# TheoCoombes/ClipCap

Measured on AMD Instinct MI355X. Metric: train samples/sec (512-d prefix, 40-tok caption), higher is better.
Workload: dtype bf16; 1 GPU; BASELINE configs[1]: TransformerMapper(8L,P=L=10,H=8)+frozen GPT-2-small; per_gpu_batch=256, global_batch=256, encoder_dim=512, train_language_model=False, parallelism=dp1

## Files before the change

clipcap_amd/_lib.py:

```python
from __future__ import annotations

import ctypes as C
import os
import threading

HERE = os.path.dirname(os.path.abspath(__file__))
_SEL = os.environ.get("CLIPCAP_HIP_LIB", "")
LIB_PATH = os.path.join(HERE, "libclipcap_hip.so") if not _SEL else os.path.join(HERE, "libclipcap_hip_lab.so") if _SEL == "lab" else _SEL
IS_LAB = _SEL == "lab"

ERR = {0: "ok", -1: "invalid argument", -2: "unsupported shape / alignment", -3: "kernel launch failed", -4: "invalid state"}


class HipExtensionMissing(RuntimeError):
    pass


class CCError(RuntimeError):
    pass


OP_BF16, OP_FP16, OP_X3 = 0, 1, 2


def op_dtype_of(precision) -> int:
    if precision in ("bf16", None) or (precision == OP_BF16 and not isinstance(precision, bool)):
        return OP_BF16
    if precision in (16, "fp16", "16", OP_FP16):
        return OP_FP16
    if precision in (32, 64, "32", "64", "bf16x3", "fp32", OP_X3):
        return OP_X3
    raise ValueError(f"unsupported precision {precision!r}: use 32 / 64 (split-bf16 operands, the reference default), 16 (fp16 operands) "
                     "or 'bf16' (bf16 operands)")


class MapperCfg(C.Structure):
    _fields_ = [(n, C.c_int32) for n in ("E", "D", "P", "L", "H", "N", "Hm", "W", "use_pos", "op_dtype")]


class Gpt2Cfg(C.Structure):
    _fields_ = [(n, C.c_int32) for n in ("D", "H", "NL", "V", "Vp", "NPOS", "op_dtype")]


class Gpt2Shape(C.Structure):
    _fields_ = [(n, C.c_int32) for n in ("B", "L", "T", "cap", "mode")] + [(n, C.c_float) for n in ("p_embd", "p_attn", "p_resid")] + \
               [("drop_seed", C.c_uint64)]


_P, _I, _L, _F = C.c_void_p, C.c_int32, C.c_int64, C.c_float
_MC, _GC, _GS = C.POINTER(MapperCfg), C.POINTER(Gpt2Cfg), C.POINTER(Gpt2Shape)

SIGNATURES = {
    "cc_abi_version": (_I, []),
    "cc_mapper_param_count": (_L, [_MC]),
    "cc_mapper_param_offsets": (_I, [_MC, C.POINTER(_L)]),
    "cc_mapper_ws_bytes": (_L, [_MC, _I, _I]),
    "cc_mapper_sync_weights": (_I, [_MC, _P, _P, _P]),
    "cc_mapper_transpose_weights": (_I, [_MC, _P, _P]),
    "cc_gpt2_sync_weights": (_I, [_GC, _P, _P, _P]),
    "cc_gpt2_transpose_weights": (_I, [_GC, _P, _P]),
    "cc_mapper_fwd": (_I, [_MC, _I, _P, _P, _P, _P, _P, _I, _P]),
    "cc_mapper_attention_probs": (_I, [_MC, _I, _P, _I, _P, _P]),
    "cc_mapper_bwd": (_I, [_MC, _I, _P, _P, _P, _P, _P, _P]),
    "cc_mapper_bwd_range": (_I, [_MC, _I, _P, _P, _P, _P, _P, _I, _I, _P]),
    "cc_gpt2_bwd_range": (_I, [_GC, _GS, _P, _P, _P, _P, _P, _P, _I, _I, _P]),
    "cc_gpt2_param_count": (_L, [_GC]),
    "cc_gpt2_param_offsets": (_I, [_GC, C.POINTER(_L)]),
    "cc_gpt2_ws_bytes": (_L, [_GC, _GS]),
    "cc_gpt2_embed": (_I, [_GC, _GS, _P, _P, _P, _P, _P]),
    "cc_gpt2_embed_from": (_I, [_GC, _GS, _P, _P, _P, _P]),
    "cc_gpt2_fwd": (_I, [_GC, _GS, _P, _P, _P, _P]),
    "cc_gpt2_logits": (_I, [_GC, _GS, _P, _P, _P, _P, _L, _P]),
    "cc_gpt2_logits_bwd": (_I, [_GC, _GS, _P, _P, _P, _P, _L, _P, _P, _P]),
    "cc_lmhead_ce_fwd": (_I, [_GC, _GS, _P, _P, _P, _P, _P, _P]),
    "cc_lmhead_score": (_I, [_GC, _GS, _P, _P, _P, _P, _I, _P, _P, _P]),
    "cc_lmhead_ce_bwd": (_I, [_GC, _GS, _P, _P, _P, _P, _P, _P, _P]),
    "cc_gpt2_bwd": (_I, [_GC, _GS, _P, _P, _P, _P, _P, _P, _P]),
    "cc_decode_ws_bytes": (_L, [_GC, _I, _I]),
    "cc_decode_fwd": (_I, [_GC, _I, _I, _I, _I, _P, _P, _P, _P, _P, _P, _P, _L, _P]),
    "cc_decode_part_floats": (_L, [_GC, _I]),
    "cc_decode_fwd_p": (_I, [_GC, _I, _I, _I, _I, _P, _P, _P, _P, _P, _P, _P, _L, _P, _P]),
    "cc_decode_fwd_g": (_I, [_GC, _I, _I, _I, _I, _P, _P, _P, _P, _P, _I, _P, _P, _L, _P, _P]),
    "cc_beam_step_p": (_I, [_I, _I, _I, _P, _L, _P, _I, _F, _I, _I, _P, _P, _P, _P, _P, _P, _P]),
    "cc_decode_reorder": (_I, [_GC, _I, _I, _I, _I, _P, _P, _P, _P]),
    "cc_beam_step": (_I, [_I, _I, _I, _P, _L, _F, _I, _I, _P, _P, _P, _P, _P, _P, _P]),
    "cc_beam_ws_bytes": (_L, [_I, _I, _I]),
    "cc_embed_tokens": (_I, [_GC, _I, _P, _P, _P, _P]),
    "cc_embed_tokens_bwd": (_I, [_GC, _I, _P, _P, _P, _P]),
    "cc_embed_tokens_bwd_ws": (_I, [_GC, _I, _P, _P, _P, _P, _P]),
    "cc_embed_tokens_bwd_ws_bytes": (_L, [_GC, _I]),
    "cc_beam_advance": (_I, [_GC, _I, _I, _P, _P, _P, _I, _I, _P, _P, _I, _I, _P, _P, _P, _P]),
    "cc_adamw_step": (_I, [_P, _P, _P, _P, _L, _F, _F, _F, _F, _F, _I, _F, _P, _P, _P]),
    "cc_adamw_step_cast": (_I, [_I, _P, _P, _P, _P, _L, _F, _F, _F, _F, _F, _I, _F, _P, _P, _P, _P]),
    "cc_cast_op16": (_I, [_I, _P, _P, _L, _P]),
    "cc_grad_wire_pack": (_I, [_P, _P, _L, _P]),
    "cc_grad_wire_unpack": (_I, [_P, _P, _L, _P]),
    "cc_grad_nonfinite": (_I, [_P, _L, _P, _P]),
    "cc_loss_scale_update": (_I, [_P, _P, _F, _F, _I, _P]),
    "cc_dropout_mask": (_I, [C.c_uint64, _I, _I, _F, _L, _P, _P]),
    "cc_sample_step": (_I, [_P, _I, _I, _I, _F, _I, _F, _I, _P, _I, _I, _F, _P, _P, _P, _P]),
    "cc_sample_step_lp": (_I, [_P, _I, _I, _I, _F, _I, _F, _I, _P, _I, _I, _F, _I, _F, _P, _P, _P, _P]),
    "cc_wgrad_scratch_bytes": (_L, []),
    "cc_gemm_wgrad": (_I, [_I, _P, _I, _P, _I, _I, _I, _I, _P, _I, _P, _P]),
    "cc_x3_image_bytes": (_L, [_L, _L]),
    "cc_x3_split_rows": (_I, [_I, _P, _L, _I, _I, _I, _P, _P]),
    "cc_gemm_act": (_I, [_I, _I, _I, _P, _I, _I, _P, _I, _I, _I, _I, _P, _I, _I, _P, _I, _P, _P, _L, _P]),
    "cc_gemm_resid": (_I, [_I, _I, _I, _P, _I, _I, _P, _I, _I, _I, _I, _P, _P, _I, _P, _F, C.c_uint64, _I, _I, _P, _L, _P]),
    "cc_gemm_dact": (_I, [_I, _I, _I, _P, _I, _I, _P, _I, _I, _I, _I, _P, _I, _I, _P, _I, _P, _L, _P]),
    "cc_gemm_f32": (_I, [_I, _I, _I, _P, _I, _I, _P, _I, _I, _I, _I, _P, _I, _P, _I, _F, _I, _P, _L, _P]),
    "cc_gemm_wgrad_split": (_I, [_I, _P, _I, _I, _P, _I, _I, _I, _I, _P, _I, _P, _P, _L, _P]),
    "cc_gemm_tile_mode": (_I, [_I]),
    "cc_gemm_skinny_mode": (_I, [_I]),
    "cc_decode_mode": (_I, [_I]),
    "cc_gemm_op16_f32": (_I, [_I, _I, _I, _P, _I, _P, _I, _I, _I, _I, _P, _I, _P, _I, _P]),
    "cc_layernorm_fwd": (_I, [_I, _P, _P, _P, _P, _P, _P, _I, _I, _P]),
    "cc_attention_fwd": (_I, [_I, _P, _I, _I, _I, _I, _I, _P, _P, _P]),
    "cc_attention_bwd": (_I, [_I, _P, _P, _P, _P, _P, _I, _I, _I, _I, _I, _P, _P]),
    "cc_red_scratch_floats": (_L, []),
    "cc_layernorm_bwd": (_I, [_I, _P, _P, _I, _P, _P, _P, _P, _P, _P, _P, _P, _P, _P, _I, _I, _P, _P]),
    "cc_colsum_bf16": (_I, [_I, _P, _I, _I, _I, _P, _P, _P]),
    "cc_colsum_multi": (_I, [_I, _P, _P, _I, _I, _I, _I, _P, _P]),
    "cc_batch_sum": (_I, [_P, _L, _P, _I, _I, _P, _P]),
    "cc_comm_unique_id": (_I, [_P]),
    "cc_comm_create": (_I, [C.POINTER(_P), _I, _I, _P]),
    "cc_allreduce_bucket": (_I, [_P, _P, _L, _I, _P]),
    "cc_broadcast_bucket": (_I, [_P, _P, _L, _I, _I, _P]),
    "cc_reduce_bucket": (_I, [_P, _P, _L, _I, _I, _P]),
    "cc_comm_destroy": (_I, [_P]),
    "cc_comm_count": (_I, [_P, C.POINTER(_I)]),
    "cc_prof_start": (_I, [_I, _I]),
    "cc_prof_stop": (_I, [C.POINTER(C.c_float), C.POINTER(C.c_double), C.POINTER(_I)]),
}

LAB_SIGNATURES = {
    "cc_decode_ws_check": (_I, [_GC, _I, _I, _P, _P]),
    "cc_decode_image_bytes": (_L, [_GC]),
    "cc_decode_image": (_I, [_GC, _P, _P, _P]),
    "cc_decode_xt_image_bytes": (_L, [_GC]),
    "cc_decode_xt_image": (_I, [_GC, _P, _P, _P]),
    "cc_decode_fwd_x": (_I, [_GC, _I, _I, _I, _I, _P, _P, _P, _P, _P, _P, _P, _I, _P, _P, _L, _P, _P]),
    "cc_decode_last_path": (_I, []),
}

ABI_VERSION = 3

SITES = {"lmhead_fwd": 1, "lmhead_dgrad": 2, "gpt2_fc_fwd": 3, "gpt2_proj2_fwd": 4, "gpt2_fc_dgrad": 5, "mapper_fc1_fwd": 6,
         "mapper_qkv_fwd": 7, "mapper_wgrad_fc2": 8, "all_gemms": 100}

_lib = None
_lock = threading.Lock()


def lib() -> C.CDLL:
    global _lib
    if _lib is not None:
        return _lib
    with _lock:
        if _lib is None:
            if not os.path.exists(LIB_PATH):
                raise HipExtensionMissing(
                    f"{LIB_PATH} not found: build it with `make -C clipcap_amd/csrc` (hipcc, gfx950). "
                    "clipcap_amd has no CPU fallback.")
            try:
                l = C.CDLL(LIB_PATH)
            except OSError as e:
                raise HipExtensionMissing(f"cannot load {LIB_PATH}: {e}") from e
            sigs = dict(SIGNATURES, **LAB_SIGNATURES) if IS_LAB else SIGNATURES
            for name, (res, args) in sigs.items():
                fn = getattr(l, name)
                fn.restype = res
                fn.argtypes = args
            if l.cc_abi_version() != ABI_VERSION:
                raise HipExtensionMissing(f"libclipcap_hip.so ABI version {l.cc_abi_version()} != {ABI_VERSION} (include/clipcap_hip.h); rebuild")
            _lib = l
    return _lib


def check(rc: int, what: str = "") -> int:
    if rc < 0:
        raise CCError(f"{what or 'clipcap_hip call'} failed: {ERR.get(rc, rc)} ({rc})")
    return rc
```

clipcap_amd/csrc/api.hip:

```cpp
#include "../../include/clipcap_hip.h"
#include "gemm_api.h"
#include "kernels.h"
#include "shared.h"

using namespace CC_NS;

#define CC_TRY(expr)                 \
    do {                             \
        int _e = (expr);             \
        if (_e != CC_OK) return _e;  \
    } while (0)

#include <vector>

namespace {

constexpr int MAX_LAYERS = 96;

#define CC_TIMED(site, st, expr)                 \
    do {                                         \
        cc_shared::ProfScope _ps(site, st);      \
        int _e = (expr);                         \
        if (_e != CC_OK) return _e;              \
    } while (0)

struct TileScope {
    int old;
    bool on;
    explicit TileScope(int mode) : old(cc_shared::g_gemm_tile_mode), on(mode != -2) { if (on) cc_shared::g_gemm_tile_mode = mode; }
    ~TileScope() { if (on) cc_shared::g_gemm_tile_mode = old; }
};
inline int env_tile(const char* name) {
    const char* e = cc_lab_env(name);
    return e ? atoi(e) : -2;
}

struct Carver {
    char* base;
    size_t off = 0;
    explicit Carver(void* p) : base(static_cast<char*>(p)) {}
    template <class T>
    T* take(size_t n) {
        off = (off + 255) & ~size_t(255);
        T* r = base ? reinterpret_cast<T*>(base + off) : nullptr;
        off += n * sizeof(T);
        return r;
    }
};

inline hipStream_t S_(void* s) { return static_cast<hipStream_t>(s); }
inline int rup(int x, int m) { return (x + m - 1) / m * m; }

constexpr int PL = kX3 ? 3 : 1;
inline const uint16_t* W16(const uint16_t* w16, int64_t off) { return w16 + (size_t)PL * off; }
inline uint16_t* W16(uint16_t* w16, int64_t off) { return w16 + (size_t)PL * off; }
inline size_t x3_img(size_t rows, size_t depth) { return ((rows * 3 * depth * sizeof(op16_t)) + 255) & ~size_t(255); }
template <class WS>
inline Call call_of(hipStream_t st, const WS& w) { return Call{st, w.red, w.x3, w.x3_bytes}; }

struct MapperOff {
    int64_t lin_w, lin_b, prefix, pos;
    struct Layer {
        int64_t n1w, n1b, wq, wkv, wp, bp, n2w, n2b, w1, b1, w2, b2;
    } layer[MAX_LAYERS];
    int64_t total;
};

bool mapper_cfg_ok(const cc_mapper_cfg* c) {
    return c && (c->op_dtype == CC_OP) && c->E > 0 && c->D > 0 && c->P > 0 && c->L > 0 && c->H > 0 && c->N >= 0 && c->N <= MAX_LAYERS && c->Hm > 0 && c->W >= 1 &&
           (c->E % 8) == 0 && (c->D % 8) == 0 && (c->Hm % 8) == 0 && (c->D % c->H) == 0 && ((c->D / c->H) % 8) == 0;
}

void mapper_offsets(const cc_mapper_cfg* c, MapperOff& o) {
    int64_t p = 0;
    const int64_t D = c->D, E = c->E, PD = (int64_t)c->P * D, Hm = c->Hm;
    o.lin_w = p; p += PD * E;
    o.lin_b = p; p += PD;
    o.prefix = p; p += (int64_t)c->L * D;
    if (c->W > 1 && c->use_pos) { o.pos = p; p += (int64_t)c->W * PD; } else o.pos = -1;
    for (int l = 0; l < c->N; l++) {
        auto& y = o.layer[l];
        y.n1w = p; p += D;
        y.n1b = p; p += D;
        y.wq = p; p += D * D;
        y.wkv = p; p += 2 * D * D;
        y.wp = p; p += D * D;
        y.bp = p; p += D;
        y.n2w = p; p += D;
        y.n2b = p; p += D;
        y.w1 = p; p += Hm * D;
        y.b1 = p; p += Hm;
        y.w2 = p; p += D * Hm;
        y.b2 = p; p += D;
    }
    o.total = p;
}

constexpr int kDeferRows = 40960;
struct MapperWS {
    act_t* emb16;
    float* lin_tmp;
    float* x[MAX_LAYERS + 1];
    float* x1[MAX_LAYERS];
    act_t *xn1[MAX_LAYERS], *xn2[MAX_LAYERS], *qkv[MAX_LAYERS], *att[MAX_LAYERS], *h[MAX_LAYERS];
    float *lse[MAX_LAYERS], *mean1[MAX_LAYERS], *rstd1[MAX_LAYERS], *mean2[MAX_LAYERS], *rstd2[MAX_LAYERS];
    float* dx32;
    act_t *dx16, *dx16b, *dh16, *dxn16, *datt16, *dqkv16, *dlin16;
    act_t *gdx[MAX_LAYERS], *gdxb[MAX_LAYERS], *gdh[MAX_LAYERS], *gdqkv[MAX_LAYERS];
    bool own_grads;
    float* wg_scratch;
    float* red;
    float* adelta;
    uint16_t* gimg;
    char* x3;
    size_t x3_bytes;
    size_t bytes;
};

void mapper_carve(const cc_mapper_cfg* c, int B, int save, void* ws, MapperWS& w) {
    Carver cv(ws);
    const int S = c->W * c->P + c->L;
    const size_t M = (size_t)B * S, D = c->D;
    w.emb16 = cv.take<act_t>((size_t)B * c->W * c->E);
    w.lin_tmp = c->W > 1 ? cv.take<float>((size_t)B * c->W * c->P * D) : nullptr;
    const int nx = save ? c->N + 1 : 2;
    float* xb[MAX_LAYERS + 1];
    for (int i = 0; i < nx; i++) xb[i] = cv.take<float>(M * D);
    for (int l = 0; l <= c->N; l++) w.x[l] = save ? xb[l] : xb[l & 1];
    const int nl = save ? c->N : 1;
    for (int l = 0; l < c->N; l++) {
        const bool fresh = l < nl;
        const int s = fresh ? l : 0;
        if (fresh) {
            w.x1[l] = cv.take<float>(M * D);
            w.xn1[l] = cv.take<act_t>(M * D);
            w.xn2[l] = cv.take<act_t>(M * D);
            w.qkv[l] = cv.take<act_t>(M * 3 * D);
            w.att[l] = cv.take<act_t>(M * D);
            w.h[l] = cv.take<act_t>(M * c->Hm);
            w.lse[l] = cv.take<float>((size_t)B * c->H * S);
            w.mean1[l] = cv.take<float>(M);
            w.rstd1[l] = cv.take<float>(M);
            w.mean2[l] = cv.take<float>(M);
            w.rstd2[l] = cv.take<float>(M);
        } else {
            w.x1[l] = w.x1[s]; w.xn1[l] = w.xn1[s]; w.xn2[l] = w.xn2[s]; w.qkv[l] = w.qkv[s]; w.att[l] = w.att[s]; w.h[l] = w.h[s];
            w.lse[l] = w.lse[s]; w.mean1[l] = w.mean1[s]; w.rstd1[l] = w.rstd1[s]; w.mean2[l] = w.mean2[s]; w.rstd2[l] = w.rstd2[s];
        }
    }
    if (save) {
        w.dx32 = cv.take<float>(M * D);
        w.dx16 = cv.take<act_t>(M * D);
        w.dx16b = cv.take<act_t>(M * D);
        w.dh16 = cv.take<act_t>(M * c->Hm);
        w.dxn16 = cv.take<act_t>(M * D);
        w.datt16 = cv.take<act_t>(M * D);
        w.dqkv16 = cv.take<act_t>(M * 3 * D);
        w.dlin16 = cv.take<act_t>((size_t)B * c->W * c->P * D);
        w.own_grads = !kX3 && M <= (size_t)kDeferRows && c->N <= 8;
        for (int l = 0; l < c->N; l++) {
            const bool own = w.own_grads;
            w.gdx[l] = own ? cv.take<act_t>(M * D) : w.dx16;
            w.gdxb[l] = own ? cv.take<act_t>(M * D) : w.dx16b;
            w.gdh[l] = own ? cv.take<act_t>(M * c->Hm) : w.dh16;
            w.gdqkv[l] = own ? cv.take<act_t>(M * 3 * D) : w.dqkv16;
        }
        w.wg_scratch = cv.take<float>(WGRAD_SCRATCH_BYTES / sizeof(float));
        w.red = cv.take<float>(RED_SCRATCH_FLOATS);
        w.adelta = cv.take<float>((size_t)B * c->H * S);
        w.gimg = kX3 ? reinterpret_cast<uint16_t*>(cv.take<char>(x3_img(M, std::max<size_t>(3 * (size_t)D, c->Hm)))) : nullptr;
    } else {
        w.dx32 = nullptr; w.dx16 = w.dx16b = w.dh16 = w.dxn16 = w.datt16 = w.dqkv16 = w.dlin16 = nullptr; w.wg_scratch = nullptr; w.adelta = nullptr;
        w.red = nullptr;
        w.gimg = nullptr;
        for (int l = 0; l < c->N; l++) w.gdx[l] = w.gdxb[l] = w.gdh[l] = w.gdqkv[l] = nullptr;
        w.own_grads = false;
    }
    w.x3 = nullptr; w.x3_bytes = 0;
    if (kX3) {
        const size_t Hm = c->Hm, Mb = (size_t)B * c->W, PD = (size_t)c->P * D;
        size_t need = std::max(x3_img(Mb, c->E), x3_img(M, std::max(D, Hm)));
        if (save) {
            need = std::max(need, x3_img(M, 3 * D));
            need = std::max(need, std::max(x3_img(M, D) + x3_img(M, Hm), x3_img(M, 3 * D) + x3_img(M, D)));
            need = std::max(need, x3_img(Mb, PD) + x3_img(Mb, c->E));
        }
        w.x3_bytes = need;
        w.x3 = cv.take<char>(need);
    }
    w.bytes = (cv.off + 255) & ~size_t(255);
}

struct Gpt2Off {
    int64_t wte, wpe, lnf_w, lnf_b;
    struct Layer {
        int64_t l1w, l1b, aw, ab, pw, pb, l2w, l2b, fw, fb, p2w, p2b;
    } layer[MAX_LAYERS];
    int64_t total;
};

bool gpt2_cfg_ok(const cc_gpt2_cfg* c) {
    return c && (c->op_dtype == CC_OP) && c->D > 0 && c->H > 0 && c->NL > 0 && c->NL <= MAX_LAYERS && c->V > 0 && c->Vp >= c->V && (c->Vp % 128) == 0 &&
           c->NPOS > 0 && (c->D % 8) == 0 && (c->D % c->H) == 0 && ((c->D / c->H) % 8) == 0;
}

void gpt2_offsets(const cc_gpt2_cfg* c, Gpt2Off& o) {
    int64_t p = 0;
    const int64_t D = c->D;
    o.wte = p; p += (int64_t)c->Vp * D;
    o.wpe = p; p += (int64_t)c->NPOS * D;
    for (int l = 0; l < c->NL; l++) {
        auto& y = o.layer[l];
        y.l1w = p; p += D;
        y.l1b = p; p += D;
        y.aw = p; p += D * 3 * D;
        y.ab = p; p += 3 * D;
        y.pw = p; p += D * D;
        y.pb = p; p += D;
        y.l2w = p; p += D;
        y.l2b = p; p += D;
        y.fw = p; p += D * 4 * D;
        y.fb = p; p += 4 * D;
        y.p2w = p; p += 4 * D * D;
        y.p2b = p; p += D;
    }
    o.lnf_w = p; p += D;
    o.lnf_b = p; p += D;
    o.total = p;
}

static bool x3_img_on() {
    static const bool on = []() { const char* e = cc_lab_env("CC_X3_IMG"); return !e || atoi(e) != 0; }();
    return on;
}
static bool lm_exp_form(const cc_gpt2_shape* s) {
    static const bool env = []() { const char* e = cc_lab_env("CC_LM_EXPFORM"); return !e || atoi(e) != 0; }();
    if (CC_OP == 0) return env;
    if (CC_OP == 2) return env && x3_img_on() && s->mode == 1;
    return false;
}
static Act lm_logits(const cc_gpt2_cfg* c, const cc_gpt2_shape* s, act_t* logits16) { return Act(logits16, (kX3 && lm_exp_form(s)) ? c->Vp : 0); }

struct Gpt2WS {
    float* x[MAX_LAYERS + 1];
    float* x1[MAX_LAYERS];
    act_t *qkv[MAX_LAYERS], *u[MAX_LAYERS];
    Act xn1[MAX_LAYERS], xn2[MAX_LAYERS], att[MAX_LAYERS], hact[MAX_LAYERS];
    float *lse[MAX_LAYERS], *mean1[MAX_LAYERS], *rstd1[MAX_LAYERS], *mean2[MAX_LAYERS], *rstd2[MAX_LAYERS];
    act_t* hf16;
    float *meanf, *rstdf;
    int *target, *row_map;
    int* keep;
    act_t* logits16;
    float *pmax, *psum, *tgt_logit, *lse_row, *row_loss;
    float *cref, *lmfac;
    act_t* hfs16;
    float* dx32;
    Act dx16, dx16b, du16, dqkv16;
    act_t *dhf16, *dxn16, *datt16;
    float* wg_scratch;
    float* red;
    void* scat;
    float* adelta;
    char* x3;
    size_t x3_bytes;
    size_t bytes;
};

void gpt2_carve(const cc_gpt2_cfg* c, const cc_gpt2_shape* s, int cap, void* ws, Gpt2WS& w) {
    Carver cv(ws);
    const int B = s->B, T = s->T, hd = c->D / c->H;
    const size_t M = (size_t)B * T, D = c->D, Mc = (size_t)B * cap;
    const bool keep = s->mode >= 1, full = s->mode >= 2;
    const bool img = kX3 && !full && x3_img_on();
    const bool bimg = img && keep && s->p_resid == 0.f && s->p_attn == 0.f && s->p_embd == 0.f;
    const int xw = img ? (int)D : 0, attw = (img && attn_fwd_can_image(T, hd)) ? (int)D : 0, hw = img ? 4 * (int)D : 0;
    const int dxw = bimg ? (int)D : 0, dqw = (bimg && attn_bwd_can_image(T, hd)) ? 3 * (int)D : 0;
    const int nx = keep ? c->NL + 1 : 2;
    float* xb[MAX_LAYERS + 1];
    for (int i = 0; i < nx; i++) xb[i] = cv.take<float>(M * D);
    for (int l = 0; l <= c->NL; l++) w.x[l] = keep ? xb[l] : xb[l & 1];
    for (int l = 0; l < c->NL; l++) {
        const bool k0 = keep || l == 0, f0 = full || l == 0;
        w.x1[l] = k0 ? cv.take<float>(M * D) : w.x1[0];
        w.qkv[l] = k0 ? cv.take<act_t>(M * 3 * D) : w.qkv[0];
        w.u[l] = k0 ? cv.take<act_t>(M * 4 * D) : w.u[0];
        w.lse[l] = k0 ? cv.take<float>((size_t)B * c->H * T) : w.lse[0];
        w.mean1[l] = k0 ? cv.take<float>(M) : w.mean1[0];
        w.rstd1[l] = k0 ? cv.take<float>(M) : w.rstd1[0];
        w.mean2[l] = k0 ? cv.take<float>(M) : w.mean2[0];
        w.rstd2[l] = k0 ? cv.take<float>(M) : w.rstd2[0];
        w.xn1[l] = f0 ? Act(cv.take<act_t>(M * D * ((kX3 && !full) ? 3 : 2) / 2), xw) : w.xn1[0];
        w.xn2[l] = f0 ? Act(cv.take<act_t>(M * D * ((kX3 && !full) ? 3 : 2) / 2), xw) : w.xn2[0];
        w.att[l] = k0 ? Act(cv.take<act_t>(M * D * ((kX3 && !full) ? 3 : 2) / 2), attw) : w.att[0];
        w.hact[l] = f0 ? Act(cv.take<act_t>(M * 4 * D * ((kX3 && !full) ? 3 : 2) / 2), hw) : w.hact[0];
    }
    const size_t Mh = std::max(M, Mc);
    w.hf16 = cv.take<act_t>(Mh * D);
    w.meanf = cv.take<float>(Mh);
    w.rstdf = cv.take<float>(Mh);
    w.target = cv.take<int>(Mh);
    w.row_map = cv.take<int>(Mh);
    w.keep = nullptr;
    if (keep) {
        const int npart = c->Vp / 64;
        w.logits16 = cv.take<act_t>(Mc * c->Vp * ((kX3 && !full) ? 3 : 2) / 2);
        w.pmax = cv.take<float>(Mc * npart);
        w.psum = cv.take<float>(Mc * npart);
        w.tgt_logit = cv.take<float>(Mc);
        w.lse_row = cv.take<float>(Mc);
        w.row_loss = cv.take<float>(Mc);
        w.cref = cv.take<float>(Mc);
        w.lmfac = cv.take<float>(2 * Mc);
        w.hfs16 = full ? cv.take<act_t>(Mc * D) : nullptr;
        w.dx32 = cv.take<float>(M * D);
        w.dx16 = Act(cv.take<act_t>(M * D * ((kX3 && !full) ? 3 : 2) / 2), dxw);
        w.dx16b = full ? Act(cv.take<act_t>(M * D)) : w.dx16;
        w.dhf16 = cv.take<act_t>(Mc * D);
        w.du16 = Act(cv.take<act_t>(M * 4 * D * ((kX3 && !full) ? 3 : 2) / 2), hw);
        w.dxn16 = cv.take<act_t>(M * D);
        w.datt16 = cv.take<act_t>(M * D);
        w.dqkv16 = Act(cv.take<act_t>(M * 3 * D * ((kX3 && !full) ? 3 : 2) / 2), dqw);
        w.wg_scratch = full ? cv.take<float>(WGRAD_SCRATCH_BYTES / sizeof(float)) : nullptr;
        w.red = full ? cv.take<float>(RED_SCRATCH_FLOATS) : nullptr;
        w.scat = full ? cv.take<char>(scatter_ws_bytes((int)Mc, (int)D)) : nullptr;
        w.adelta = cv.take<float>((size_t)B * c->H * T);
    } else {
        w.wg_scratch = nullptr; w.adelta = nullptr; w.red = nullptr; w.scat = nullptr;
        w.logits16 = nullptr; w.pmax = w.psum = w.tgt_logit = w.lse_row = w.row_loss = nullptr;
        w.cref = w.lmfac = nullptr; w.hfs16 = nullptr;
        w.dx32 = nullptr; w.dx16 = w.dx16b = w.du16 = w.dqkv16 = Act(); w.dhf16 = w.dxn16 = w.datt16 = nullptr;
        if (Mc > 0) {
            const int npart = c->Vp / 64;
            w.pmax = cv.take<float>(Mc * npart);
            w.psum = cv.take<float>(Mc * npart);
            w.tgt_logit = cv.take<float>(Mc);
            w.lse_row = cv.take<float>(Mc);
            w.keep = cv.take<int>(Mc);
        }
    }
    w.x3 = nullptr; w.x3_bytes = 0;
    if (kX3) {
        size_t need = x3_img(Mh, 4 * D);
        if (keep) need = std::max(need, x3_img(Mc, c->Vp));
        if (full) need = std::max(need, std::max(x3_img(M, D) + x3_img(M, 4 * D), x3_img(Mc, c->Vp) + x3_img(Mc, D)));
        w.x3_bytes = need;
        w.x3 = cv.take<char>(need);
    }
    w.bytes = (cv.off + 255) & ~size_t(255);
}

}

extern "C" {

int CC_API(cc_mapper_bwd_range)(const cc_mapper_cfg* c, int32_t B, const float* w32, const uint16_t* w16, void* ws, const float* dout, float* g32,
                        int32_t l_hi, int32_t l_lo, void* stream);
int CC_API(cc_gpt2_bwd_range)(const cc_gpt2_cfg* c, const cc_gpt2_shape* s, const float* w32, const uint16_t* w16, void* ws, const int64_t* tokens,
                      float* dprefix, float* g32, int32_t l_hi, int32_t l_lo, void* stream);

int64_t CC_API(cc_mapper_param_count)(const cc_mapper_cfg* cfg) {
    if (!mapper_cfg_ok(cfg)) return CC_ERR_SHAPE;
    MapperOff o;
    mapper_offsets(cfg, o);
    return o.total;
}

int CC_API(cc_mapper_param_offsets)(const cc_mapper_cfg* cfg, int64_t* offs) {
    if (!mapper_cfg_ok(cfg) || !offs) return CC_ERR_SHAPE;
    MapperOff o;
    mapper_offsets(cfg, o);
    int k = 0;
    offs[k++] = o.lin_w; offs[k++] = o.lin_b; offs[k++] = o.prefix; offs[k++] = o.pos;
    for (int l = 0; l < cfg->N; l++) {
        const auto& y = o.layer[l];
        const int64_t v[12] = {y.n1w, y.n1b, y.wq, y.wkv, y.wp, y.bp, y.n2w, y.n2b, y.w1, y.b1, y.w2, y.b2};
        for (int i = 0; i < 12; i++) offs[k++] = v[i];
    }
    return CC_OK;
}

int64_t CC_API(cc_mapper_ws_bytes)(const cc_mapper_cfg* cfg, int32_t B, int32_t save) {
    if (!mapper_cfg_ok(cfg) || B <= 0) return CC_ERR_SHAPE;
    MapperWS w;
    mapper_carve(cfg, B, save, nullptr, w);
    return (int64_t)w.bytes;
}

#if CC_OP == 2
static int mapper_sync_x3(const cc_mapper_cfg* c, const float* w32, uint16_t* w16, hipStream_t st) {
    MapperOff o;
    mapper_offsets(c, o);
    const int D = c->D, Hm = c->Hm;
    X3SplitBatch sb;
    sb.add(w32 + o.lin_w, W16(w16, o.lin_w), c->P * D, c->E, 0, 1);
    for (int l = 0; l < c->N; l++) {
        const auto& y = o.layer[l];
        const int64_t off[4] = {y.wq, y.wp, y.w1, y.w2};
        const int R[4] = {3 * D, D, Hm, D}, C[4] = {D, D, D, Hm};
        for (int i = 0; i < 4; i++) {
            if (sb.n + 2 > 32) { CC_TRY(x3_split_multi(sb, st)); sb.n = 0; }
            sb.add(w32 + off[i], W16(w16, off[i]), R[i], C[i], 0, 1);
            sb.add(w32 + off[i], W16(w16, o.total + off[i]), R[i], C[i], 1, 1);
        }
    }
    return x3_split_multi(sb, st);
}
#endif

static int mapper_transposes(const cc_mapper_cfg* c, uint16_t* w16, hipStream_t st) {
    if (kX3) return CC_ERR_ARG;
    MapperOff o;
    mapper_offsets(c, o);
    op16_t* t = w16 + o.total;
    const int D = c->D, Hm = c->Hm;
    TransposeBatch tb;
    for (int l = 0; l < c->N; l++) {
        const auto& y = o.layer[l];
        tb.add(w16 + y.wq, t + y.wq, 3 * D, D);
        tb.add(w16 + y.wp, t + y.wp, D, D);
        tb.add(w16 + y.w1, t + y.w1, Hm, D);
        tb.add(w16 + y.w2, t + y.w2, D, Hm);
        if (tb.n == 32) { CC_TRY(transpose_bf16_multi(tb, st)); tb.n = 0; }
    }
    CC_TRY(transpose_bf16_multi(tb, st));
    return CC_OK;
}

int CC_API(cc_mapper_sync_weights)(const cc_mapper_cfg* c, const float* w32, uint16_t* w16, void* stream) {
    if (!mapper_cfg_ok(c) || !w32 || !w16) return CC_ERR_ARG;
    hipStream_t st = S_(stream);
#if CC_OP == 2
    return mapper_sync_x3(c, w32, w16, st);
#else
    MapperOff o;
    mapper_offsets(c, o);
    CC_TRY(f32_to_bf16(w32, w16, (size_t)o.total, st));
    return mapper_transposes(c, w16, st);
#endif
}

int CC_API(cc_mapper_transpose_weights)(const cc_mapper_cfg* c, uint16_t* w16, void* stream) {
    if (!mapper_cfg_ok(c) || !w16) return CC_ERR_ARG;
    return mapper_transposes(c, w16, S_(stream));
}

int CC_API(cc_mapper_fwd)(const cc_mapper_cfg* c, int32_t B, const float* w32, const uint16_t* w16, const float* emb, void* ws, float* out,
                  int32_t save, void* stream) {
    if (!mapper_cfg_ok(c) || B <= 0 || !w32 || !w16 || !emb || !ws || !out) return CC_ERR_ARG;
    hipStream_t st = S_(stream);
    MapperOff o;
    mapper_offsets(c, o);
    MapperWS w;
    mapper_carve(c, B, save, ws, w);
    Call cx = call_of(st, w);
    const int D = c->D, PP = c->W * c->P, S = PP + c->L, M = B * S, H = c->H, hd = D / H, Hm = c->Hm;
    const int PD = c->P * D;
    CC_TRY(f32_to_act(emb, w.emb16, (size_t)B * c->W * c->E, st));
    if (c->W == 1) {
        CC_TRY(gemm_f32out(0, 0, w.emb16, c->E, W16(w16, o.lin_w), c->E, B, PD, c->E, w.x[0], S * D, w32 + o.lin_b, 0, 1.0f, 1, cx));
    } else {
        CC_TRY(gemm_f32out(0, 0, w.emb16, c->E, W16(w16, o.lin_w), c->E, B * c->W, PD, c->E, w.lin_tmp, PD, w32 + o.lin_b, 0, 1.0f, 1, cx));
        CC_TRY(copy_rows(w.lin_tmp, (size_t)PP * D, w.x[0], (size_t)S * D, PP * D, B, st));
        if (o.pos >= 0) CC_TRY(add_rows(w.x[0], (size_t)S * D, w32 + o.pos, PP * D, B, st));
    }
    CC_TRY(broadcast_rows(w.x[0] + (size_t)PP * D, (size_t)S * D, w32 + o.prefix, c->L * D, B, st));
    for (int l = 0; l < c->N; l++) {
        const auto& y = o.layer[l];
        CC_TRY(ln_fwd(w.x[l], D, nullptr, w32 + y.n1w, w32 + y.n1b, w.xn1[l], nullptr, w.mean1[l], w.rstd1[l], M, D, st));
        CC_TIMED(CC_SITE_MAPPER_QKV_FWD, st, gemm_bf16out(0, 0, w.xn1[l], D, W16(w16, y.wq), D, M, 3 * D, D, w.qkv[l], 3 * D, nullptr, 0, nullptr, cx));
        CC_TRY(attn_fwd(w.qkv[l], B, S, H, hd, false, w.att[l], w.lse[l], st));
        CC_TRY(gemm_resid(0, 0, w.att[l], D, W16(w16, y.wp), D, M, D, D, w.x1[l], w.x[l], D, w32 + y.bp, cx));
        CC_TRY(ln_fwd(w.x1[l], D, nullptr, w32 + y.n2w, w32 + y.n2b, w.xn2[l], nullptr, w.mean2[l], w.rstd2[l], M, D, st));
        CC_TIMED(CC_SITE_MAPPER_FC1_FWD, st, gemm_bf16out(0, 0, w.xn2[l], D, W16(w16, y.w1), D, M, Hm, D, w.h[l], Hm, w32 + y.b1, 1, nullptr, cx));
        CC_TRY(gemm_resid(0, 0, w.h[l], Hm, W16(w16, y.w2), Hm, M, D, Hm, w.x[l + 1], w.x1[l], D, w32 + y.b2, cx));
    }
    CC_TRY(copy_rows(w.x[c->N] + (size_t)PP * D, (size_t)S * D, out, (size_t)c->L * D, c->L * D, B, st));
    return CC_OK;
}

int CC_API(cc_mapper_attention_probs)(const cc_mapper_cfg* c, int32_t B, void* ws, int32_t layer, float* out, void* stream) {
    if (!mapper_cfg_ok(c) || B <= 0 || !ws || !out || layer < 0 || layer >= c->N) return CC_ERR_ARG;
    MapperWS w;
    mapper_carve(c, B, 1, ws, w);
    const int S = c->W * c->P + c->L;
    return attn_probs(w.qkv[layer], B, S, c->H, c->D / c->H, out, S_(stream));
}

int CC_API(cc_mapper_bwd)(const cc_mapper_cfg* c, int32_t B, const float* w32, const uint16_t* w16, void* ws, const float* dout, float* g32,
                  void* stream) {
    if (!mapper_cfg_ok(c)) return CC_ERR_ARG;
    return CC_API(cc_mapper_bwd_range)(c, B, w32, w16, ws, dout, g32, c->N, 0, stream);
}

int CC_API(cc_mapper_bwd_range)(const cc_mapper_cfg* c, int32_t B, const float* w32, const uint16_t* w16, void* ws, const float* dout, float* g32,
                        int32_t l_hi, int32_t l_lo, void* stream) {
    if (!mapper_cfg_ok(c) || B <= 0 || !w32 || !w16 || !ws || !dout || !g32 || l_lo < 0 || l_hi > c->N || l_lo > l_hi) return CC_ERR_ARG;
    hipStream_t st = S_(stream);
    MapperOff o;
    mapper_offsets(c, o);
    MapperWS w;
    mapper_carve(c, B, 1, ws, w);
    Call cx = call_of(st, w);
    const int D = c->D, PP = c->W * c->P, S = PP + c->L, M = B * S, H = c->H, hd = D / H, Hm = c->Hm;
    const int PD = c->P * D;
    const uint16_t* w16t = W16(w16, o.total);
    if (l_hi == c->N) {
        if (hipMemsetAsync(w.dx32, 0, (size_t)M * D * sizeof(float), st) != hipSuccess) return CC_ERR_LAUNCH;
        CC_TRY(copy_rows(dout, (size_t)c->L * D, w.dx32 + (size_t)PP * D, (size_t)S * D, c->L * D, B, st));
        if (c->N > 0) CC_TRY(f32_to_act(w.dx32, w.gdx[c->N - 1], (size_t)M * D, st));
    }
    WgradBatch wb;
    wb.defer = true;
    constexpr bool kDeferAll = !kX3;
    static const bool defer_all_on = []() { const char* e = cc_lab_env("CC_MAPPER_WGRAD_DEFER"); return !e || atoi(e) != 0; }();
    static const int defer_rows = []() { const char* e = cc_lab_env("CC_MAPPER_DEFER_ROWS"); return e ? std::min(atoi(e), kDeferRows) : kDeferRows; }();
    const bool defer_all = kDeferAll && defer_all_on && w.own_grads && 4 * (l_hi - l_lo) <= 32 && M <= defer_rows;
    if (defer_all) { wb.direct = true; wb.cap = 4 * (l_hi - l_lo); }
    ColsumBatch cs;
#if CC_OP == 2
    static const bool share = []() { const char* e = cc_lab_env("CC_X3_SHARE"); return !e || atoi(e) != 0; }();
    int g2rc = CC_OK;
    auto G2 = [&](const act_t* t, int width) -> ActIn {
        if (!share) return t;
        g2rc = x3_split_rows(t, (size_t)width, w.gimg, M, width, 0, st);
        return ActIn(reinterpret_cast<const act_t*>(w.gimg), width);
    };
#else
    auto G2 = [&](const act_t* t, int) -> ActIn { return t; };
    const int g2rc = CC_OK;
#endif
    for (int l = l_hi - 1; l >= l_lo; l--) {
        const auto& y = o.layer[l];
        act_t* dx16 = w.gdx[l];
        act_t* dx16b = w.gdxb[l];
        act_t* dh16 = w.gdh[l];
        act_t* dqkv16 = w.gdqkv[l];
        act_t* dx16_below = l > 0 ? w.gdx[l - 1] : w.datt16;
        const ActIn gx = G2(dx16, D);
        CC_TRY(g2rc);
        CC_TIMED(CC_SITE_MAPPER_WGRAD_FC2, st, gemm_wgrad(gx, D, w.h[l], Hm, D, Hm, M, g32 + y.w2, Hm, w.wg_scratch, cx, &wb));
        if (l == c->N - 1) CC_TRY(colsum_bf16(dx16, D, M, D, g32 + y.b2, cx));
        CC_TRY(gemm_dact(0, 0, gx, D, W16(w16t, y.w2), D, M, Hm, D, dh16, Hm, w.h[l], 1, cx));
        const ActIn gh = G2(dh16, Hm);
        CC_TRY(g2rc);
        CC_TRY(gemm_wgrad(gh, Hm, w.xn2[l], D, Hm, D, M, g32 + y.w1, D, w.wg_scratch, cx, &wb));
        if (defer_all) cs.add(dh16, g32 + y.b1);
        else CC_TRY(colsum_bf16(dh16, Hm, M, Hm, g32 + y.b1, cx));
        CC_TRY(gemm_bf16out(0, 0, gh, Hm, W16(w16t, y.w1), Hm, M, D, Hm, w.dxn16, D, nullptr, 0, nullptr, cx));
        CC_TRY(ln_bwd(w.dxn16, w.x1[l], D, nullptr, w.mean2[l], w.rstd2[l], w32 + y.n2w, w.dx32, w.dx32, dx16b, g32 + y.n2w,
                      g32 + y.n2b, M, D, cx, g32 + y.bp));
        const ActIn gb = G2(dx16b, D);
        CC_TRY(g2rc);
        CC_TRY(gemm_wgrad(gb, D, w.att[l], D, D, D, M, g32 + y.wp, D, w.wg_scratch, cx, &wb));
        CC_TRY(gemm_bf16out(0, 0, gb, D, W16(w16t, y.wp), D, M, D, D, w.datt16, D, nullptr, 0, nullptr, cx));
        CC_TRY(attn_bwd(w.qkv[l], w.datt16, w.att[l], w.lse[l], w.adelta, B, S, H, hd, false, dqkv16, st));
        const ActIn gq = G2(dqkv16, 3 * D);
        CC_TRY(g2rc);
        CC_TRY(gemm_wgrad(gq, 3 * D, w.xn1[l], D, 3 * D, D, M, g32 + y.wq, D, w.wg_scratch, cx, &wb));
        CC_TRY(gemm_bf16out(0, 0, gq, 3 * D, W16(w16t, y.wq), 3 * D, M, D, 3 * D, w.dxn16, D, nullptr, 0, nullptr, cx));
        if (!defer_all) CC_TRY(wgrad_flush(wb, st));
        CC_TRY(ln_bwd(w.dxn16, w.x[l], D, nullptr, w.mean1[l], w.rstd1[l], w32 + y.n1w, w.dx32, w.dx32, dx16_below, g32 + y.n1w,
                      g32 + y.n1b, M, D, cx, l > 0 ? g32 + o.layer[l - 1].b2 : nullptr));
    }
    CC_TRY(wgrad_flush(wb, st));
    CC_TRY(colsum_bf16_multi(cs, Hm, M, Hm, cx));
    if (l_lo > 0) return CC_OK;
    CC_TRY(batch_sum(w.dx32 + (size_t)PP * D, (size_t)S * D, g32 + o.prefix, c->L * D, B, cx));
    if (o.pos >= 0) CC_TRY(batch_sum(w.dx32, (size_t)S * D, g32 + o.pos, PP * D, B, cx));
    CC_TRY(slice_f32_to_bf16(w.dx32, (size_t)S * D, w.dlin16, (size_t)PP * D, PP * D, B, st));
    CC_TRY(gemm_wgrad(w.dlin16, PD, w.emb16, c->E, PD, c->E, B * c->W, g32 + o.lin_w, c->E, w.wg_scratch, cx));
    CC_TRY(colsum_bf16(w.dlin16, PD, B * c->W, PD, g32 + o.lin_b, cx));
    return CC_OK;
}

namespace {
static bool gelu_grad_fwd() {
    static const bool on = []() { const char* e = cc_lab_env("CC_GELU_GRAD_FWD"); return !e || atoi(e) != 0; }();
    return on;
}
static bool shape_ok(const cc_gpt2_cfg* c, const cc_gpt2_shape* s) {
    return s && s->B > 0 && s->T > 0 && s->L >= 0 && s->L <= s->T && s->cap >= s->T - s->L && s->mode >= 0 && s->mode <= 2 && s->T <= c->NPOS &&
           s->p_embd >= 0.f && s->p_embd < 1.f && s->p_attn >= 0.f && s->p_attn < 1.f && s->p_resid >= 0.f && s->p_resid < 1.f;
}
}

int64_t CC_API(cc_gpt2_param_count)(const cc_gpt2_cfg* cfg) {
    if (!gpt2_cfg_ok(cfg)) return CC_ERR_SHAPE;
    Gpt2Off o;
    gpt2_offsets(cfg, o);
    return o.total;
}

int CC_API(cc_gpt2_param_offsets)(const cc_gpt2_cfg* cfg, int64_t* offs) {
    if (!gpt2_cfg_ok(cfg) || !offs) return CC_ERR_SHAPE;
    Gpt2Off o;
    gpt2_offsets(cfg, o);
    int k = 0;
    offs[k++] = o.wte; offs[k++] = o.wpe;
    for (int l = 0; l < cfg->NL; l++) {
        const auto& y = o.layer[l];
        const int64_t v[12] = {y.l1w, y.l1b, y.aw, y.ab, y.pw, y.pb, y.l2w, y.l2b, y.fw, y.fb, y.p2w, y.p2b};
        for (int i = 0; i < 12; i++) offs[k++] = v[i];
    }
    offs[k++] = o.lnf_w; offs[k++] = o.lnf_b;
    return CC_OK;
}

int64_t CC_API(cc_gpt2_ws_bytes)(const cc_gpt2_cfg* cfg, const cc_gpt2_shape* s) {
    if (!gpt2_cfg_ok(cfg) || !shape_ok(cfg, s)) return CC_ERR_SHAPE;
    Gpt2WS w;
    gpt2_carve(cfg, s, s->T - s->L, nullptr, w);
    return (int64_t)w.bytes;
}

#if CC_OP == 2
static int gpt2_sync_x3(const cc_gpt2_cfg* c, const float* w32, uint16_t* w16, hipStream_t st) {
    Gpt2Off o;
    gpt2_offsets(c, o);
    const int D = c->D;
    X3SplitBatch sb;
    sb.add(w32 + o.wte, W16(w16, o.wte), c->Vp, D, 0, 1);
    sb.add(w32 + o.wte, W16(w16, o.total + o.wte), c->Vp, D, 1, 1);
    CC_TRY(x3_split_multi(sb, st));
    sb.n = 0;
    for (int l = 0; l < c->NL; l++) {
        const auto& y = o.layer[l];
        const int64_t off[4] = {y.aw, y.pw, y.fw, y.p2w};
        const int R[4] = {D, D, D, 4 * D}, C[4] = {3 * D, D, 4 * D, D};
        for (int i = 0; i < 4; i++) {
            if (sb.n + 2 > 32) { CC_TRY(x3_split_multi(sb, st)); sb.n = 0; }
            sb.add(w32 + off[i], W16(w16, off[i]), R[i], C[i], 0, 1);
            sb.add(w32 + off[i], W16(w16, o.total + off[i]), R[i], C[i], 1, 1);
        }
    }
    return x3_split_multi(sb, st);
}
#endif

static int gpt2_transposes(const cc_gpt2_cfg* c, uint16_t* w16, hipStream_t st) {
    if (kX3) return CC_ERR_ARG;
    Gpt2Off o;
    gpt2_offsets(c, o);
    op16_t* t = w16 + o.total;
    const int D = c->D;
    CC_TRY(transpose_bf16(w16 + o.wte, t + o.wte, c->Vp, D, st));
    TransposeBatch tb;
    for (int l = 0; l < c->NL; l++) {
        const auto& y = o.layer[l];
        tb.add(w16 + y.aw, t + y.aw, D, 3 * D);
        tb.add(w16 + y.pw, t + y.pw, D, D);
        tb.add(w16 + y.fw, t + y.fw, D, 4 * D);
        tb.add(w16 + y.p2w, t + y.p2w, 4 * D, D);
        if (tb.n == 32) { CC_TRY(transpose_bf16_multi(tb, st)); tb.n = 0; }
    }
    CC_TRY(transpose_bf16_multi(tb, st));
    return CC_OK;
}

int CC_API(cc_gpt2_sync_weights)(const cc_gpt2_cfg* c, const float* w32, uint16_t* w16, void* stream) {
    if (!gpt2_cfg_ok(c) || !w32 || !w16) return CC_ERR_ARG;
    hipStream_t st = S_(stream);
#if CC_OP == 2
    return gpt2_sync_x3(c, w32, w16, st);
#else
    Gpt2Off o;
    gpt2_offsets(c, o);
    CC_TRY(f32_to_bf16(w32, w16, (size_t)o.total, st));
    return gpt2_transposes(c, w16, st);
#endif
}

int CC_API(cc_gpt2_transpose_weights)(const cc_gpt2_cfg* c, uint16_t* w16, void* stream) {
    if (!gpt2_cfg_ok(c) || !w16) return CC_ERR_ARG;
    return gpt2_transposes(c, w16, S_(stream));
}

int CC_API(cc_dropout_mask)(uint64_t seed, int32_t site, int32_t layer, float p, int64_t n, uint8_t* out, void* stream) {
    if (!out || n < 0 || site < 0 || site > 3 || layer < 0 || layer > 255 || p < 0.f || p >= 1.f) return CC_ERR_ARG;
    return dropout_mask_u8(out, (size_t)n, make_drop(p, seed, (unsigned)site, (unsigned)layer), S_(stream));
}

int CC_API(cc_gpt2_embed)(const cc_gpt2_cfg* c, const cc_gpt2_shape* s, const float* w32, const float* prefix, const int64_t* tokens, void* ws,
                  void* stream) {
    if (!gpt2_cfg_ok(c) || !shape_ok(c, s) || !w32 || !ws || (s->L > 0 && !prefix) || (s->T > s->L && !tokens)) return CC_ERR_ARG;
    Gpt2Off o;
    gpt2_offsets(c, o);
    Gpt2WS w;
    gpt2_carve(c, s, s->T - s->L, ws, w);
    CC_TRY(embed_concat(prefix, reinterpret_cast<const long long*>(tokens), s->cap, w32 + o.wte, w32 + o.wpe, w.x[0], s->B, s->L, s->T,
                        c->D, 0, S_(stream)));
    return dropout_f32(w.x[0], (size_t)s->B * s->T * c->D, make_drop(s->p_embd, s->drop_seed, DROP_EMBD, 0), S_(stream));
}

int CC_API(cc_gpt2_embed_from)(const cc_gpt2_cfg* c, const cc_gpt2_shape* s, const float* w32, const float* inputs_embeds, void* ws,
                       void* stream) {
    if (!gpt2_cfg_ok(c) || !shape_ok(c, s) || !w32 || !ws || !inputs_embeds) return CC_ERR_ARG;
    Gpt2Off o;
    gpt2_offsets(c, o);
    Gpt2WS w;
    gpt2_carve(c, s, s->T - s->L, ws, w);
    return embed_concat(inputs_embeds, nullptr, 0, w32 + o.wte, w32 + o.wpe, w.x[0], s->B, s->T, s->T, c->D, 0, S_(stream));
}

int CC_API(cc_gpt2_fwd)(const cc_gpt2_cfg* c, const cc_gpt2_shape* s, const float* w32, const uint16_t* w16, void* ws, void* stream) {
    if (!gpt2_cfg_ok(c) || !shape_ok(c, s) || !w32 || !w16 || !ws) return CC_ERR_ARG;
    hipStream_t st = S_(stream);
    Gpt2Off o;
    gpt2_offsets(c, o);
    Gpt2WS w;
    gpt2_carve(c, s, s->T - s->L, ws, w);
    Call cx = call_of(st, w);
    const int D = c->D, M = s->B * s->T, H = c->H, hd = D / H;
    const uint16_t* w16t = W16(w16, o.total);
    for (int l = 0; l < c->NL; l++) {
        const auto& y = o.layer[l];
        CC_TRY(ln_fwd(w.x[l], D, nullptr, w32 + y.l1w, w32 + y.l1b, w.xn1[l], nullptr, w.mean1[l], w.rstd1[l], M, D, st));
        CC_TRY(gemm_bf16out(0, 0, w.xn1[l], D, W16(w16t, y.aw), D, M, 3 * D, D, w.qkv[l], 3 * D, w32 + y.ab, 0, nullptr, cx));
        CC_TRY(attn_fwd(w.qkv[l], s->B, s->T, H, hd, true, w.att[l], w.lse[l], st, make_drop(s->p_attn, s->drop_seed, DROP_ATTN, l)));
        {
            static const int tile_proj = env_tile("CC_TILE_PROJ");
            TileScope ts(tile_proj);
            CC_TRY(gemm_resid(0, 0, w.att[l], D, W16(w16t, y.pw), D, M, D, D, w.x1[l], w.x[l], D, w32 + y.pb, cx,
                              make_drop(s->p_resid, s->drop_seed, DROP_RESID_ATTN, l)));
        }
        CC_TRY(ln_fwd(w.x1[l], D, nullptr, w32 + y.l2w, w32 + y.l2b, w.xn2[l], nullptr, w.mean2[l], w.rstd2[l], M, D, st));
        {
            static const int tile_fc = env_tile("CC_TILE_FC");
            TileScope ts(tile_fc);
            CC_TIMED(CC_SITE_GPT2_FC_FWD, st, gemm_bf16out(0, 0, w.xn2[l], D, W16(w16t, y.fw), D, M, 4 * D, D, w.hact[l], 4 * D, w32 + y.fb, (s->mode >= 1 && gelu_grad_fwd()) ? 3 : 2,
                                                            s->mode >= 1 ? w.u[l] : nullptr, cx));
        }
        {
            static const int tile_proj2 = env_tile("CC_TILE_PROJ2");
            TileScope ts(tile_proj2);
            CC_TIMED(CC_SITE_GPT2_PROJ2_FWD, st, gemm_resid(0, 0, w.hact[l], 4 * D, W16(w16t, y.p2w), 4 * D, M, D, 4 * D, w.x[l + 1], w.x1[l], D, w32 + y.p2b, cx,
                                                           make_drop(s->p_resid, s->drop_seed, DROP_RESID_MLP, l)));
        }
    }
    return CC_OK;
}

int CC_API(cc_gpt2_logits)(const cc_gpt2_cfg* c, const cc_gpt2_shape* s, const float* w32, const uint16_t* w16, void* ws, float* logits,
                   int64_t ldl, void* stream) {
    if (!gpt2_cfg_ok(c) || !shape_ok(c, s) || !w32 || !w16 || !ws || !logits) return CC_ERR_ARG;
    const int Ns = std::min(c->Vp, rup(c->V, 8));
    if (ldl < Ns || (ldl & 3) || ldl > 0x7fffffff) return CC_ERR_SHAPE;
    hipStream_t st = S_(stream);
    Gpt2Off o;
    gpt2_offsets(c, o);
    Gpt2WS w;
    gpt2_carve(c, s, s->T - s->L, ws, w);
    Call cx = call_of(st, w);
    const int D = c->D, M = s->B * s->T;
    CC_TRY(ln_fwd(w.x[c->NL], D, nullptr, w32 + o.lnf_w, w32 + o.lnf_b, w.hf16, nullptr, w.meanf, w.rstdf, M, D, st));
    return gemm_f32out(0, 0, w.hf16, D, W16(w16, o.wte), D, M, Ns, D, logits, (int)ldl, nullptr, 0, 1.0f, 1, cx);
}

int CC_API(cc_lmhead_ce_fwd)(const cc_gpt2_cfg* c, const cc_gpt2_shape* s, const float* w32, const uint16_t* w16, void* ws, const int64_t* tokens,
                     float* stats, void* stream) {
    if (!gpt2_cfg_ok(c) || !shape_ok(c, s) || s->mode < 1 || s->L < 1 || !w32 || !w16 || !ws || !tokens || !stats) return CC_ERR_ARG;
    hipStream_t st = S_(stream);
    Gpt2Off o;
    gpt2_offsets(c, o);
    Gpt2WS w;
    const int cap = s->T - s->L;
    gpt2_carve(c, s, cap, ws, w);
    Call cx = call_of(st, w);
    const int D = c->D, Mc = s->B * cap, npart = c->Vp / 64;
    if (cap != s->cap) return CC_ERR_SHAPE;
    if (hipMemsetAsync(stats, 0, 2 * sizeof(float), st) != hipSuccess) return CC_ERR_LAUNCH;
    CC_TRY(ce_targets(reinterpret_cast<const long long*>(tokens), w.target, w.row_map, s->B, cap, s->L, s->T, st));
    CC_TRY(ln_fwd(w.x[c->NL], D, w.row_map, w32 + o.lnf_w, w32 + o.lnf_b, w.hf16, nullptr, w.meanf, w.rstdf, Mc, D, st));
    const bool ef = lm_exp_form(s);
    const op16_t* wte_rows = kX3 ? reinterpret_cast<const op16_t*>(w32 + o.wte) : W16(w16, o.wte);
    if (ef) CC_TRY(lm_tgt_ref(w.hf16, wte_rows, D, w.target, w.cref, Mc, st));
    CC_TIMED(CC_SITE_LMHEAD_FWD, st, gemm_lmhead(w.hf16, D, W16(w16, o.wte), D, Mc, c->Vp, c->V, D, lm_logits(c, s, w.logits16), c->Vp, w.pmax, w.psum, npart, w.target, w.tgt_logit, cx,
                                                 ef ? w.cref : nullptr));
    CC_TRY(ce_rows(w.pmax, w.psum, npart, w.target, ef ? w.cref : w.tgt_logit, w.lse_row, w.row_loss, stats, Mc, st));
    return CC_OK;
}

int CC_API(cc_lmhead_score)(const cc_gpt2_cfg* c, const cc_gpt2_shape* s, const float* w32, const uint16_t* w16, void* ws, const int64_t* tokens,
                    int32_t ignore_zero, float* token_logprob, float* sample_stats, void* stream) {
    if (!gpt2_cfg_ok(c) || !shape_ok(c, s) || s->mode != 0 || s->L < 1 || !w32 || !w16 || !ws || !tokens || !token_logprob || !sample_stats)
        return CC_ERR_ARG;
    const int cap = s->T - s->L;
    if (cap < 1 || cap != s->cap) return CC_ERR_SHAPE;
    hipStream_t st = S_(stream);
    Gpt2Off o;
    gpt2_offsets(c, o);
    Gpt2WS w;
    gpt2_carve(c, s, cap, ws, w);
    Call cx = call_of(st, w);
    const int D = c->D, Mc = s->B * cap, npart = c->Vp / 64;
    CC_TRY(ce_targets(reinterpret_cast<const long long*>(tokens), w.target, w.row_map, s->B, cap, s->L, s->T, st));
    CC_TRY(score_keep(reinterpret_cast<const long long*>(tokens), w.keep, Mc, ignore_zero, st));
    CC_TRY(ln_fwd(w.x[c->NL], D, w.row_map, w32 + o.lnf_w, w32 + o.lnf_b, w.hf16, nullptr, w.meanf, w.rstdf, Mc, D, st));
    CC_TIMED(CC_SITE_LMHEAD_FWD, st, gemm_lmhead_score(w.hf16, D, W16(w16, o.wte), D, Mc, c->Vp, c->V, D, w.pmax, w.psum, npart, w.target, w.tgt_logit, cx));
    return score_rows(w.pmax, w.psum, npart, w.keep, w.tgt_logit, w.lse_row, token_logprob, sample_stats, s->B, cap, st);
}

int CC_API(cc_lmhead_ce_bwd)(const cc_gpt2_cfg* c, const cc_gpt2_shape* s, const float* w32, const uint16_t* w16, void* ws, const float* denom,
                     const float* loss_scale, float* g32, void* stream) {
    if (!gpt2_cfg_ok(c) || !shape_ok(c, s) || s->mode < 1 || !w32 || !w16 || !ws || !denom || (s->mode == 2 && !g32)) return CC_ERR_ARG;
    hipStream_t st = S_(stream);
    Gpt2Off o;
    gpt2_offsets(c, o);
    Gpt2WS w;
    const int cap = s->T - s->L;
    gpt2_carve(c, s, cap, ws, w);
    Call cx = call_of(st, w);
    const int D = c->D, Mc = s->B * cap, M = s->B * s->T;
    const bool full = s->mode == 2;
    const bool ef = lm_exp_form(s);
    const LmFix fix{w.lmfac, w.target, kX3 ? reinterpret_cast<const op16_t*>(w32 + o.wte) : W16(w16, o.wte)};
    if (ef) CC_TRY(lm_rowfac(w.cref, w.lse_row, w.target, denom, loss_scale, w.lmfac, Mc, st));
    const Act lg = lm_logits(c, s, w.logits16);
    ActIn dlog = lg;
    op16_t* dimg = (kX3 && !ef && !full && x3_img_on()) ? x3_scratch_block(cx, x3_img(Mc, c->Vp)) : nullptr;
    if (dimg) dlog = ActIn(reinterpret_cast<const act_t*>(dimg), c->Vp);
    if (!ef) CC_TRY(ce_dlogits(w.logits16, c->Vp, c->V, w.target, w.lse_row, denom, loss_scale, Mc, st, dimg));
    const auto lm_dgrad = [&]() {
        const int rc = gemm_nt_deepk(dlog, c->Vp, W16(w16, o.total + o.wte), c->Vp, Mc, D, c->Vp, w.dhf16, D, reinterpret_cast<float*>(w.du16.p),
                                     (size_t)M * 4 * D * sizeof(act_t), cx, ef ? &fix : nullptr);
        if (rc != CC_ERR_SHAPE) return rc;
        const int rc2 = gemm_bf16out(0, 0, dlog, c->Vp, W16(w16, o.total + o.wte), c->Vp, Mc, D, c->Vp, w.dhf16, D, nullptr, 0, nullptr, cx);
        return (rc2 != CC_OK || !ef) ? rc2 : lm_dgrad_fix(w.dhf16, w.lmfac, w.target, fix.wte, D, Mc, st);
    };
    CC_TIMED(CC_SITE_LMHEAD_DGRAD, st, lm_dgrad());
    if (full) {
        if (ef) {
            CC_TRY(lm_scale_rows(w.hf16, w.lmfac, w.hfs16, D, Mc, st));
            CC_TRY(gemm_wgrad(lg, c->Vp, w.hfs16, D, c->Vp, D, Mc, g32 + o.wte, D, w.wg_scratch, cx));
            ScatterSrc oh;
            oh.ids32 = w.target; oh.act = w.hf16; oh.fac = w.lmfac;
            CC_TRY(scatter_rows(oh, Mc, D, c->Vp, g32 + o.wte, w.scat, st));
        } else {
            CC_TRY(gemm_wgrad(lg, c->Vp, w.hf16, D, c->Vp, D, Mc, g32 + o.wte, D, w.wg_scratch, cx));
        }
    }
    if (hipMemsetAsync(w.dx32, 0, (size_t)M * D * sizeof(float), st) != hipSuccess) return CC_ERR_LAUNCH;
    const size_t dx16_bytes = (size_t)M * D * (w.dx16.img ? 3 * sizeof(op16_t) : sizeof(act_t));
    if (hipMemsetAsync(w.dx16.p, 0, dx16_bytes, st) != hipSuccess) return CC_ERR_LAUNCH;
    CC_TRY(ln_bwd(w.dhf16, w.x[c->NL], D, w.row_map, w.meanf, w.rstdf, w32 + o.lnf_w, nullptr, w.dx32, w.dx16, full ? g32 + o.lnf_w : nullptr,
                  full ? g32 + o.lnf_b : nullptr, Mc, D, cx));
    return CC_OK;
}

int CC_API(cc_gpt2_logits_bwd)(const cc_gpt2_cfg* c, const cc_gpt2_shape* s, const float* w32, const uint16_t* w16, void* ws, const float* dlogits,
                       int64_t ldl, float* dx0, float* g32, void* stream) {
    if (!gpt2_cfg_ok(c) || !shape_ok(c, s) || s->mode < 1 || s->L != 0 || !w32 || !w16 || !ws || !dlogits || ldl < c->V || (s->mode == 2 && !g32))
        return CC_ERR_ARG;
    hipStream_t st = S_(stream);
    Gpt2Off o;
    gpt2_offsets(c, o);
    Gpt2WS w;
    gpt2_carve(c, s, s->T, ws, w);
    Call cx = call_of(st, w);
    const int D = c->D, M = s->B * s->T;
    const bool full = s->mode == 2;
    CC_TRY(f32_to_op16_pad(dlogits, ldl, c->V, w.logits16, c->Vp, M, st));
    CC_TRY(gemm_bf16out(0, 0, w.logits16, c->Vp, W16(w16, o.total + o.wte), c->Vp, M, D, c->Vp, w.dhf16, D, nullptr, 0, nullptr, cx));
    if (full) CC_TRY(gemm_wgrad(w.logits16, c->Vp, w.hf16, D, c->Vp, D, M, g32 + o.wte, D, w.wg_scratch, cx));
    if (hipMemsetAsync(w.dx32, 0, (size_t)M * D * sizeof(float), st) != hipSuccess) return CC_ERR_LAUNCH;
    CC_TRY(ln_bwd(w.dhf16, w.x[c->NL], D, nullptr, w.meanf, w.rstdf, w32 + o.lnf_w, nullptr, w.dx32, w.dx16, full ? g32 + o.lnf_w : nullptr,
                  full ? g32 + o.lnf_b : nullptr, M, D, cx));
    CC_TRY(CC_API(cc_gpt2_bwd_range)(c, s, w32, w16, ws, nullptr, nullptr, g32, c->NL, 0, stream));
    if (dx0 && hipMemcpyAsync(dx0, w.dx32, (size_t)M * D * sizeof(float), hipMemcpyDeviceToDevice, st) != hipSuccess) return CC_ERR_LAUNCH;
    return CC_OK;
}

int CC_API(cc_gpt2_bwd)(const cc_gpt2_cfg* c, const cc_gpt2_shape* s, const float* w32, const uint16_t* w16, void* ws, const int64_t* tokens,
                float* dprefix, float* g32, void* stream) {
    if (!gpt2_cfg_ok(c)) return CC_ERR_ARG;
    return CC_API(cc_gpt2_bwd_range)(c, s, w32, w16, ws, tokens, dprefix, g32, c->NL, 0, stream);
}

int CC_API(cc_gpt2_bwd_range)(const cc_gpt2_cfg* c, const cc_gpt2_shape* s, const float* w32, const uint16_t* w16, void* ws, const int64_t* tokens,
                      float* dprefix, float* g32, int32_t l_hi, int32_t l_lo, void* stream) {
    if (!gpt2_cfg_ok(c) || !shape_ok(c, s) || s->mode < 1 || !w32 || !w16 || !ws || (s->L > 0 && !dprefix) || (s->mode == 2 && !g32) ||
        l_lo < 0 || l_hi > c->NL || l_lo > l_hi)
        return CC_ERR_ARG;
    hipStream_t st = S_(stream);
    Gpt2Off o;
    gpt2_offsets(c, o);
    Gpt2WS w;
    gpt2_carve(c, s, s->T - s->L, ws, w);
    Call cx = call_of(st, w);
    const int D = c->D, M = s->B * s->T, H = c->H, hd = D / H, D3 = 3 * D, D4 = 4 * D;
    const bool full = s->mode == 2;
    WgradBatch wb;
    wb.defer = full;
    WgradBatch* wbp = full ? &wb : nullptr;
    if (full && (w.dx16.img || w.dx16b.img || w.du16.img || w.dqkv16.img)) return CC_ERR_STATE;
    for (int l = l_hi - 1; l >= l_lo; l--) {
        const auto& y = o.layer[l];
        const bool top = l == c->NL - 1;
        if (top) CC_TRY(dropout_bf16(w.dx16.p, (size_t)M * D, make_drop(s->p_resid, s->drop_seed, DROP_RESID_MLP, l), st));
        if (full) {
            CC_TRY(gemm_wgrad(w.hact[l], D4, w.dx16.p, D, D4, D, M, g32 + y.p2w, D, w.wg_scratch, cx, wbp));
            if (top) CC_TRY(colsum_bf16(w.dx16.p, D, M, D, g32 + y.p2b, cx));
        }
        {
            static const int tile_dact = env_tile("CC_TILE_DACT");
            TileScope ts(tile_dact);
            CC_TRY(gemm_dact(0, 0, w.dx16, D, W16(w16, y.p2w), D, M, D4, D, w.du16, D4, w.u[l], gelu_grad_fwd() ? 3 : 2, cx));
        }
        if (full) {
            CC_TRY(gemm_wgrad(w.xn2[l], D, w.du16.p, D4, D, D4, M, g32 + y.fw, D4, w.wg_scratch, cx, wbp));
            CC_TRY(colsum_bf16(w.du16.p, D4, M, D4, g32 + y.fb, cx));
        }
        CC_TIMED(CC_SITE_GPT2_FC_DGRAD, st, gemm_bf16out(0, 0, w.du16, D4, W16(w16, y.fw), D4, M, D, D4, w.dxn16, D, nullptr, 0, nullptr, cx));
        CC_TRY(ln_bwd(w.dxn16, w.x1[l], D, nullptr, w.mean2[l], w.rstd2[l], w32 + y.l2w, w.dx32, w.dx32, w.dx16b, full ? g32 + y.l2w : nullptr,
                      full ? g32 + y.l2b : nullptr, M, D, cx, full ? g32 + y.pb : nullptr,
                      make_drop(s->p_resid, s->drop_seed, DROP_RESID_ATTN, l)));
        if (full) CC_TRY(gemm_wgrad(w.att[l], D, w.dx16b.p, D, D, D, M, g32 + y.pw, D, w.wg_scratch, cx, wbp));
        CC_TRY(gemm_bf16out(0, 0, w.dx16b, D, W16(w16, y.pw), D, M, D, D, w.datt16, D, nullptr, 0, nullptr, cx));
        CC_TRY(attn_bwd(w.qkv[l], w.datt16, w.att[l].p, w.lse[l], w.adelta, s->B, s->T, H, hd, true, w.dqkv16, st,
                        make_drop(s->p_attn, s->drop_seed, DROP_ATTN, l)));
        if (full) {
            CC_TRY(gemm_wgrad(w.xn1[l], D, w.dqkv16.p, D3, D, D3, M, g32 + y.aw, D3, w.wg_scratch, cx, wbp));
            CC_TRY(colsum_bf16(w.dqkv16.p, D3, M, D3, g32 + y.ab, cx));
        }
        CC_TRY(gemm_bf16out(0, 0, w.dqkv16, D3, W16(w16, y.aw), D3, M, D, D3, w.dxn16, D, nullptr, 0, nullptr, cx));
        if (full) CC_TRY(wgrad_flush(wb, st));
        CC_TRY(ln_bwd(w.dxn16, w.x[l], D, nullptr, w.mean1[l], w.rstd1[l], w32 + y.l1w, w.dx32, w.dx32, w.dx16, full ? g32 + y.l1w : nullptr,
                      full ? g32 + y.l1b : nullptr, M, D, cx, (full && l > 0) ? g32 + o.layer[l - 1].p2b : nullptr,
                      l > 0 ? make_drop(s->p_resid, s->drop_seed, DROP_RESID_MLP, l - 1) : Drop()));
    }
    if (l_lo > 0) return CC_OK;
    CC_TRY(dropout_f32(w.dx32, (size_t)M * D, make_drop(s->p_embd, s->drop_seed, DROP_EMBD, 0), st));
    if (s->L > 0) CC_TRY(copy_rows(w.dx32, (size_t)s->T * D, dprefix, (size_t)s->L * D, s->L * D, s->B, st));
    if (full) {
        if (tokens) {
            ScatterSrc e;
            e.ids64 = reinterpret_cast<const long long*>(tokens);
            e.ids_ld = s->cap;
            e.f32 = w.dx32 + (size_t)s->L * D; e.rpb = s->T - s->L; e.bstride = (size_t)s->T * D;
            CC_TRY(scatter_rows(e, s->B * (s->T - s->L), D, c->Vp, g32 + o.wte, w.scat, st));
        }
        CC_TRY(batch_sum(w.dx32, (size_t)s->T * D, g32 + o.wpe, s->T * D, s->B, cx));
    }
    return CC_OK;
}

int CC_API(cc_adamw_step)(float* p32, const float* g32, float* m, float* v, int64_t n, float lr, float beta1, float beta2, float eps,
                  float weight_decay, int32_t step, float grad_scale, const float* loss_scale, const float* found_inf, void* stream) {
    if (!p32 || !g32 || !m || !v || n < 0 || step < 0 || (step == 0 && !loss_scale)) return CC_ERR_ARG;
    return adamw(p32, g32, m, v, (size_t)n, lr, beta1, beta2, eps, weight_decay, step, grad_scale, loss_scale, found_inf, S_(stream));
}

int CC_API(cc_adamw_step_cast)(float* p32, const float* g32, float* m, float* v, int64_t n, float lr, float beta1, float beta2, float eps,
                       float weight_decay, int32_t step, float grad_scale, const float* loss_scale, const float* found_inf, uint16_t* w16, void* stream) {
    if (!p32 || !g32 || !m || !v || !w16 || n < 0 || step < 0 || (step == 0 && !loss_scale)) return CC_ERR_ARG;
    if (kX3) return CC_ERR_ARG;
    return adamw(p32, g32, m, v, (size_t)n, lr, beta1, beta2, eps, weight_decay, step, grad_scale, loss_scale, found_inf, S_(stream), w16);
}

int CC_API(cc_cast_op16)(const float* src, uint16_t* dst, int64_t n, void* stream) {
    if (!src || !dst || n < 0 || kX3) return CC_ERR_ARG;
    return f32_to_bf16(src, dst, (size_t)n, S_(stream));
}

int CC_API(cc_grad_wire_pack)(const float* g32, uint16_t* wire, int64_t n, void* stream) {
    if (!g32 || !wire || n < 0) return CC_ERR_ARG;
    return wire_pack(g32, wire, (size_t)n, S_(stream));
}

int CC_API(cc_grad_wire_unpack)(const uint16_t* wire, float* g32, int64_t n, void* stream) {
    if (!g32 || !wire || n < 0) return CC_ERR_ARG;
    return wire_unpack(wire, g32, (size_t)n, S_(stream));
}

int CC_API(cc_grad_nonfinite)(const float* g32, int64_t n, float* found_inf, void* stream) {
    if (!g32 || !found_inf || n < 0) return CC_ERR_ARG;
    return grad_nonfinite(g32, (size_t)n, found_inf, S_(stream));
}

int CC_API(cc_loss_scale_update)(float* state, float* found_inf, float growth, float backoff, int32_t interval, void* stream) {
    if (!state || !found_inf || growth < 1.f || backoff <= 0.f || backoff > 1.f || interval < 1) return CC_ERR_ARG;
    return loss_scale_update(state, found_inf, growth, backoff, interval, S_(stream));
}

int CC_API(cc_gemm_op16_f32)(int32_t al, int32_t bl, const uint16_t* A, int32_t lda, const uint16_t* B, int32_t ldb, int32_t M, int32_t N, int32_t K,
                     float* C, int32_t ldc, const float* bias, int32_t ksplit, void* stream) {
    if (!A || !B || !C || kX3) return CC_ERR_ARG;
    Call cx{S_(stream)};
    return gemm_f32out(al, bl, reinterpret_cast<const act_t*>(A), lda, B, ldb, M, N, K, C, ldc, ksplit > 1 ? nullptr : bias, ksplit > 1 ? 2 : 0, 1.0f, ksplit, cx);
}

int CC_API(cc_sample_step)(const float* logits, int32_t R, int32_t V, int32_t ld, float temperature, int32_t top_k, float top_p, int32_t mode,
                   const int64_t* history, int32_t hist_len, int32_t hist_ld, float repetition_penalty, const float* u, int32_t* next_token,
                   float* probs_out, void* stream) {
    if (!logits || !u || !next_token || R < 0) return CC_ERR_ARG;
    return sample_rows(logits, R, V, ld, temperature, top_k, top_p, mode, reinterpret_cast<const long long*>(history), hist_len, hist_ld,
                       repetition_penalty, u, next_token, probs_out, S_(stream));
}

int CC_API(cc_sample_step_lp)(const float* logits, int32_t R, int32_t V, int32_t ld, float temperature, int32_t top_k, float top_p, int32_t mode,
                      const int64_t* history, int32_t hist_len, int32_t hist_ld, float repetition_penalty, int32_t stop_token,
                      float length_penalty, const float* u, int32_t* next_token, float* probs_out, void* stream) {
    if (!logits || !u || !next_token || R < 0) return CC_ERR_ARG;
    return sample_rows(logits, R, V, ld, temperature, top_k, top_p, mode, reinterpret_cast<const long long*>(history), hist_len, hist_ld,
                       repetition_penalty, u, next_token, probs_out, S_(stream), stop_token, length_penalty);
}

int64_t CC_API(cc_wgrad_scratch_bytes)(void) { return (int64_t)WGRAD_SCRATCH_BYTES; }

int CC_API(cc_gemm_wgrad)(const uint16_t* X, int32_t ldx, const uint16_t* Y, int32_t ldy, int32_t Mw, int32_t Nw, int32_t K, float* dW, int32_t ldw,
                  float* scratch, void* stream) {
    if (!X || !Y || !dW || kX3) return CC_ERR_ARG;
    Call cx{S_(stream)};
    return gemm_wgrad(reinterpret_cast<const act_t*>(X), ldx, reinterpret_cast<const act_t*>(Y), ldy, Mw, Nw, K, dW, ldw, scratch, cx);
}

int CC_API(cc_layernorm_fwd)(const float* x, const float* gamma, const float* beta, uint16_t* y, float* mean, float* rstd, int32_t rows, int32_t D,
                     void* stream) {
    if (!x || !gamma || !beta || !y) return CC_ERR_ARG;
    return ln_fwd(x, D, nullptr, gamma, beta, reinterpret_cast<act_t*>(y), nullptr, mean, rstd, rows, D, S_(stream));
}

int64_t CC_API(cc_red_scratch_floats)(void) { return (int64_t)RED_SCRATCH_FLOATS; }

int CC_API(cc_layernorm_bwd)(const uint16_t* dy, const float* x, int32_t ldx, const int32_t* row_map, const float* mean, const float* rstd,
                     const float* gamma, const float* dres, float* dx32, uint16_t* dx16, float* dgamma, float* dbeta, float* dcol, int32_t rows,
                     int32_t D, float* red_ws, void* stream) {
    if (!dy || !x || !mean || !rstd || !gamma || !dx32 || !dgamma != !dbeta || kX3) return CC_ERR_ARG;
    Call cx{S_(stream), red_ws};
    return ln_bwd(reinterpret_cast<const act_t*>(dy), x, ldx, row_map, mean, rstd, gamma, dres, dx32, reinterpret_cast<act_t*>(dx16), dgamma,
                  dbeta, rows, D, cx, dcol);
}

int CC_API(cc_colsum_bf16)(const uint16_t* X, int32_t ld, int32_t M, int32_t N, float* out, float* red_ws, void* stream) {
    if (!X || !out || kX3) return CC_ERR_ARG;
    Call cx{S_(stream), red_ws};
    return colsum_bf16(reinterpret_cast<const act_t*>(X), ld, M, N, out, cx);
}

int CC_API(cc_colsum_multi)(const uint16_t* const* X_host, float* const* out_host, int32_t n, int32_t ld, int32_t M, int32_t N, float* red_ws,
                    void* stream) {
    if (!X_host || !out_host || n < 0 || n > 32 || kX3) return CC_ERR_ARG;
    ColsumBatch b;
    for (int i = 0; i < n; i++) {
        if (!X_host[i] || !out_host[i]) return CC_ERR_ARG;
        b.add(reinterpret_cast<const act_t*>(X_host[i]), out_host[i]);
    }
    Call cx{S_(stream), red_ws};
    return colsum_bf16_multi(b, ld, M, N, cx);
}

int CC_API(cc_batch_sum)(const float* src, int64_t src_stride, float* dst, int32_t len, int32_t B, float* red_ws, void* stream) {
    if (!src || !dst || len < 0 || src_stride < len) return CC_ERR_ARG;
    Call cx{S_(stream), red_ws};
    return batch_sum(src, (size_t)src_stride, dst, len, B, cx);
}

int CC_API(cc_attention_fwd)(const uint16_t* qkv, int32_t B, int32_t S, int32_t H, int32_t hd, int32_t causal, uint16_t* out, float* lse, void* stream) {
    if (!qkv || !out) return CC_ERR_ARG;
    return attn_fwd(reinterpret_cast<const act_t*>(qkv), B, S, H, hd, causal != 0, reinterpret_cast<act_t*>(out), lse, S_(stream));
}

int CC_API(cc_attention_bwd)(const uint16_t* qkv, const uint16_t* dout, const uint16_t* o, const float* lse, float* delta_ws, int32_t B, int32_t S,
                     int32_t H, int32_t hd, int32_t causal, uint16_t* dqkv, void* stream) {
    if (!qkv || !dout || !lse || !dqkv) return CC_ERR_ARG;
    return attn_bwd(reinterpret_cast<const act_t*>(qkv), reinterpret_cast<const act_t*>(dout), reinterpret_cast<const act_t*>(o), lse, delta_ws, B, S, H, hd,
                    causal != 0, reinterpret_cast<act_t*>(dqkv), S_(stream));
}

namespace {
inline bool al16(const void* p) { return ((uintptr_t)p & 15) == 0; }
inline bool hook_operands_ok(int al, int bl, const void* A, int a_img, int lda, const void* B, int ldb, int M, int N, int K) {
    if (!A || !B || !al16(A) || !al16(B) || M <= 0 || N <= 0 || K <= 0 || a_img < 0) return false;
    if (!kX3 && a_img) return false;
    return lda >= (a_img ? 0 : (al ? M : K)) && ldb >= (bl ? N : K);
}
inline void hook_scratch(Call& cx, void* x3, int64_t x3_bytes) {
    if (kX3 && x3 && x3_bytes > 0 && al16(x3)) { cx.x3 = static_cast<char*>(x3); cx.x3_bytes = (size_t)x3_bytes; }
}
inline bool hook_c_img_ok(int c_img, int N) { return c_img == 0 || (kX3 && c_img == N); }
}

int64_t CC_API(cc_x3_image_bytes)(int64_t rows, int64_t depth) {
    if (rows < 0 || depth < 0) return CC_ERR_ARG;
    return (int64_t)x3_img((size_t)rows, (size_t)depth);
}

int CC_API(cc_x3_split_rows)(const float* src, int64_t ld, int32_t rows, int32_t width, int32_t form, uint16_t* dst, void* stream) {
#if CC_OP == 2
    if (!src || !dst || rows < 0 || width < 0 || ld < width || (form != 0 && form != 1)) return CC_ERR_ARG;
    return x3_split_rows(src, (size_t)ld, dst, rows, width, form, S_(stream));
#else
    (void)src; (void)ld; (void)rows; (void)width; (void)form; (void)dst; (void)stream;
    return CC_ERR_ARG;
#endif
}

int CC_API(cc_gemm_act)(int32_t al, int32_t bl, const void* A, int32_t a_img, int32_t lda, const uint16_t* B, int32_t ldb, int32_t M, int32_t N, int32_t K,
                void* C, int32_t c_img, int32_t ldc, const float* bias, int32_t act, void* pre, void* x3, int64_t x3_bytes, void* stream) {
    if (!hook_operands_ok(al, bl, A, a_img, lda, B, ldb, M, N, K) || !C || !al16(C) || !al16(pre) || !al16(bias) || ldc < N || act < 0 || act > 3 ||
        !hook_c_img_ok(c_img, N))
        return CC_ERR_ARG;
    Call cx{S_(stream)};
    hook_scratch(cx, x3, x3_bytes);
    return gemm_bf16out(al, bl, ActIn(static_cast<const act_t*>(A), a_img), lda, B, ldb, M, N, K, Act(static_cast<act_t*>(C), c_img), ldc, bias, act,
                        static_cast<act_t*>(pre), cx);
}

int CC_API(cc_gemm_resid)(int32_t al, int32_t bl, const void* A, int32_t a_img, int32_t lda, const uint16_t* B, int32_t ldb, int32_t M, int32_t N, int32_t K,
                  float* out, const float* res, int32_t ld, const float* bias, float p, uint64_t seed, int32_t site, int32_t layer, void* x3,
                  int64_t x3_bytes, void* stream) {
    if (!hook_operands_ok(al, bl, A, a_img, lda, B, ldb, M, N, K) || !out || !res || !al16(out) || !al16(res) || !al16(bias) || ld < N || site < 0 ||
        site > 3 || layer < 0 || layer > 255 || p < 0.f || p >= 1.f)
        return CC_ERR_ARG;
    Call cx{S_(stream)};
    hook_scratch(cx, x3, x3_bytes);
    return gemm_resid(al, bl, ActIn(static_cast<const act_t*>(A), a_img), lda, B, ldb, M, N, K, out, res, ld, bias, cx,
                      make_drop(p, seed, (unsigned)site, (unsigned)layer));
}

int CC_API(cc_gemm_dact)(int32_t al, int32_t bl, const void* A, int32_t a_img, int32_t lda, const uint16_t* B, int32_t ldb, int32_t M, int32_t N, int32_t K,
                 void* C, int32_t c_img, int32_t ldc, const void* aux, int32_t act, void* x3, int64_t x3_bytes, void* stream) {
    if (!hook_operands_ok(al, bl, A, a_img, lda, B, ldb, M, N, K) || !C || !aux || !al16(C) || !al16(aux) || ldc < N || act < 1 || act > 3 ||
        !hook_c_img_ok(c_img, N))
        return CC_ERR_ARG;
    Call cx{S_(stream)};
    hook_scratch(cx, x3, x3_bytes);
    return gemm_dact(al, bl, ActIn(static_cast<const act_t*>(A), a_img), lda, B, ldb, M, N, K, Act(static_cast<act_t*>(C), c_img), ldc,
                     static_cast<const act_t*>(aux), act, cx);
}

int CC_API(cc_gemm_f32)(int32_t al, int32_t bl, const void* A, int32_t a_img, int32_t lda, const uint16_t* B, int32_t ldb, int32_t M, int32_t N, int32_t K,
                float* C, int32_t ldc, const float* bias, int32_t mode, float alpha, int32_t ksplit, void* x3, int64_t x3_bytes, void* stream) {
    if (!hook_operands_ok(al, bl, A, a_img, lda, B, ldb, M, N, K) || !C || !al16(C) || !al16(bias) || ldc < N || mode < 0 || mode > 2 || ksplit < 1 ||
        (bias && mode != 0))
        return CC_ERR_ARG;
    Call cx{S_(stream)};
    hook_scratch(cx, x3, x3_bytes);
    return gemm_f32out(al, bl, ActIn(static_cast<const act_t*>(A), a_img), lda, B, ldb, M, N, K, C, ldc, bias, mode, alpha, ksplit, cx);
}

int CC_API(cc_gemm_wgrad_split)(const void* X, int32_t x_img, int32_t ldx, const float* Y, int32_t ldy, int32_t Mw, int32_t Nw, int32_t K, float* dW,
                     int32_t ldw, float* scratch, void* x3, int64_t x3_bytes, void* stream) {
#if CC_OP == 2
    if (!X || !Y || !dW || !al16(X) || !al16(Y) || !al16(dW) || Mw <= 0 || Nw <= 0 || K <= 0 || x_img < 0 || (!x_img && ldx < Mw) || ldy < Nw || ldw < Nw)
        return CC_ERR_ARG;
    Call cx{S_(stream)};
    hook_scratch(cx, x3, x3_bytes);
    return gemm_wgrad(ActIn(static_cast<const act_t*>(X), x_img), ldx, Y, ldy, Mw, Nw, K, dW, ldw, scratch, cx);
#else
    (void)X; (void)x_img; (void)ldx; (void)Y; (void)ldy; (void)Mw; (void)Nw; (void)K; (void)dW; (void)ldw; (void)scratch; (void)x3; (void)x3_bytes; (void)stream;
    return CC_ERR_ARG;
#endif
}

}
```

clipcap_amd/csrc/gemm_api.h:

```cpp
#pragma once
#include "common.hip.h"
#include "shared.h"

namespace CC_NS {
int gemm_bf16out(int al, int bl, ActIn A, int lda, const op16_t* B, int ldb, int M, int N, int K, Act C, int ldc,
                 const float* bias, int act, act_t* pre, Call& cx);
int gemm_resid(int al, int bl, ActIn A, int lda, const op16_t* B, int ldb, int M, int N, int K, float* out, const float* res,
               int ld, const float* bias, Call& cx, Drop drop = Drop());
int gemm_f32out(int al, int bl, ActIn A, int lda, const op16_t* B, int ldb, int M, int N, int K, float* C, int ldc,
                const float* bias, int mode, float alpha, int ksplit, Call& cx);
int gemm_dact(int al, int bl, ActIn A, int lda, const op16_t* B, int ldb, int M, int N, int K, Act C, int ldc,
              const act_t* aux, int act, Call& cx);
int gemm_lmhead(ActIn A, int lda, const op16_t* B, int ldb, int M, int Vp, int V, int K, Act C, int ldc, float* pmax,
                float* psum, int npart, const int* target, float* tgt_logit, Call& cx, const float* cref = nullptr);
int gemm_lmhead_score(ActIn A, int lda, const op16_t* B, int ldb, int M, int Vp, int V, int K, float* pmax, float* psum, int npart,
                      const int* target, float* tgt_logit, Call& cx);

int gemm_logits_part(ActIn A, int lda, const op16_t* B, int ldb, int M, int Ns, int V, int K, float* C, int ldc, float* pmax, float* psum,
                     int npart, Call& cx);

#if CC_OP == 2
const op16_t* x3_operand(Call& cx, const float* src, size_t ld, int rows, int width, int form, bool first, int* rc);
#endif
inline op16_t* x3_scratch_block(const Call& cx, size_t bytes) { return (cx.x3 && bytes <= cx.x3_bytes) ? reinterpret_cast<op16_t*>(cx.x3) : nullptr; }
inline int nt_operand(Call& cx, ActIn A, int al, int bl, int M, int& lda, int& ldb, int& K, const op16_t*& A16) {
#if CC_OP == 2
    if (al || bl || (A.img && A.img != K)) return CC_ERR_ARG;
    if (A.img) {
        A16 = reinterpret_cast<const op16_t*>(A.p);
    } else {
        int rc = CC_OK;
        A16 = x3_operand(cx, A.p, (size_t)lda, M, K, 0, true, &rc);
        if (!A16) return rc;
    }
    lda = 3 * K; ldb = 3 * ldb; K = 3 * K;
#else
    if (A.img) return CC_ERR_ARG;
    A16 = A.p;
#endif
    return CC_OK;
}
constexpr size_t WGRAD_SCRATCH_BYTES = size_t(96) << 20;
struct WgradBatch {
    struct Item { const float* slabs; size_t slab; int ks, Nw; float* dW; int ldw; size_t n4; };
    Item it[8];
    int n = 0;
    size_t used = 0;
    bool defer = false;
    struct Deferred { const op16_t* X; const op16_t* Y; int ldx, ldy, Mw, Nw, K; float* dW; int ldw; };
    Deferred d[32];
    int nd = 0;
    int cap = 4;
    bool direct = false;
    float* scratch = nullptr;
};
int wgrad_flush(WgradBatch& b, hipStream_t st);
int gemm_wgrad(ActIn X, int ldx, const act_t* Y, int ldy, int Mw, int Nw, int K, float* dW, int ldw, float* scratch,
               Call& cx, WgradBatch* batch = nullptr);
struct SkinnyFuse {
    const float* ln_gamma = nullptr;
    const float* ln_beta = nullptr;
    act_t* ln_out16 = nullptr;
    act_t* kcache = nullptr;
    act_t* vcache = nullptr;
    int Tn = 1, pos0 = 0, ctx_max = 0;
    const op16_t* bimg = nullptr;
};
int skinny_image(const op16_t* W, op16_t* img, int N, int K, hipStream_t st);
int gemm_nt_skinny(ActIn A, int lda, const op16_t* B, int ldb, int M, int N, int K, const float* bias, int act, const float* res,
                   float* out32, act_t* out16, int ldo, float* scratch, size_t scratch_bytes, Call& cx,
                   const SkinnyFuse* fuse = nullptr);
struct LmFix { const float* fac; const int* target; const op16_t* wte; };
int gemm_nt_deepk(ActIn A, int lda, const op16_t* B, int ldb, int M, int N, int K, act_t* out16, int ldo, float* scratch,
                  size_t scratch_bytes, Call& cx, const LmFix* fix = nullptr);
int skinny_single_min_tiles();
bool gemm_nt_skinny_can_fuse(int M, int N, int K, size_t scratch_bytes);
}
```

clipcap_amd/csrc/gemm_inst_f32.hip:

```cpp
#include "gemm.hip.h"
#include <algorithm>
#include "gemm_api.h"
namespace CC_NS {
static int gemm_f32out_op(int al, int bl, const op16_t* A, int lda, const op16_t* B, int ldb, int M, int N, int K, float* C, int ldc,
                          const float* bias, int mode, float alpha, int ksplit, hipStream_t st) {
    if ((ldc & 3) || (N & 7)) return CC_ERR_SHAPE;
    if (ksplit > 1 && mode != 2) return CC_ERR_ARG;
    EpiF32 e{C, bias, ldc, M, N, mode, alpha};
    return launch_gemm(al, bl, A, lda, B, ldb, M, N, K, ksplit, e, st);
}
int gemm_f32out(int al, int bl, ActIn A, int lda, const op16_t* B, int ldb, int M, int N, int K, float* C, int ldc,
                const float* bias, int mode, float alpha, int ksplit, Call& cx) {
    const hipStream_t st = cx.st;
    cc_shared::ProfScope _all(cc_shared::SITE_ALL_GEMMS, st, 2.0 * M * N * (double)K);
    const op16_t* A16;
    const int rca = nt_operand(cx, A, al, bl, M, lda, ldb, K, A16);
    if (rca != CC_OK) return rca;
    return gemm_f32out_op(al, bl, A16, lda, B, ldb, M, N, K, C, ldc, bias, mode, alpha, ksplit, st);
}
__global__ __launch_bounds__(256) void k_slab_reduce(const float* __restrict__ slabs, size_t slab_elems, int ks, int Nw, float* __restrict__ dW,
                                                     int ldw, size_t n4) {
    for (size_t i = (size_t)blockIdx.x * blockDim.x + threadIdx.x; i < n4; i += (size_t)gridDim.x * blockDim.x) {
        float4 a = reinterpret_cast<const float4*>(slabs)[i];
        for (int s = 1; s < ks; s++) {
            const float4 b = reinterpret_cast<const float4*>(slabs + s * slab_elems)[i];
            a.x += b.x; a.y += b.y; a.z += b.z; a.w += b.w;
        }
        const size_t e = i * 4;
        float* d = dW + (e / Nw) * ldw + (e % Nw);
        const float4 c = *reinterpret_cast<const float4*>(d);
        *reinterpret_cast<float4*>(d) = make_float4(a.x + c.x, a.y + c.y, a.z + c.z, a.w + c.w);
    }
}

struct SlabItems { WgradBatch::Item it[8]; };
__global__ __launch_bounds__(256) void k_slab_reduce_multi(SlabItems items) {
    const WgradBatch::Item& q = items.it[blockIdx.y];
    for (size_t i = (size_t)blockIdx.x * blockDim.x + threadIdx.x; i < q.n4; i += (size_t)gridDim.x * blockDim.x) {
        float4 a = reinterpret_cast<const float4*>(q.slabs)[i];
        for (int s = 1; s < q.ks; s++) {
            const float4 b = reinterpret_cast<const float4*>(q.slabs + s * q.slab)[i];
            a.x += b.x; a.y += b.y; a.z += b.z; a.w += b.w;
        }
        const size_t e = i * 4;
        float* d = q.dW + (e / q.Nw) * q.ldw + (e % q.Nw);
        const float4 c = *reinterpret_cast<const float4*>(d);
        *reinterpret_cast<float4*>(d) = make_float4(a.x + c.x, a.y + c.y, a.z + c.z, a.w + c.w);
    }
}
static int wgrad_launch_group(WgradBatch& b, hipStream_t st) {
    if (b.nd == 0) return CC_OK;
    TTGroup grp;
    grp.n = b.nd;
    grp.mode = 0;
    const int K = b.d[0].K;
    if (b.direct) {
        double fl = 0.0;
        for (int i = 0; i < b.nd; i++) fl += 2.0 * b.d[i].Mw * b.d[i].Nw * (double)K;
        cc_shared::ProfScope _alld(cc_shared::SITE_ALL_GEMMS, st, fl);
        const bool t256 = (K % H_BK) == 0;
        const int tile = t256 ? 256 : 128;
        const int kt64 = (K + G_BK - 1) / G_BK;
        int first = 0;
        for (int i = 0; i < b.nd; i++) {
            const auto& d = b.d[i];
            grp.A[i] = d.X; grp.B[i] = d.Y;
            grp.g[i] = GemmShape{d.Mw, d.Nw, d.K, d.ldx, d.ldy, kt64 * G_BK, 8, 0};
            grp.slab[i] = d.dW; grp.zstride[i] = 0; grp.ldc[i] = d.ldw;
            grp.first[i] = first;
            first += ((d.Mw + tile - 1) / tile) * ((d.Nw + tile - 1) / tile);
        }
        for (int i = b.nd; i <= TT_GROUP_MAX; i++) grp.first[i] = first;
        grp.mode = 1;
        if (t256) {
            static const bool tail_on = []() { const char* e = cc_lab_env("CC_WGRAD_TAIL"); return !e || atoi(e) != 0; }();
            const int full = (first / 256) * 256, rem = first - full;
            int sp = rem > 0 ? 256 / rem : 1;
            sp = std::min(sp, std::min(8, std::max(1, (K / H_BK) / 16)));
            if (tail_on && full > 0 && sp >= 2 && b.scratch && b.n == 0 && (size_t)rem * sp * H_BM * H_BN * sizeof(float) <= WGRAD_SCRATCH_BYTES) {
                grp.whole = full; grp.split = sp; grp.tail = b.scratch;
            }
        }
        b.nd = 0;
        return t256 ? launch_gemm_tt256_group(grp, st) : launch_gemm_tt128_group(grp, st);
    }
    double flops = 0.0;
    for (int i = 0; i < b.nd; i++) flops += 2.0 * b.d[i].Mw * b.d[i].Nw * (double)K;
    cc_shared::ProfScope _all(cc_shared::SITE_ALL_GEMMS, st, flops);
    size_t slab_sum = 0;
    for (int i = 0; i < b.nd; i++) slab_sum += (((size_t)b.d[i].Mw * b.d[i].Nw * sizeof(float)) + 255) & ~size_t(255);
    const size_t room = WGRAD_SCRATCH_BYTES - b.used;
    static const int force_tile = []() { const char* e = cc_lab_env("CC_WGRAD_TILE"); return e ? atoi(e) : 0; }();
    static const int force_ks = []() { const char* e = cc_lab_env("CC_WGRAD_KS"); return e ? atoi(e) : 0; }();
    int best_tile = 128, best_ks = 1;
    double best_cost = 1e30;
    for (int tile : {256, 128}) {
        if (force_tile && tile != force_tile) continue;
        if (tile == 256 && (K % H_BK)) continue;
        const int bk = tile == 256 ? H_BK : G_BK, ksteps = K / bk;
        int total = 0;
        for (int i = 0; i < b.nd; i++) total += ((b.d[i].Mw + tile - 1) / tile) * ((b.d[i].Nw + tile - 1) / tile);
        const double step_cost = tile == 256 ? 1.25 : 1.0, fixed = tile == 256 ? 16.0 : 14.0;
        for (int ks = 1; ks <= 8 && (size_t)ks * slab_sum <= room && ksteps / ks >= 8; ks++) {
            if (force_ks && ks != force_ks) continue;
            const int per = (ksteps + ks - 1) / ks;
            const int rounds = (total * ks + 255) / 256;
            const double cost = rounds * (per * step_cost + fixed);
            if (cost < best_cost) { best_cost = cost; best_tile = tile; best_ks = ks; }
        }
    }
    if (best_cost >= 1e30) return CC_ERR_STATE;
    const int bk = best_tile == 256 ? H_BK : G_BK, ksteps = K / bk;
    const int kt64 = (K + G_BK - 1) / G_BK;
    const int per64 = (kt64 + best_ks - 1) / best_ks, ks = (kt64 + per64 - 1) / per64;
    (void)ksteps;
    int first = 0;
    for (int i = 0; i < b.nd; i++) {
        const auto& d = b.d[i];
        const size_t slab = (size_t)d.Mw * d.Nw;
        float* sc = b.scratch + b.used / sizeof(float);
        const int tiles = ((d.Mw + best_tile - 1) / best_tile) * ((d.Nw + best_tile - 1) / best_tile);
        grp.A[i] = d.X; grp.B[i] = d.Y;
        grp.g[i] = GemmShape{d.Mw, d.Nw, d.K, d.ldx, d.ldy, per64 * G_BK, 8, 0};
        grp.slab[i] = sc; grp.zstride[i] = slab; grp.ldc[i] = d.Nw;
        grp.first[i] = first;
        first += tiles * ks;
        b.it[b.n++] = WgradBatch::Item{sc, slab, ks, d.Nw, d.dW, d.ldw, slab / 4};
        b.used += (size_t)ks * slab * sizeof(float);
        b.used = (b.used + 255) & ~size_t(255);
    }
    for (int i = b.nd; i <= TT_GROUP_MAX; i++) grp.first[i] = first;
    b.nd = 0;
    return best_tile == 256 ? launch_gemm_tt256_group(grp, st) : launch_gemm_tt128_group(grp, st);
}

int wgrad_flush(WgradBatch& b, hipStream_t st) {
    const int rcg = wgrad_launch_group(b, st);
    if (rcg != CC_OK) return rcg;
    if (b.n == 0) return CC_OK;
    SlabItems items;
    size_t nmax = 0;
    for (int i = 0; i < b.n; i++) { items.it[i] = b.it[i]; nmax = std::max(nmax, b.it[i].n4); }
    hipLaunchKernelGGL(k_slab_reduce_multi, dim3((int)std::min<size_t>((nmax + 255) / 256, 1024), b.n), dim3(256), 0, st, items);
    b.n = 0;
    b.used = 0;
    return hipGetLastError() == hipSuccess ? CC_OK : CC_ERR_LAUNCH;
}
static int wgrad_reduce(const float* slabs, size_t slab, int ks, int Nw, float* dW, int ldw, WgradBatch* batch, hipStream_t st) {
    const size_t n4 = slab / 4;
    if (batch) {
        batch->it[batch->n++] = WgradBatch::Item{slabs, slab, ks, Nw, dW, ldw, n4};
        batch->used += (size_t)ks * slab * sizeof(float);
        batch->used = (batch->used + 255) & ~size_t(255);
        if (batch->n == 8) return wgrad_flush(*batch, st);
        return CC_OK;
    }
    hipLaunchKernelGGL(k_slab_reduce, dim3((int)std::min<size_t>((n4 + 255) / 256, 2048)), dim3(256), 0, st, slabs, slab, ks, Nw, dW, ldw, n4);
    return hipGetLastError() == hipSuccess ? CC_OK : CC_ERR_LAUNCH;
}

int gemm_wgrad(ActIn Xa, int ldx, const act_t* Ya, int ldy, int Mw, int Nw, int K, float* dW, int ldw, float* scratch,
               Call& cx, WgradBatch* batch) {
    const hipStream_t st = cx.st;
    if ((Nw & 7) || (ldw & 3)) return CC_ERR_SHAPE;
    const double flops = 2.0 * Mw * Nw * (double)K;
#if CC_OP == 2
    if (Mw & 7) return CC_ERR_SHAPE;
    if (Xa.img && Xa.img != Mw) return CC_ERR_ARG;
    int rcx = CC_OK;
    const bool ximg = Xa.img != 0;
    const op16_t* X = ximg ? reinterpret_cast<const op16_t*>(Xa.p) : x3_operand(cx, Xa.p, (size_t)ldx, K, Mw, 0, true, &rcx);
    if (!X) return rcx;
    const op16_t* Y = x3_operand(cx, Ya, (size_t)ldy, K, Nw, 1, ximg, &rcx);
    if (!Y) return rcx;
    ldx = Mw; ldy = Nw; K *= 3;
    const bool may_defer = false;
#else
    if (Xa.img) return CC_ERR_ARG;
    const op16_t* X = Xa.p;
    const op16_t* Y = Ya;
    const bool may_defer = true;
#endif
    const size_t slab = (size_t)Mw * Nw;
    const bool tt_ok = (Mw & 7) == 0 && (ldx & 7) == 0 && (ldy & 7) == 0 && ((uintptr_t)X & 15) == 0 && ((uintptr_t)Y & 15) == 0;
    if (batch && scratch && batch->n > 0 && WGRAD_SCRATCH_BYTES - batch->used < 2 * slab * sizeof(float)) {
        const int rcf = wgrad_flush(*batch, st);
        if (rcf != CC_OK) return rcf;
    }
    const size_t slab_bytes = ((slab * sizeof(float)) + 255) & ~size_t(255);
    if (may_defer && batch && batch->defer && g_gemm_tile_mode != 0 && tt_ok && scratch && (K % G_BK) == 0 && K >= 1024 && (slab & 3) == 0 &&
        slab_bytes <= WGRAD_SCRATCH_BYTES && (batch->nd == 0 || batch->d[0].K == K)) {
        size_t pending = 0;
        for (int i = 0; i < batch->nd; i++) pending += (((size_t)batch->d[i].Mw * batch->d[i].Nw * sizeof(float)) + 255) & ~size_t(255);
        const int cap = std::min(std::max(batch->cap, 1), 32);
        if (batch->nd == cap || (!batch->direct && (batch->n + batch->nd >= 8 || batch->used + pending + slab_bytes > WGRAD_SCRATCH_BYTES))) {
            const int rcf = wgrad_flush(*batch, st);
            if (rcf != CC_OK) return rcf;
        }
        batch->scratch = scratch;
        batch->d[batch->nd++] = WgradBatch::Deferred{X, Y, ldx, ldy, Mw, Nw, K, dW, ldw};
        return CC_OK;
    }
    cc_shared::ProfScope _all(cc_shared::SITE_ALL_GEMMS, st, flops);
    const size_t used = (batch && scratch) ? batch->used : 0;
    float* sc = scratch ? scratch + used / sizeof(float) : nullptr;
    const size_t fit = scratch ? (WGRAD_SCRATCH_BYTES - used) / (slab * sizeof(float)) : 1;
    if (g_gemm_tile_mode != 0 && tt_ok && (K % H_BK) == 0 && (g_gemm_tile_mode == 4 || 2.0 * Mw * Nw * (double)K >= 3e10)) {
        const int tiles = ((Mw + H_BM - 1) / H_BM) * ((Nw + H_BN - 1) / H_BN);
        int ks = std::max(1, 256 / tiles);
        ks = std::min(ks, std::max(1, K / 512));
        if ((size_t)ks > fit) ks = (int)std::max<size_t>(fit, 1);
        if (ks == 1) {
            EpiF32 e{dW, nullptr, ldw, Mw, Nw, 1, 1.0f};
            return launch_gemm_tt256(X, ldx, Y, ldy, Mw, Nw, K, 1, e, nullptr, st);
        }
        EpiF32 e{sc, nullptr, Nw, Mw, Nw, 3, 1.0f};
        e.zstride = slab;
        int ks_eff = 1;
        const int rc = launch_gemm_tt256(X, ldx, Y, ldy, Mw, Nw, K, ks, e, &ks_eff, st);
        if (rc != CC_OK) return rc;
        return wgrad_reduce(sc, slab, ks_eff, Nw, dW, ldw, batch, st);
    }
    const int tiles = ((Mw + G_BM - 1) / G_BM) * ((Nw + G_BN - 1) / G_BN);
    if (g_gemm_tile_mode != 0 && tt_ok && (K % G_BK) == 0 && K >= 1024 && tiles <= 256 && scratch && fit >= 1) {

        int ks = std::max(1, 256 / tiles);
        ks = std::min(ks, std::max(1, K / (4 * G_BK)));
        if ((size_t)ks > fit) ks = (int)fit;
        EpiF32 e{sc, nullptr, Nw, Mw, Nw, 3, 1.0f};
        e.zstride = slab;
        int ks_eff = 1;
        const int rc = launch_gemm_tt128(X, ldx, Y, ldy, Mw, Nw, K, ks, e, &ks_eff, st);
        if (rc != CC_OK) return rc;
        return wgrad_reduce(sc, slab, ks_eff, Nw, dW, ldw, batch, st);
    }
    int ks = 512 / (tiles > 0 ? tiles : 1);
    const int kmax = (K + 255) / 256;
    if (ks > kmax) ks = kmax;
    if (scratch) { if ((size_t)ks > fit) ks = (int)fit; } else ks = 1;
    if (ks <= 1) return gemm_f32out_op(1, 1, X, ldx, Y, ldy, Mw, Nw, K, dW, ldw, nullptr, 1, 1.0f, 1, st);
    EpiF32 e{sc, nullptr, Nw, Mw, Nw, 3, 1.0f};
    e.zstride = slab;
    int rc = launch_gemm(1, 1, X, ldx, Y, ldy, Mw, Nw, K, ks, e, st);
    if (rc != CC_OK) return rc;
    const int kt = (K + G_BK - 1) / G_BK, per = (kt + ks - 1) / ks;
    const int ks_eff = (kt + per - 1) / per;
    return wgrad_reduce(sc, slab, ks_eff, Nw, dW, ldw, batch, st);
}

__global__ __launch_bounds__(256) void k_splitk_finish(const float* __restrict__ slabs, size_t slab_elems, int ks, int M, int N,
                                                       const float* __restrict__ bias, int act, const float* __restrict__ res,
                                                       float* __restrict__ out32, act_t* __restrict__ out16, int ldo) {
    const size_t n8 = (size_t)M * (N >> 3);
    for (size_t i = (size_t)blockIdx.x * blockDim.x + threadIdx.x; i < n8; i += (size_t)gridDim.x * blockDim.x) {
        const int row = (int)(i / (N >> 3)), col = (int)(i % (N >> 3)) * 8;
        const size_t e = (size_t)row * N + col;
        float v[8] = {0, 0, 0, 0, 0, 0, 0, 0};
        for (int s = 0; s < ks; s++) {
            const float4 a = *reinterpret_cast<const float4*>(slabs + s * slab_elems + e);
            const float4 b = *reinterpret_cast<const float4*>(slabs + s * slab_elems + e + 4);
            v[0] += a.x; v[1] += a.y; v[2] += a.z; v[3] += a.w; v[4] += b.x; v[5] += b.y; v[6] += b.z; v[7] += b.w;
        }
        if (bias) {
#pragma unroll
            for (int k = 0; k < 8; k++) v[k] += bias[col + k];
        }
        if (act == 1) {
#pragma unroll
            for (int k = 0; k < 8; k++) v[k] = fmaxf(v[k], 0.f);
        } else if (act == 2) {
#pragma unroll
            for (int k = 0; k < 8; k++) v[k] = gelu_new_f(v[k]);
        }
        const size_t o = (size_t)row * ldo + col;
        if (res) {
#pragma unroll
            for (int k = 0; k < 8; k++) v[k] += res[o + k];
        }
        if (out32) {
            *reinterpret_cast<float4*>(out32 + o) = make_float4(v[0], v[1], v[2], v[3]);
            *reinterpret_cast<float4*>(out32 + o + 4) = make_float4(v[4], v[5], v[6], v[7]);
        }
        if (out16) act_st8(out16 + o, v);
    }
}

__device__ __forceinline__ float block_sum256(float v, float* red) {
    v = wave_sum(v);
    if ((threadIdx.x & 63) == 0) red[threadIdx.x >> 6] = v;
    __syncthreads();
    const float t = red[0] + red[1] + red[2] + red[3];
    __syncthreads();
    return t;
}

__global__ __launch_bounds__(256) void k_splitk_finish_row(const float* __restrict__ slabs, size_t slab_elems, int ks, int M, int N,
                                                           const float* __restrict__ bias, int act, const float* __restrict__ res,
                                                           float* __restrict__ out32, act_t* __restrict__ out16, int ldo, SkinnyFuse f) {
    __shared__ float red[4];
    const int row = blockIdx.x;
    constexpr int MAXV = 3;
    float4 v[MAXV];
    float s1 = 0.f;
    float4 lg_[MAXV], lb_[MAXV];
    if (f.ln_out16) {
#pragma unroll
        for (int it = 0; it < MAXV; it++) {
            const int c = threadIdx.x * 4 + it * 1024;
            if (c < N) { lg_[it] = *reinterpret_cast<const float4*>(f.ln_gamma + c); lb_[it] = *reinterpret_cast<const float4*>(f.ln_beta + c); }
        }
    }
#pragma unroll
    for (int it = 0; it < MAXV; it++) {
        const int c = threadIdx.x * 4 + it * 1024;
        if (c < N) {
            float4 a = make_float4(0, 0, 0, 0);
            const float* sp = slabs + (size_t)row * N + c;
            float4 bb = make_float4(0, 0, 0, 0), rr = make_float4(0, 0, 0, 0);
            if (bias) bb = *reinterpret_cast<const float4*>(bias + c);
            if (res) rr = *reinterpret_cast<const float4*>(res + (size_t)row * ldo + c);
            int s = 0;
            for (; s + 4 <= ks; s += 4) {
                const float4 p0 = *reinterpret_cast<const float4*>(sp + (s + 0) * slab_elems), p1 = *reinterpret_cast<const float4*>(sp + (s + 1) * slab_elems);
                const float4 p2 = *reinterpret_cast<const float4*>(sp + (s + 2) * slab_elems), p3 = *reinterpret_cast<const float4*>(sp + (s + 3) * slab_elems);
                a.x += (p0.x + p1.x) + (p2.x + p3.x); a.y += (p0.y + p1.y) + (p2.y + p3.y);
                a.z += (p0.z + p1.z) + (p2.z + p3.z); a.w += (p0.w + p1.w) + (p2.w + p3.w);
            }
            if (ks - s == 3) {
                const float4 p0 = *reinterpret_cast<const float4*>(sp + (s + 0) * slab_elems), p1 = *reinterpret_cast<const float4*>(sp + (s + 1) * slab_elems);
                const float4 p2 = *reinterpret_cast<const float4*>(sp + (s + 2) * slab_elems);
                a.x += (p0.x + p1.x) + p2.x; a.y += (p0.y + p1.y) + p2.y; a.z += (p0.z + p1.z) + p2.z; a.w += (p0.w + p1.w) + p2.w;
            } else {
                for (; s < ks; s++) {
                    const float4 p = *reinterpret_cast<const float4*>(sp + s * slab_elems);
                    a.x += p.x; a.y += p.y; a.z += p.z; a.w += p.w;
                }
            }
            a.x += bb.x; a.y += bb.y; a.z += bb.z; a.w += bb.w;
            if (act == 2) { a.x = gelu_new_f(a.x); a.y = gelu_new_f(a.y); a.z = gelu_new_f(a.z); a.w = gelu_new_f(a.w); }
            else if (act == 1) { a.x = fmaxf(a.x, 0.f); a.y = fmaxf(a.y, 0.f); a.z = fmaxf(a.z, 0.f); a.w = fmaxf(a.w, 0.f); }
            const size_t o = (size_t)row * ldo + c;
            a.x += rr.x; a.y += rr.y; a.z += rr.z; a.w += rr.w;
            if (out32) *reinterpret_cast<float4*>(out32 + o) = a;
            const act_raw4 pk = act_pack4(a.x, a.y, a.z, a.w);
            if (out16) act_straw4(out16 + o, pk);
            if (f.kcache) {
                const int D = N / 3, which = c / D, cc_ = c - which * D;
                if (which > 0) {
                    const int r = row / f.Tn, t = row - r * f.Tn;
                    act_t* dst = (which == 1 ? f.kcache : f.vcache) + ((size_t)r * f.ctx_max + f.pos0 + t) * D + cc_;
                    act_straw4(dst, pk);
                }
            }
            v[it] = a;
            s1 += a.x + a.y + a.z + a.w;
        }
    }
    if (!f.ln_out16) return;
    const float mu = block_sum256(s1, red) / N;
    float q = 0.f;
#pragma unroll
    for (int it = 0; it < MAXV; it++) {
        const int c = threadIdx.x * 4 + it * 1024;
        if (c < N) { const float a = v[it].x - mu, b = v[it].y - mu, c2 = v[it].z - mu, d = v[it].w - mu; q += a * a + b * b + c2 * c2 + d * d; }
    }
    const float rs = rsqrtf(block_sum256(q, red) / N + 1e-5f);
#pragma unroll
    for (int it = 0; it < MAXV; it++) {
        const int c = threadIdx.x * 4 + it * 1024;
        if (c < N) {
            const float4 g = lg_[it], b = lb_[it];
            act_st4(f.ln_out16 + (size_t)row * N + c, (v[it].x - mu) * rs * g.x + b.x, (v[it].y - mu) * rs * g.y + b.y,
                    (v[it].z - mu) * rs * g.z + b.z, (v[it].w - mu) * rs * g.w + b.w);
        }
    }
}

int skinny_single_min_tiles() {
    static const int v = []() { const char* e = cc_lab_env("CC_SKINNY_SINGLE"); return e ? atoi(e) : 60; }();
    return v;
}
bool gemm_nt_skinny_can_fuse(int M, int N, int K, size_t scratch_bytes) {
    return M > 0 && N > 0 && (N & 7) == 0 && N <= 3072 && (K % G_BK) == 0 && scratch_bytes >= (size_t)M * N * sizeof(float);
}

__global__ __launch_bounds__(256) void k_deepk_finish_lm(const float* __restrict__ slabs, size_t slab_elems, int ks, int M, int N, LmFix f,
                                                         act_t* __restrict__ out16, int ldo) {
    const size_t n8 = (size_t)M * (N >> 3);
    for (size_t i = (size_t)blockIdx.x * blockDim.x + threadIdx.x; i < n8; i += (size_t)gridDim.x * blockDim.x) {
        const int row = (int)(i / (N >> 3)), col = (int)(i % (N >> 3)) * 8;
        const size_t e = (size_t)row * N + col;
        float v[8] = {0, 0, 0, 0, 0, 0, 0, 0}, b[8];
        for (int s = 0; s < ks; s++) {
            const float4 a = *reinterpret_cast<const float4*>(slabs + s * slab_elems + e);
            const float4 c = *reinterpret_cast<const float4*>(slabs + s * slab_elems + e + 4);
            v[0] += a.x; v[1] += a.y; v[2] += a.z; v[3] += a.w; v[4] += c.x; v[5] += c.y; v[6] += c.z; v[7] += c.w;
        }
        const float r = f.fac[2 * row], w = f.fac[2 * row + 1];
#if CC_OP == 2
        act_ld8(reinterpret_cast<const float*>(f.wte) + (size_t)f.target[row] * N + col, b);
#else
        unpack8(*reinterpret_cast<const uint4*>(f.wte + (size_t)f.target[row] * N + col), b);
#endif
#pragma unroll
        for (int k = 0; k < 8; k++) v[k] = r * v[k] - w * b[k];
        act_st8(out16 + (size_t)row * ldo + col, v);
    }
}

int gemm_nt_deepk(ActIn Aa, int lda, const op16_t* B, int ldb, int M, int N, int K, act_t* out16, int ldo, float* scratch,
                  size_t scratch_bytes, Call& cx, const LmFix* fix) {
    const hipStream_t st = cx.st;
    static const int knob = []() { const char* e = cc_lab_env("CC_DEEPK"); return e ? atoi(e) : -1; }();
    if (knob == 0 || g_gemm_tile_mode == 0 || !scratch || (N & 7) || (ldo & 7) || (K % 64) || (lda & 7) || (ldb & 7)) return CC_ERR_SHAPE;
    const long tiles = (long)((M + H_BM - 1) / H_BM) * ((N + H_BN - 1) / H_BN);
    const size_t slab = (size_t)M * N;
    int ks = knob > 0 ? knob : (int)(256 / (tiles > 0 ? tiles : 1));
    const size_t fit = scratch_bytes / (slab * sizeof(float));
    if ((size_t)ks > fit) ks = (int)fit;
    if (ks > K / 2048) ks = K / 2048;
    if (ks < 2 || tiles > 128) return CC_ERR_SHAPE;
    cc_shared::ProfScope _all(cc_shared::SITE_ALL_GEMMS, st, 2.0 * M * N * (double)K);
    const op16_t* A;
    const int rca = nt_operand(cx, Aa, 0, 0, M, lda, ldb, K, A);
    if (rca != CC_OK) return rca;
    EpiF32 e{scratch, nullptr, N, M, N, 3, 1.0f};
    e.zstride = slab;
    int tile = 4, tiles_n = (N + H_BN - 1) / H_BN;
    long tl = tiles;
    if (kX3 && x3_fused_on() && (K % (3 * H_BK)) == 0) {
        tile = 3;
        tiles_n = (N + 191) / 192;
        tl = (long)((M + H_BM - 1) / H_BM) * tiles_n;
        const int nc = K / (3 * H_BK);
        long best = -1;
        int best_ks = ks;
// ... 102 lines not shown
```

clipcap_amd/csrc/kernels.h:

```cpp
#pragma once
#include <algorithm>
#include <cmath>
#include <cstdlib>
#include "common.hip.h"

namespace CC_NS {

int f32_to_bf16(const float* src, op16_t* dst, size_t n, hipStream_t st);
int f32_to_act(const float* src, act_t* dst, size_t n, hipStream_t st);
int wire_pack(const float* src, unsigned short* dst, size_t n, hipStream_t st);
int wire_unpack(const unsigned short* src, float* dst, size_t n, hipStream_t st);
int slice_f32_to_bf16(const float* src, size_t src_stride, act_t* dst, size_t dst_stride, int len, int B, hipStream_t st);
int broadcast_rows(float* dst, size_t dst_stride, const float* src, int len, int B, hipStream_t st);
int add_rows(float* dst, size_t dst_stride, const float* add, int len, int B, hipStream_t st);
constexpr size_t RED_SCRATCH_FLOATS = size_t(1) << 20;
int batch_sum(const float* src, size_t src_stride, float* dst, int len, int B, Call& cx);
int copy_rows(const float* src, size_t src_stride, float* dst, size_t dst_stride, int len, int B, hipStream_t st);

int transpose_bf16(const op16_t* src, op16_t* dst, int R, int C, hipStream_t st);
struct TransposeBatch {
    struct Item { const op16_t* src; op16_t* dst; int R, C; };
    Item it[32];
    int n = 0;
    void add(const op16_t* s, op16_t* d, int R, int C) { it[n++] = Item{s, d, R, C}; }
};
int transpose_bf16_multi(const TransposeBatch& b, hipStream_t st);

int ln_fwd(const float* x, int ldx, const int* row_map, const float* gamma, const float* beta, Act y, float* y32, float* mean,
           float* rstd, int rows, int D, hipStream_t st);
int ln_bwd(const act_t* dy, const float* x, int ldx, const int* row_map, const float* mean, const float* rstd, const float* gamma,
           const float* dres, float* dx32, Act dx16, float* dgamma, float* dbeta, int rows, int D, Call& cx,
           float* dcol = nullptr, Drop dmask = Drop());
int colsum_bf16(const act_t* X, int ld, int M, int N, float* out, Call& cx);
struct ColsumBatch { const act_t* X[32]; float* out[32]; int n = 0; void add(const act_t* x, float* o) { X[n] = x; out[n] = o; n++; } };
int colsum_bf16_multi(const ColsumBatch& b, int ld, int M, int N, Call& cx);

int attn_probs(const act_t* qkv, int B, int S, int H, int hd, float* out, hipStream_t st);
int attn_fwd(const act_t* qkv, int B, int S, int H, int hd, bool causal, Act out, float* lse, hipStream_t st, Drop drop = Drop());
int attn_bwd(const act_t* qkv, const act_t* dout, const act_t* o, const float* lse, float* delta, int B, int S, int H, int hd, bool causal,
             Act dqkv, hipStream_t st, Drop drop = Drop());
bool attn_fwd_can_image(int S, int hd);
bool attn_bwd_can_image(int S, int hd);
int dropout_f32(float* x, size_t n, Drop drop, hipStream_t st);
int dropout_bf16(act_t* x, size_t n, Drop drop, hipStream_t st);
int dropout_mask_u8(unsigned char* out, size_t n, Drop drop, hipStream_t st);

int embed_concat(const float* prefix, const long long* tokens, int cap, const float* wte, const float* wpe, float* x0, int B, int L,
                 int T, int D, int pos0, hipStream_t st);
int f32_to_op16_pad(const float* src, long long lds, int V, act_t* dst, int ldd, int M, hipStream_t st);
constexpr int SCATTER_CHUNK = 512;
constexpr unsigned SC_SKIP = 0xffffffffu;
struct ScatterSrc {
    const int* ids32 = nullptr;
    const long long* ids64 = nullptr;
    const float* f32 = nullptr;
    size_t bstride = 0;
    int rpb = 1;
    size_t ids_ld = 1;
    const act_t* act = nullptr;
    const float* fac = nullptr;
};
size_t scatter_ws_bytes(int R, int D);
int scatter_rows(const ScatterSrc& s, int R, int D, int Vp, float* dst, void* ws, hipStream_t st);

int ce_rows(const float* pmax, const float* psum, int npart, const int* target, const float* tgt_logit, float* lse, float* row_loss,
            float* stats, int M, hipStream_t st);
int score_rows(const float* pmax, const float* psum, int npart, const int* keep, const float* tgt_logit, float* lse, float* token_logprob,
               float* sample_stats, int B, int cap, hipStream_t st);
int ce_dlogits(act_t* logits, int ld, int V, const int* target, const float* lse, const float* denom, const float* loss_scale, int M,
               hipStream_t st, op16_t* img = nullptr);
int sample_rows(const float* logits, int R, int V, int ld, float temperature, int top_k, float top_p, int mode, const long long* hist,
                int hist_len, int hist_ld, float rep_pen, const float* u, int* next_token, float* probs_out, hipStream_t st, int stop_tok = -1,
                float len_pen = 1.0f);
int ce_targets(const long long* tokens, int* target, int* row_map, int B, int cap, int L, int T, hipStream_t st);
int score_keep(const long long* tokens, int* keep, int n, int ignore_zero, hipStream_t st);
int lm_tgt_ref(const act_t* hf, const op16_t* wte, int D, const int* target, float* cref, int M, hipStream_t st);
int lm_rowfac(const float* cref, const float* lse, const int* target, const float* denom, const float* loss_scale, float* fac, int M, hipStream_t st);
int lm_dgrad_fix(act_t* dhf, const float* fac, const int* target, const op16_t* wte, int D, int M, hipStream_t st);
int lm_scale_rows(const act_t* hf, const float* fac, act_t* out, int D, int M, hipStream_t st);

int adamw(float* p, const float* g, float* m, float* v, size_t n, float lr, float b1, float b2, float eps, float wd, int step, float gscale,
          const float* loss_scale, const float* found_inf, hipStream_t st, op16_t* w16 = nullptr);
int grad_nonfinite(const float* g, size_t n, float* found_inf, hipStream_t st);

int x3_split_rows(const float* src, size_t lds, op16_t* dst, int M, int K, int form, hipStream_t st);
struct X3SplitBatch {
    struct Item { const float* src; op16_t* dst; int R, C, tr, form; };
    Item it[32];
    int n = 0;
    void add(const float* s, op16_t* d, int R, int C, int tr, int form) { it[n++] = Item{s, d, R, C, tr, form}; }
};
int x3_split_multi(const X3SplitBatch& b, hipStream_t st);
int loss_scale_update(float* state, float* found_inf, float growth, float backoff, int interval, hipStream_t st);

}
```

clipcap_amd/csrc/kernels.hip:

```cpp
#include "kernels.h"
#include "gemm_api.h"

namespace CC_NS {

__global__ void k_f32_to_bf16(const float* __restrict__ src, op16_t* __restrict__ dst, size_t n8) {
    for (size_t i = (size_t)blockIdx.x * blockDim.x + threadIdx.x; i < n8; i += (size_t)gridDim.x * blockDim.x) {
        const float4 a = reinterpret_cast<const float4*>(src)[2 * i], b = reinterpret_cast<const float4*>(src)[2 * i + 1];
        float v[8] = {a.x, a.y, a.z, a.w, b.x, b.y, b.z, b.w};
        reinterpret_cast<uint4*>(dst)[i] = pack8(v);
    }
}
int f32_to_bf16(const float* src, op16_t* dst, size_t n, hipStream_t st) {
    if (n & 7) return CC_ERR_SHAPE;
    const size_t n8 = n >> 3;
    if (!n8) return CC_OK;
    const int grid = (int)std::min<size_t>((n8 + 255) / 256, 2048);
    hipLaunchKernelGGL(k_f32_to_bf16, dim3(grid), dim3(256), 0, st, src, dst, n8);
    return CC_OK;
}

__device__ __forceinline__ unsigned short wire_bf16(float f) {
    const unsigned u = __float_as_uint(f);
    if ((u & 0x7fffffffu) > 0x7f800000u) return (unsigned short)((u >> 16) | 0x40u);
    return (unsigned short)((u + 0x7fffu + ((u >> 16) & 1u)) >> 16);
// ... 271 lines not shown
#pragma unroll
    for (int it = 0; it < NV; it++) {
        const int c = lane * 4 + it * 256;
        g[it] = c < D ? *reinterpret_cast<const float4*>(gamma + c) : make_float4(0, 0, 0, 0);
        bt[it] = c < D ? *reinterpret_cast<const float4*>(beta + c) : make_float4(0, 0, 0, 0);
    }
    float mu[R], rs[R];
#pragma unroll
    for (int r = 0; r < R; r++) {
        float s = 0.f;
#pragma unroll
        for (int it = 0; it < NV; it++) s += v[r][it].x + v[r][it].y + v[r][it].z + v[r][it].w;
        mu[r] = wave_sum(s) / D;
        float q = 0.f;
#pragma unroll
        for (int it = 0; it < NV; it++) {
            const int c = lane * 4 + it * 256;
            if (c < D) {
                const float a = v[r][it].x - mu[r], b = v[r][it].y - mu[r], cc_ = v[r][it].z - mu[r], d = v[r][it].w - mu[r];
                q += a * a + b * b + cc_ * cc_ + d * d;
            }
        }
        rs[r] = rsqrtf(wave_sum(q) / D + eps);
    }
#pragma unroll
    for (int r = 0; r < R; r++) {
        const int row = row0 + r;
        if (row >= rows) break;
        if (lane == 0) {
            if (mean) mean[row] = mu[r];
            if (rstd) rstd[row] = rs[r];
        }
#pragma unroll
        for (int it = 0; it < NV; it++) {
            const int c = lane * 4 + it * 256;
            if (c < D) {
                const float o0 = (v[r][it].x - mu[r]) * rs[r] * g[it].x + bt[it].x, o1 = (v[r][it].y - mu[r]) * rs[r] * g[it].y + bt[it].y;
                const float o2 = (v[r][it].z - mu[r]) * rs[r] * g[it].z + bt[it].z, o3 = (v[r][it].w - mu[r]) * rs[r] * g[it].w + bt[it].w;
#if CC_OP == 2
                if (y && img) {
                    const unsigned h01 = pack2op(o0, o1), h23 = pack2op(o2, o3);
                    float a0, a1, a2, a3;
                    unpack2(h01, a0, a1);
                    unpack2(h23, a2, a3);
                    const uint2 hi = make_uint2(h01, h23), lo = make_uint2(pack2op(o0 - a0, o1 - a1), pack2op(o2 - a2, o3 - a3));
                    op16_t* r3 = reinterpret_cast<op16_t*>(y) + (size_t)row * 3 * D + c;
                    *reinterpret_cast<uint2*>(r3) = hi;
                    *reinterpret_cast<uint2*>(r3 + D) = hi;
                    *reinterpret_cast<uint2*>(r3 + 2 * D) = lo;
                } else
#endif
                if (y) act_st4(y + (size_t)row * D + c, o0, o1, o2, o3);
                if (y32) *reinterpret_cast<float4*>(y32 + (size_t)row * D + c) = make_float4(o0, o1, o2, o3);
            }
        }
    }
}
int ln_fwd(const float* x, int ldx, const int* row_map, const float* gamma, const float* beta, Act yo, float* y32,
           float* mean, float* rstd, int rows, int D, hipStream_t st) {
    if (D > LN_MAXV * 256 || (D & 3) || (ldx & 3)) return CC_ERR_SHAPE;
    if (rows <= 0) return CC_OK;
    const int rpb = D <= 1024 ? 8 : 4;
    const dim3 gr((rows + rpb - 1) / rpb);
    act_t* const y = yo.p;
    const int img = yo.img ? 1 : 0;
    if (img && (!kX3 || yo.img != D)) return CC_ERR_STATE;
#define LN_FWD(NV) hipLaunchKernelGGL(k_ln_fwd<NV>, gr, dim3(256), 0, st, x, ldx, row_map, gamma, beta, y, y32, mean, rstd, rows, D, 1e-5f, img)
    if (D <= 256) LN_FWD(1); else if (D <= 512) LN_FWD(2); else if (D <= 768) LN_FWD(3); else if (D <= 1024) LN_FWD(4); else LN_FWD(LN_MAXV);
#undef LN_FWD
    return CC_OK;
}

template <int NV, bool DG, int NW>
__global__ __launch_bounds__(NW * 64) void k_ln_bwd(const act_t* __restrict__ dy, const float* __restrict__ x, int ldx,
                                                const int* __restrict__ row_map, const float* __restrict__ mean,
                                                const float* __restrict__ rstd, const float* __restrict__ gamma,
                                                const float* __restrict__ dres, float* __restrict__ dx32,
                                                act_t* __restrict__ dx16, float* __restrict__ dgamma, float* __restrict__ dbeta,
                                                float* __restrict__ dcol, int rows, int D, Drop dmask, int img, float* __restrict__ part) {
    extern __shared__ __attribute__((aligned(16))) float ln_red[];
    const int lane = threadIdx.x & 63, wave = threadIdx.x >> 6;
    float4 pg[DG ? NV : 1], pb[DG ? NV : 1], pc[DG ? NV : 1];
#pragma unroll
    for (int it = 0; it < (DG ? NV : 1); it++) pg[it] = pb[it] = pc[it] = make_float4(0, 0, 0, 0);
    float4 gmv[NV];
#pragma unroll
    for (int it = 0; it < NV; it++) {
        const int c = lane * 4 + it * 256;
        gmv[it] = c < D ? *reinterpret_cast<const float4*>(gamma + c) : make_float4(0, 0, 0, 0);
    }
    struct RowIn { act_raw4 d[NV]; float4 xv[NV], rr[NV]; float mu, rs; size_t xr; };
    auto fetch = [&](int row, RowIn& r) {
        r.xr = (size_t)(row_map ? row_map[row] : row) * ldx;
        r.mu = mean[row]; r.rs = rstd[row];
#pragma unroll
        for (int it = 0; it < NV; it++) {
            const int c = lane * 4 + it * 256;
            if (c < D) {
                r.d[it] = act_ldraw4(dy + (size_t)row * D + c);
                r.xv[it] = *reinterpret_cast<const float4*>(x + r.xr + c);
                r.rr[it] = dres ? *reinterpret_cast<const float4*>(dres + r.xr + c) : make_float4(0, 0, 0, 0);
            }
        }
    };
    const int rstep = gridDim.x * NW;
    int row = blockIdx.x * NW + wave;
    RowIn cur;
    if (row < rows) fetch(row, cur);
    for (; row < rows; row += rstep) {
        RowIn nxt;
        const bool more = DG && row + rstep < rows;
        if constexpr (DG) { if (more) fetch(row + rstep, nxt); }
        const size_t xr = cur.xr;
        const float mu = cur.mu, rs = cur.rs;
        float4 g[NV], xh[NV], rr[NV];
        float s1 = 0.f, s2 = 0.f;
#pragma unroll
        for (int it = 0; it < NV; it++) {
            const int c = lane * 4 + it * 256;
            if (c < D) {
                float d0, d1, d2, d3;
                act_unpack4(cur.d[it], d0, d1, d2, d3);
                const float4 xv = cur.xv[it];
                const float4 gm = gmv[it];
                rr[it] = cur.rr[it];
                xh[it] = make_float4((xv.x - mu) * rs, (xv.y - mu) * rs, (xv.z - mu) * rs, (xv.w - mu) * rs);
                g[it] = make_float4(d0 * gm.x, d1 * gm.y, d2 * gm.z, d3 * gm.w);
                s1 += g[it].x + g[it].y + g[it].z + g[it].w;
                s2 += g[it].x * xh[it].x + g[it].y * xh[it].y + g[it].z * xh[it].z + g[it].w * xh[it].w;
                if constexpr (DG) {
                    pg[it].x += d0 * xh[it].x; pg[it].y += d1 * xh[it].y; pg[it].z += d2 * xh[it].z; pg[it].w += d3 * xh[it].w;
                    pb[it].x += d0; pb[it].y += d1; pb[it].z += d2; pb[it].w += d3;
                }
            }
        }
        const float m1 = wave_sum(s1) / D, m2 = wave_sum(s2) / D;
#pragma unroll
        for (int it = 0; it < NV; it++) {
            const int c = lane * 4 + it * 256;
            if (c < D) {
                float4 o = make_float4(rs * (g[it].x - m1 - xh[it].x * m2), rs * (g[it].y - m1 - xh[it].y * m2),
                                       rs * (g[it].z - m1 - xh[it].z * m2), rs * (g[it].w - m1 - xh[it].w * m2));
                o.x += rr[it].x; o.y += rr[it].y; o.z += rr[it].z; o.w += rr[it].w;
                *reinterpret_cast<float4*>(dx32 + xr + c) = o;
                if (dx16) {
                    if (dmask.thresh) {
                        const unsigned e = (unsigned)(xr + c);
                        float m0, m1, m2, m3;
                        drop_mul_pair(dmask, e, m0, m1);
                        drop_mul_pair(dmask, e + 2, m2, m3);
                        o.x *= m0; o.y *= m1; o.z *= m2; o.w *= m3;
                    }
                    const act_raw4 pk = act_pack4(o.x, o.y, o.z, o.w);
#if CC_OP == 2
                    if (img) {
                        const unsigned h01 = pack2op(o.x, o.y), h23 = pack2op(o.z, o.w);
                        float a0, a1, a2, a3;
                        unpack2(h01, a0, a1);
                        unpack2(h23, a2, a3);
                        const uint2 hi = make_uint2(h01, h23), lo = make_uint2(pack2op(o.x - a0, o.y - a1), pack2op(o.z - a2, o.w - a3));
                        op16_t* r3 = reinterpret_cast<op16_t*>(dx16) + 3 * (size_t)xr + c;
                        *reinterpret_cast<uint2*>(r3) = hi;
                        *reinterpret_cast<uint2*>(r3 + D) = hi;
                        *reinterpret_cast<uint2*>(r3 + 2 * D) = lo;
                    } else
#endif
                    act_straw4(dx16 + xr + c, pk);
                    if constexpr (DG) {
                        if (dcol) {
                            float r0, r1, r2, r3;
                            act_unpack4(pk, r0, r1, r2, r3);
                            pc[it].x += r0; pc[it].y += r1; pc[it].z += r2; pc[it].w += r3;
                        }
                    }
                }
            }
        }
        if constexpr (DG) { if (more) cur = nxt; } else { if (row + rstep < rows) fetch(row + rstep, cur); }
    }
    if constexpr (DG) {
        float* rg = ln_red;
        float* rb = ln_red + NW * D;
        float* pp = part + (size_t)blockIdx.x * (dcol ? 3 : 2) * D;
#pragma unroll
        for (int it = 0; it < NV; it++) {
            const int c = lane * 4 + it * 256;
            if (c < D) {
                *reinterpret_cast<float4*>(rg + wave * D + c) = pg[it];
                *reinterpret_cast<float4*>(rb + wave * D + c) = pb[it];
            }
        }
        __syncthreads();
        for (int c = threadIdx.x; c < D; c += NW * 64) {
            float sg = 0.f, sb = 0.f;
#pragma unroll
            for (int w = 0; w < NW; w++) { sg += rg[w * D + c]; sb += rb[w * D + c]; }
            pp[c] = sg;
            pp[D + c] = sb;
        }
        if (dcol) {
            __syncthreads();
#pragma unroll
            for (int it = 0; it < NV; it++) {
                const int c = lane * 4 + it * 256;
                if (c < D) *reinterpret_cast<float4*>(rg + wave * D + c) = pc[it];
            }
            __syncthreads();
            for (int c = threadIdx.x; c < D; c += NW * 64) {
                float sc = 0.f;
#pragma unroll
                for (int w = 0; w < NW; w++) sc += rg[w * D + c];
                pp[2 * D + c] = sc;
            }
        }
    }
}
int ln_bwd(const act_t* dy, const float* x, int ldx, const int* row_map, const float* mean, const float* rstd,
           const float* gamma, const float* dres, float* dx32, Act dxo, float* dgamma, float* dbeta, int rows, int D,
           Call& cx, float* dcol, Drop dmask) {
    const hipStream_t st = cx.st;
    act_t* const dx16 = dxo.p;
    if (D > LN_MAXV * 256 || (D & 3) || (ldx & 3) || (dcol && (!dgamma || !dx16 || row_map)) || (dmask.thresh && (row_map || ldx != D)))
        return CC_ERR_SHAPE;
    if (rows <= 0) return CC_OK;
    const int nw = (dgamma && (size_t)16 * D * sizeof(float) <= 65536) ? 8 : 4;
    static const int dg_grid = []() { const char* e = cc_lab_env("CC_LNBWD_GRID"); return e ? atoi(e) : 256; }();
    const int nvec = dcol ? 3 : 2;
    const int grid = std::min((rows + nw - 1) / nw, dgamma ? std::max(1, std::min(dg_grid, (int)(RED_SCRATCH_FLOATS / ((size_t)nvec * D)))) : 8192);
    float* part = dgamma ? red_scratch(cx, (size_t)grid * nvec * D) : nullptr;
    if (dgamma && !part) return CC_ERR_STATE;
    const size_t sh = dgamma ? (size_t)2 * nw * D * sizeof(float) : 0;
    const int img = dxo.img ? 1 : 0;
    if (img && (!kX3 || dxo.img != D || ldx != D || dcol || dmask.thresh)) return CC_ERR_STATE;
#define LN_BWD(NV, DG, NW) hipLaunchKernelGGL((k_ln_bwd<NV, DG, NW>), dim3(grid), dim3(NW * 64), sh, st, dy, x, ldx, row_map, mean, rstd, gamma, dres, dx32, dx16, dgamma, dbeta, dcol, rows, D, dmask, img, part)
#define LN_BWD_D(DG, NW) { if (D <= 256) LN_BWD(1, DG, NW); else if (D <= 512) LN_BWD(2, DG, NW); else if (D <= 768) LN_BWD(3, DG, NW); else if (D <= 1024) LN_BWD(4, DG, NW); else LN_BWD(LN_MAXV, DG, NW); }
    if (dgamma && nw == 8) LN_BWD_D(true, 8) else if (dgamma) LN_BWD_D(true, 4) else LN_BWD_D(false, 4)
#undef LN_BWD_D
#undef LN_BWD
    if (!dgamma) return CC_OK;
    FoldOut o{};
    o.p[0] = dgamma; o.p[1] = dbeta; o.p[2] = dcol; o.m = D; o.k = nvec;
    return fold_partials(part, grid, nvec * D, 1, o, st);
}

__global__ __launch_bounds__(256) void k_colsum_bf16(const act_t* __restrict__ X, int ld, int M, int N, float* __restrict__ out,
                                                     int rows_per_slice, float* __restrict__ part) {
    __shared__ float red[32][65];
    const int cg = threadIdx.x & 7, rl = threadIdx.x >> 3;
    const int col = blockIdx.x * 64 + cg * 8;
    const int r0 = blockIdx.y * rows_per_slice, r1 = min(M, r0 + rows_per_slice);
    float acc[8] = {0, 0, 0, 0, 0, 0, 0, 0};
    if (col < N) {
        for (int r = r0 + rl; r < r1; r += 32) {
            float f[8];
            act_ld8(X + (size_t)r * ld + col, f);
#pragma unroll
            for (int e = 0; e < 8; e++) acc[e] += f[e];
        }
    }
#pragma unroll
    for (int e = 0; e < 8; e++) red[rl][cg * 8 + e] = acc[e];
    __syncthreads();
    if (threadIdx.x < 64) {
        float s = 0.f;
#pragma unroll
        for (int r = 0; r < 32; r++) s += red[r][threadIdx.x];
        const int c = blockIdx.x * 64 + threadIdx.x;
        if (c < N) {
            if (gridDim.y == 1) out[c] += s;
            else part[(size_t)blockIdx.y * N + c] = s;
        }
    }
}
__global__ __launch_bounds__(256) void k_colsum_bf16_multi(ColsumBatch b, int ld, int M, int N, int rows_per_slice, float* __restrict__ part) {
    __shared__ float red[32][65];
    const act_t* __restrict__ X = b.X[blockIdx.z];
    float* __restrict__ out = b.out[blockIdx.z];
    const int cg = threadIdx.x & 7, rl = threadIdx.x >> 3;
    const int col = blockIdx.x * 64 + cg * 8;
    const int r0 = blockIdx.y * rows_per_slice, r1 = min(M, r0 + rows_per_slice);
    float acc[8] = {0, 0, 0, 0, 0, 0, 0, 0};
    if (col < N) {
        for (int r = r0 + rl; r < r1; r += 32) {
            float f[8];
            act_ld8(X + (size_t)r * ld + col, f);
#pragma unroll
            for (int e = 0; e < 8; e++) acc[e] += f[e];
        }
    }
#pragma unroll
    for (int e = 0; e < 8; e++) red[rl][cg * 8 + e] = acc[e];
    __syncthreads();
    if (threadIdx.x < 64) {
        float s = 0.f;
#pragma unroll
        for (int r = 0; r < 32; r++) s += red[r][threadIdx.x];
        const int c = blockIdx.x * 64 + threadIdx.x;
        if (c < N) {
            if (gridDim.y == 1) out[c] += s;
            else part[((size_t)blockIdx.z * gridDim.y + blockIdx.y) * N + c] = s;
        }
    }
}
int colsum_bf16_multi(const ColsumBatch& b, int ld, int M, int N, Call& cx) {
    const hipStream_t st = cx.st;
    if ((N & 7) || (ld & 7) || b.n < 0 || b.n > 32) return CC_ERR_SHAPE;
    if (M <= 0 || N <= 0 || b.n == 0) return CC_OK;
    const int cb = (N + 63) / 64;
    int slices = std::max(1, std::min((M + 255) / 256, std::max(1, 1024 / (cb * b.n))));
    const int rps = ((M + slices - 1) / slices + 31) / 32 * 32;
    slices = (M + rps - 1) / rps;
    float* part = slices > 1 ? red_scratch(cx, (size_t)b.n * slices * N) : nullptr;
    if (slices > 1 && !part) return CC_ERR_STATE;
    hipLaunchKernelGGL(k_colsum_bf16_multi, dim3(cb, slices, b.n), dim3(256), 0, st, b, ld, M, N, rps, part);
    if (hipGetLastError() != hipSuccess) return CC_ERR_LAUNCH;
    if (slices == 1) return CC_OK;
    FoldOut o{};
    for (int i = 0; i < b.n; i++) o.p[i] = b.out[i];
    o.m = N; o.k = 1;
    return fold_partials(part, slices, N, b.n, o, st);
}
int colsum_bf16(const act_t* X, int ld, int M, int N, float* out, Call& cx) {
    const hipStream_t st = cx.st;
    if ((N & 7) || (ld & 7)) return CC_ERR_SHAPE;
    if (M <= 0 || N <= 0) return CC_OK;
    const int cb = (N + 63) / 64;
    int slices = std::max(1, std::min((M + 255) / 256, 1024 / cb));
    const int rps = ((M + slices - 1) / slices + 31) / 32 * 32;
    slices = (M + rps - 1) / rps;
    float* part = slices > 1 ? red_scratch(cx, (size_t)slices * N) : nullptr;
    if (slices > 1 && !part) return CC_ERR_STATE;
    hipLaunchKernelGGL(k_colsum_bf16, dim3(cb, slices), dim3(256), 0, st, X, ld, M, N, out, rps, part);
    if (slices == 1) return CC_OK;
    FoldOut o{};
    o.p[0] = out; o.m = N; o.k = 1;
    return fold_partials(part, slices, N, 1, o, st);
}

__device__ __forceinline__ void load_head_rows(float* dst, int hdp, const act_t* src, size_t ld, int S, int hd) {
    const int c8n = hd >> 3;
    for (int idx = threadIdx.x; idx < S * c8n; idx += blockDim.x) {
        const int r = idx / c8n, c = idx % c8n;
        float f[8];
        act_ld8(src + (size_t)r * ld + c * 8, f);
        float* d = dst + r * hdp + c * 8;
        *reinterpret_cast<float4*>(d) = make_float4(f[0], f[1], f[2], f[3]);
        *reinterpret_cast<float4*>(d + 4) = make_float4(f[4], f[5], f[6], f[7]);
    }
}

template <bool CAUSAL, bool DROP = false>
__global__ __launch_bounds__(256) void k_attn_fwd(const act_t* __restrict__ qkv, int S, int H, int hd, float scale,
                                                  act_t* __restrict__ out, float* __restrict__ lse, Drop drop = Drop(), int img = 0) {
    extern __shared__ __attribute__((aligned(16))) float sm[];
    const int D = H * hd, hdp = hd + 4, Sp = S + 1;
    float* Qs = sm;
    float* Ks = Qs + S * hdp;
    float* Vs = Ks + S * hdp;
    float* Ps = Vs + S * hdp;
    const int b = blockIdx.x / H, h = blockIdx.x % H;
    const act_t* base = qkv + (size_t)b * S * 3 * D + h * hd;
    load_head_rows(Qs, hdp, base, 3 * D, S, hd);
    load_head_rows(Ks, hdp, base + D, 3 * D, S, hd);
    load_head_rows(Vs, hdp, base + 2 * D, 3 * D, S, hd);
    __syncthreads();
    const int nib = (S + 3) >> 2;
    for (int idx = threadIdx.x; idx < nib * S; idx += 256) {
        const int ib = idx / S, j = idx % S, i0 = ib * 4;
        if (CAUSAL && j > i0 + 3) {
#pragma unroll
            for (int ii = 0; ii < 4; ii++)
                if (i0 + ii < S) Ps[(i0 + ii) * Sp + j] = -INFINITY;
            continue;
        }
        float a0 = 0, a1 = 0, a2 = 0, a3 = 0;
        const float* kr = Ks + j * hdp;
        const float* q0 = Qs + min(i0, S - 1) * hdp;
        const float* q1 = Qs + min(i0 + 1, S - 1) * hdp;
        const float* q2 = Qs + min(i0 + 2, S - 1) * hdp;
        const float* q3 = Qs + min(i0 + 3, S - 1) * hdp;
        for (int d = 0; d < hd; d += 4) {
            const float4 k = *reinterpret_cast<const float4*>(kr + d);
            const float4 x0 = *reinterpret_cast<const float4*>(q0 + d), x1 = *reinterpret_cast<const float4*>(q1 + d);
            const float4 x2 = *reinterpret_cast<const float4*>(q2 + d), x3 = *reinterpret_cast<const float4*>(q3 + d);
            a0 += x0.x * k.x + x0.y * k.y + x0.z * k.z + x0.w * k.w;
            a1 += x1.x * k.x + x1.y * k.y + x1.z * k.z + x1.w * k.w;
            a2 += x2.x * k.x + x2.y * k.y + x2.z * k.z + x2.w * k.w;
            a3 += x3.x * k.x + x3.y * k.y + x3.z * k.z + x3.w * k.w;
        }
        const float a[4] = {a0, a1, a2, a3};
#pragma unroll
        for (int ii = 0; ii < 4; ii++)
            if (i0 + ii < S) Ps[(i0 + ii) * Sp + j] = (CAUSAL && j > i0 + ii) ? -INFINITY : a[ii] * scale;
    }
    __syncthreads();
    const int lane = threadIdx.x & 63, wave = threadIdx.x >> 6;
    for (int i = wave; i < S; i += 4) {
        float m = -INFINITY;
        for (int j = lane; j < S; j += 64) m = fmaxf(m, Ps[i * Sp + j]);
        m = wave_max(m);
        float s = 0.f;
        for (int j = lane; j < S; j += 64) {
            const float e = __expf(Ps[i * Sp + j] - m);
            Ps[i * Sp + j] = e;
            s += e;
        }
        s = wave_sum(s);
        const float inv = 1.f / s;
        for (int j = lane; j < S; j += 64) Ps[i * Sp + j] = act_round(Ps[i * Sp + j] * inv);
        if (lane == 0 && lse) lse[((size_t)b * H + h) * S + i] = m + __logf(s);
    }
    __syncthreads();
    const int d4n = hd >> 2;
    for (int idx = threadIdx.x; idx < S * d4n; idx += 256) {
        const int i = idx / d4n, d0 = (idx % d4n) * 4;
        float4 o = make_float4(0, 0, 0, 0);
        const int jmax = CAUSAL ? i + 1 : S;
        for (int j = 0; j < jmax; j++) {
            float p = Ps[i * Sp + j];
            if (DROP) p *= drop_mul(drop, ((unsigned)(b * H + h) * S + i) * S + j);
            const float4 v = *reinterpret_cast<const float4*>(Vs + j * hdp + d0);
            o.x += p * v.x; o.y += p * v.y; o.z += p * v.z; o.w += p * v.w;
        }
#if CC_OP == 2
        if (img) {
            const unsigned h01 = pack2op(o.x, o.y), h23 = pack2op(o.z, o.w);
            float a0, a1, a2, a3;
            unpack2(h01, a0, a1);
            unpack2(h23, a2, a3);
            const uint2 hi = make_uint2(h01, h23), lo = make_uint2(pack2op(o.x - a0, o.y - a1), pack2op(o.z - a2, o.w - a3));
            op16_t* r3 = reinterpret_cast<op16_t*>(out) + ((size_t)b * S + i) * 3 * D + h * hd + d0;
            *reinterpret_cast<uint2*>(r3) = hi;
            *reinterpret_cast<uint2*>(r3 + D) = hi;
            *reinterpret_cast<uint2*>(r3 + 2 * D) = lo;
            continue;
        }
#endif
        act_st4(out + ((size_t)b * S + i) * D + h * hd + d0, o.x, o.y, o.z, o.w);
    }
}

typedef __attribute__((ext_vector_type(16))) float f32x16;

template <int HD> struct AttLd { static constexpr int v = HD == 128 ? 160 : 96; };
template <int HD>
__device__ __forceinline__ op16x8 frag_tr(const op16_t* blk, int nb, int t, int lane) {
    typedef __attribute__((ext_vector_type(4))) short s16x4_t;
    typedef __attribute__((address_space(3))) s16x4_t* lp_t;
    constexpr int LD = AttLd<HD>::v;
    const int half = lane >> 5, j = lane & 15, dsub = (lane >> 4) & 1;
    const op16_t* p = blk + (16 * t + 4 * half + (j >> 2)) * LD + nb * 32 + 16 * dsub + 4 * (j & 3);
    const s16x4_t lo = __builtin_amdgcn_ds_read_tr16_b64_v4i16((lp_t)p);
    const s16x4_t hi = __builtin_amdgcn_ds_read_tr16_b64_v4i16((lp_t)(p + 8 * LD));
    typedef __attribute__((ext_vector_type(8))) short s16x8_t;
    const s16x8_t v = {lo[0], lo[1], lo[2], lo[3], hi[0], hi[1], hi[2], hi[3]};
    return __builtin_bit_cast(op16x8, v);
}

#if CC_OP == 2
__device__ __forceinline__ void x3_split8(const float (&f)[8], op16x8& hi, op16x8& lo) {
    const uint4 h = pack8(f);
    float hf[8], d[8];
    unpack8(h, hf);
#pragma unroll
    for (int e = 0; e < 8; e++) d[e] = f[e] - hf[e];
    hi = __builtin_bit_cast(op16x8, h);
    lo = __builtin_bit_cast(op16x8, pack8(d));
}
template <int HD, bool CAUSAL, bool DROP = false>
__global__ __launch_bounds__(256, 2) void k_attn_fwd_mfma3(const float* __restrict__ qkv, int B, int S, int H, float scale, float* __restrict__ out,
                                                           float* __restrict__ lse_out, Drop drop, int img) {
    constexpr int KK = HD / 16, NB = HD / 32, C8 = HD / 8, LD = AttLd<HD>::v;
    __shared__ __attribute__((aligned(16))) op16_t vsm[4][2][32 * LD];
    const int lane = threadIdx.x & 63, wave = threadIdx.x >> 6;
    const int nqb = (S + 31) >> 5;
    const int item = blockIdx.x * 4 + wave;
    if (item >= B * H * nqb) return;
    const int qb = item % nqb, h = (item / nqb) % H, b = item / (nqb * H);
    const int D = H * HD;
    const size_t rs = (size_t)3 * D;
    const float* base = qkv + (size_t)b * S * rs + h * HD;
    const int half = lane >> 5, q = qb * 32 + (lane & 31);
    op16_t* vh = vsm[wave][0];
    op16_t* vl = vsm[wave][1];
    auto ld8 = [](const float* p, bool ok, float (&f)[8]) {
        const float4 a = *reinterpret_cast<const float4*>(p), c = *reinterpret_cast<const float4*>(p + 4);
        f[0] = ok ? a.x : 0.f; f[1] = ok ? a.y : 0.f; f[2] = ok ? a.z : 0.f; f[3] = ok ? a.w : 0.f;
        f[4] = ok ? c.x : 0.f; f[5] = ok ? c.y : 0.f; f[6] = ok ? c.z : 0.f; f[7] = ok ? c.w : 0.f;
    };
    op16x8 qh[KK], ql[KK];
#pragma unroll
    for (int kk = 0; kk < KK; kk++) {
        float f[8];
        ld8(base + (size_t)min(q, S - 1) * rs + kk * 16 + half * 8, q < S, f);
        x3_split8(f, qh[kk], ql[kk]);
    }
    f32x16 o[NB];
#pragma unroll
    for (int nb = 0; nb < NB; nb++)
#pragma unroll
        for (int r = 0; r < 16; r++) o[nb][r] = 0.f;
    float m = -INFINITY, l = 0.f;
    const int nkb = CAUSAL ? qb + 1 : nqb;
    const int key_l = lane & 31;
    for (int kb = 0; kb < nkb; kb++) {
#pragma unroll
        for (int c = 0; c < HD / 16; c++) {
            const int idx = lane + 64 * c;
            const int vk = idx / C8, vc = idx % C8;
            float f[8];
            ld8(base + 2 * D + (size_t)min(kb * 32 + vk, S - 1) * rs + vc * 8, kb * 32 + vk < S, f);
            op16x8 a, c2;
            x3_split8(f, a, c2);
            *reinterpret_cast<op16x8*>(vh + vk * LD + vc * 8) = a;
            *reinterpret_cast<op16x8*>(vl + vk * LD + vc * 8) = c2;
        }
        f32x16 s;
#pragma unroll
        for (int r = 0; r < 16; r++) s[r] = 0.f;
#pragma unroll
        for (int kk = 0; kk < KK; kk++) {
            float f[8];
            const int key = kb * 32 + key_l;
            ld8(base + D + (size_t)min(key, S - 1) * rs + kk * 16 + half * 8, key < S, f);
            op16x8 kh, kl;
            x3_split8(f, kh, kl);
            s = CC_MFMA_32x32x16(kl, qh[kk], s);
            s = CC_MFMA_32x32x16(kh, ql[kk], s);
            s = CC_MFMA_32x32x16(kh, qh[kk], s);
        }
        float mx = -INFINITY;
#pragma unroll
        for (int r = 0; r < 16; r++) {
            const int kr = kb * 32 + (r & 3) + 8 * (r >> 2) + 4 * half;
            const bool ok = kr < S && (!CAUSAL || kr <= q);
            s[r] = ok ? s[r] * scale : -INFINITY;
            mx = fmaxf(mx, s[r]);
        }
        mx = fmaxf(mx, __shfl_xor(mx, 32, 64));
        const float m_new = fmaxf(m, mx);
        const float alpha = (m == -INFINITY) ? 0.f : __expf(m - m_new);
        float p[16], ps = 0.f;
#pragma unroll
        for (int r = 0; r < 16; r++) {
            p[r] = (m_new == -INFINITY) ? 0.f : __expf(s[r] - m_new);
            ps += p[r];
        }
        ps += __shfl_xor(ps, 32, 64);
        l = l * alpha + ps;
        m = m_new;
#pragma unroll
        for (int nb = 0; nb < NB; nb++)
#pragma unroll
            for (int r = 0; r < 16; r++) o[nb][r] *= alpha;
        if (DROP) {
            const unsigned rowbase = ((unsigned)(b * H + h) * S + min(q, S - 1)) * S;
#pragma unroll
            for (int r = 0; r < 16; r++) p[r] *= drop_mul(drop, rowbase + min(kb * 32 + (r & 3) + 8 * (r >> 2) + 4 * half, S - 1));
        }
        op16x8 ph[2], pl[2];
#pragma unroll
        for (int t = 0; t < 2; t++) {
            const float f[8] = {p[t * 8 + 0], p[t * 8 + 1], p[t * 8 + 2], p[t * 8 + 3], p[t * 8 + 4], p[t * 8 + 5], p[t * 8 + 6], p[t * 8 + 7]};
            x3_split8(f, ph[t], pl[t]);
        }
#pragma unroll
        for (int t = 0; t < 2; t++)
#pragma unroll
            for (int nb = 0; nb < NB; nb++) {
                const op16x8 fh = frag_tr<HD>(vh, nb, t, lane), fl = frag_tr<HD>(vl, nb, t, lane);
                o[nb] = CC_MFMA_32x32x16(fl, ph[t], o[nb]);
                o[nb] = CC_MFMA_32x32x16(fh, pl[t], o[nb]);
                o[nb] = CC_MFMA_32x32x16(fh, ph[t], o[nb]);
            }
    }
    if (q < S) {
        const float inv = l > 0.f ? 1.f / l : 0.f;
#pragma unroll
        for (int nb = 0; nb < NB; nb++)
#pragma unroll
            for (int g = 0; g < 4; g++) {
                const int d0 = nb * 32 + 8 * g + 4 * half;
                const float o0 = o[nb][g * 4 + 0] * inv, o1 = o[nb][g * 4 + 1] * inv, o2 = o[nb][g * 4 + 2] * inv, o3 = o[nb][g * 4 + 3] * inv;
                if (img) {
                    const unsigned h01 = pack2op(o0, o1), h23 = pack2op(o2, o3);
                    float a0, a1, a2, a3;
                    unpack2(h01, a0, a1);
                    unpack2(h23, a2, a3);
                    const uint2 hi = make_uint2(h01, h23), lo = make_uint2(pack2op(o0 - a0, o1 - a1), pack2op(o2 - a2, o3 - a3));
                    op16_t* r3 = reinterpret_cast<op16_t*>(out) + ((size_t)b * S + q) * 3 * D + h * HD + d0;
                    *reinterpret_cast<uint2*>(r3) = hi;
                    *reinterpret_cast<uint2*>(r3 + D) = hi;
                    *reinterpret_cast<uint2*>(r3 + 2 * D) = lo;
                } else {
                    *reinterpret_cast<float4*>(out + ((size_t)b * S + q) * D + h * HD + d0) = make_float4(o0, o1, o2, o3);
                }
            }
        if (half == 0 && lse_out) lse_out[((size_t)b * H + h) * S + q] = m + __logf(l);
    }
}
template <int HD>
static int attn_fwd_mfma3_launch(const float* qkv, int B, int S, int H, bool causal, float* out, float* lse, hipStream_t st, Drop drop, int img) {
    const int items = B * H * ((S + 31) / 32);
    const float scale = 1.0f / sqrtf((float)HD);
    if (drop.thresh) {
        if (!causal) return CC_ERR_SHAPE;
        hipLaunchKernelGGL((k_attn_fwd_mfma3<HD, true, true>), dim3((items + 3) / 4), dim3(256), 0, st, qkv, B, S, H, scale, out, lse, drop, img);
    } else if (causal)
        hipLaunchKernelGGL((k_attn_fwd_mfma3<HD, true>), dim3((items + 3) / 4), dim3(256), 0, st, qkv, B, S, H, scale, out, lse, drop, img);
    else
        hipLaunchKernelGGL((k_attn_fwd_mfma3<HD, false>), dim3((items + 3) / 4), dim3(256), 0, st, qkv, B, S, H, scale, out, lse, drop, img);
    return hipGetLastError() == hipSuccess ? CC_OK : CC_ERR_LAUNCH;
// ... 2406 lines not shown
```

clipcap_amd/csrc/shared.cpp:

```cpp
#include "../../include/clipcap_hip.h"
#ifdef CC_EXPERIMENTS
#include "../../include/clipcap_hip_lab.h"
#endif
#include "shared.h"
#include <dlfcn.h>
#include <rccl/rccl.h>
#include <algorithm>
#include <cstdlib>
#include <cstring>

namespace cc_shared {
int g_gemm_tile_mode = []() { const char* e = cc_lab_env("CC_GEMM_S256"); return e ? atoi(e) : -1; }();
int g_gemm_s64 = []() { const char* e = cc_lab_env("CC_GEMM_S64"); return e ? atoi(e) : -1; }();
int g_gemm_small_x2 = []() { const char* e = cc_lab_env("CC_GEMM_X2"); return e ? atoi(e) : 1; }();
int g_decode_mode = []() {
    const char* g = cc_lab_env("CC_DEC_GROUP");
    const char* p = cc_lab_env("CC_DEC_PK");
    const char* x = cc_lab_env("CC_DEC_XT");
    return ((g ? atoi(g) : 1) ? 1 : 0) | ((p ? atoi(p) : 0) ? 2 : 0) | ((x ? atoi(x) : 0) ? 4 : 0);
}();
Prof g_prof;
int g_decode_last_path = 0;
}

using namespace cc_shared;

extern "C" {

int cc_abi_version(void) { return CC_ABI_VERSION; }

int cc_gemm_tile_mode(int32_t mode) {
    const int old = g_gemm_tile_mode;
    g_gemm_tile_mode = mode;
    return old;
}

int cc_decode_mode(int32_t mode) {
    const int old = g_decode_mode;
    if (mode >= 0) g_decode_mode = mode & 15;
    return old;
}

#ifdef CC_EXPERIMENTS
int cc_decode_last_path(void) { return g_decode_last_path; }
#endif

int cc_gemm_skinny_mode(int32_t mode) {
    const int old = g_gemm_s64;
    g_gemm_s64 = mode;
    return old;
}

int cc_prof_start(int32_t site, int32_t max_samples) {
    if (site < 0 || max_samples < 0 || max_samples > (1 << 16)) return CC_ERR_ARG;
    for (hipEvent_t e : g_prof.ev) (void)hipEventDestroy(e);
    g_prof.ev.clear();
    g_prof.flops.assign((size_t)max_samples, 0.0);
    g_prof.n = 0;
    g_prof.cap = max_samples;
    g_prof.site = site;
    for (int i = 0; i < 2 * max_samples; i++) {
        hipEvent_t e;
        if (hipEventCreate(&e) != hipSuccess) return CC_ERR_LAUNCH;
        g_prof.ev.push_back(e);
    }
    return CC_OK;
}

int cc_prof_stop(float* ms_host, double* flops_host, int32_t* n_host) {
    if (!ms_host || !n_host) return CC_ERR_ARG;
    const int n = std::min(g_prof.n, (int)*n_host);
    for (int i = 0; i < n; i++) {
        if (hipEventSynchronize(g_prof.ev[2 * i + 1]) != hipSuccess) return CC_ERR_LAUNCH;
        if (hipEventElapsedTime(&ms_host[i], g_prof.ev[2 * i], g_prof.ev[2 * i + 1]) != hipSuccess) return CC_ERR_LAUNCH;
        if (flops_host) flops_host[i] = g_prof.flops[i];
    }
    *n_host = n;
    g_prof.site = 0;
    for (hipEvent_t e : g_prof.ev) (void)hipEventDestroy(e);
    g_prof.ev.clear();
    g_prof.flops.clear();
    g_prof.n = g_prof.cap = 0;
    return CC_OK;
}

namespace {
struct Rccl {
    void* h = nullptr;
    ncclResult_t (*get_uid)(ncclUniqueId*) = nullptr;
    ncclResult_t (*init_rank)(ncclComm_t*, int, ncclUniqueId, int) = nullptr;
    ncclResult_t (*all_reduce)(const void*, void*, size_t, ncclDataType_t, ncclRedOp_t, ncclComm_t, hipStream_t) = nullptr;
    ncclResult_t (*destroy)(ncclComm_t) = nullptr;
    ncclResult_t (*count)(const ncclComm_t, int*) = nullptr;
    ncclResult_t (*bcast)(const void*, void*, size_t, ncclDataType_t, int, ncclComm_t, hipStream_t) = nullptr;
    ncclResult_t (*reduce)(const void*, void*, size_t, ncclDataType_t, ncclRedOp_t, int, ncclComm_t, hipStream_t) = nullptr;
    bool ok = false;
    Rccl() {
        const char* names[] = {"librccl.so.1", "librccl.so", "/opt/rocm/lib/librccl.so.1"};
        for (const char* n : names)
            if ((h = dlopen(n, RTLD_NOW | RTLD_GLOBAL))) break;
        if (!h) return;
        get_uid = reinterpret_cast<decltype(get_uid)>(dlsym(h, "ncclGetUniqueId"));
        init_rank = reinterpret_cast<decltype(init_rank)>(dlsym(h, "ncclCommInitRank"));
        all_reduce = reinterpret_cast<decltype(all_reduce)>(dlsym(h, "ncclAllReduce"));
        destroy = reinterpret_cast<decltype(destroy)>(dlsym(h, "ncclCommDestroy"));
        count = reinterpret_cast<decltype(count)>(dlsym(h, "ncclCommCount"));
        bcast = reinterpret_cast<decltype(bcast)>(dlsym(h, "ncclBroadcast"));
        reduce = reinterpret_cast<decltype(reduce)>(dlsym(h, "ncclReduce"));
        ok = get_uid && init_rank && all_reduce && destroy;
    }
};
extern "C++" Rccl& rccl() {
    static Rccl r;
    return r;
}
static_assert(sizeof(ncclUniqueId) == CC_COMM_UID_BYTES, "cc_comm unique id size");
}

int cc_comm_unique_id(uint8_t* uid_host) {
    if (!uid_host) return CC_ERR_ARG;
    if (!rccl().ok) return CC_ERR_STATE;
    ncclUniqueId id;
    if (rccl().get_uid(&id) != ncclSuccess) return CC_ERR_LAUNCH;
    memcpy(uid_host, &id, sizeof(id));
    return CC_OK;
}

int cc_comm_create(void** comm, int32_t nranks, int32_t rank, const uint8_t* uid_host) {
    if (!comm || !uid_host || nranks < 1 || rank < 0 || rank >= nranks) return CC_ERR_ARG;
    if (!rccl().ok) return CC_ERR_STATE;
    ncclUniqueId id;
    memcpy(&id, uid_host, sizeof(id));
    ncclComm_t c = nullptr;
    if (rccl().init_rank(&c, nranks, id, rank) != ncclSuccess) return CC_ERR_LAUNCH;
    *comm = c;
    return CC_OK;
}

int cc_allreduce_bucket(void* comm, void* buf, int64_t count, int32_t dtype, void* stream) {
    if (!comm || !buf || count < 0 || dtype < CC_RED_F32 || dtype > CC_RED_F16) return CC_ERR_ARG;
    if (!rccl().ok) return CC_ERR_STATE;
    if (count == 0) return CC_OK;
    const ncclDataType_t t = dtype == CC_RED_F32 ? ncclFloat32 : dtype == CC_RED_BF16 ? ncclBfloat16 : ncclFloat16;
    return rccl().all_reduce(buf, buf, (size_t)count, t, ncclSum, static_cast<ncclComm_t>(comm), static_cast<hipStream_t>(stream)) == ncclSuccess
               ? CC_OK : CC_ERR_LAUNCH;
}

int cc_broadcast_bucket(void* comm, void* buf, int64_t count, int32_t dtype, int32_t root, void* stream) {
    if (!comm || !buf || count < 0 || root < 0 || dtype < CC_RED_F32 || dtype > CC_RED_F16) return CC_ERR_ARG;
    if (!rccl().ok || !rccl().bcast) return CC_ERR_STATE;
    if (count == 0) return CC_OK;
    const ncclDataType_t t = dtype == CC_RED_F32 ? ncclFloat32 : dtype == CC_RED_BF16 ? ncclBfloat16 : ncclFloat16;
    return rccl().bcast(buf, buf, (size_t)count, t, root, static_cast<ncclComm_t>(comm), static_cast<hipStream_t>(stream)) == ncclSuccess
               ? CC_OK : CC_ERR_LAUNCH;
}

int cc_reduce_bucket(void* comm, void* buf, int64_t count, int32_t dtype, int32_t root, void* stream) {
    if (!comm || !buf || count < 0 || root < 0 || dtype < CC_RED_F32 || dtype > CC_RED_F16) return CC_ERR_ARG;
    if (!rccl().ok || !rccl().reduce) return CC_ERR_STATE;
    if (count == 0) return CC_OK;
    const ncclDataType_t t = dtype == CC_RED_F32 ? ncclFloat32 : dtype == CC_RED_BF16 ? ncclBfloat16 : ncclFloat16;
    return rccl().reduce(buf, buf, (size_t)count, t, ncclSum, root, static_cast<ncclComm_t>(comm), static_cast<hipStream_t>(stream)) == ncclSuccess
               ? CC_OK : CC_ERR_LAUNCH;
}

int cc_comm_count(void* comm, int32_t* nranks) {
    if (!comm || !nranks) return CC_ERR_ARG;
    if (!rccl().ok || !rccl().count) return CC_ERR_STATE;
    int n = 0;
    if (rccl().count(static_cast<ncclComm_t>(comm), &n) != ncclSuccess) return CC_ERR_LAUNCH;
    *nranks = n;
    return CC_OK;
}

int cc_comm_destroy(void* comm) {
    if (!comm) return CC_ERR_ARG;
    if (!rccl().ok) return CC_ERR_STATE;
    return rccl().destroy(static_cast<ncclComm_t>(comm)) == ncclSuccess ? CC_OK : CC_ERR_LAUNCH;
}

}
```

clipcap_amd/csrc/shared.h:

```cpp
#pragma once
#include <hip/hip_runtime.h>
#include <vector>

#include "lab_env.h"

namespace cc_shared {

extern int g_gemm_tile_mode;
extern int g_gemm_s64;
extern int g_gemm_small_x2;
extern int g_decode_mode;
extern int g_decode_last_path;

struct Prof {
    int site = 0, cap = 0, n = 0;
    bool busy = false;
    std::vector<hipEvent_t> ev;
    std::vector<double> flops;
};
extern Prof g_prof;

struct ProfScope {
    hipStream_t st;
    bool on;
    ProfScope(int site, hipStream_t s, double flops = 0.0) : st(s), on(g_prof.site == site && g_prof.n < g_prof.cap && !g_prof.busy) {
        if (on) {
            g_prof.busy = true;
            g_prof.flops[g_prof.n] = flops;
            (void)hipEventRecord(g_prof.ev[2 * g_prof.n], st);
        }
    }
    ~ProfScope() {
        if (on) {
            (void)hipEventRecord(g_prof.ev[2 * g_prof.n + 1], st);
            g_prof.n++;
            g_prof.busy = false;
        }
    }
};

constexpr int SITE_ALL_GEMMS = 100;

}
```

include/clipcap_hip.h:

```cpp
#ifndef CLIPCAP_HIP_H
#define CLIPCAP_HIP_H

#include <stdint.h>

#ifdef __cplusplus
extern "C" {
#endif

#define CC_OK 0
#define CC_ERR_ARG (-1)
#define CC_ERR_SHAPE (-2)
#define CC_ERR_LAUNCH (-3)
#define CC_ERR_STATE (-4)

#define CC_ABI_VERSION 3
int cc_abi_version(void);

#define CC_OP_BF16 0
#define CC_OP_FP16 1
#define CC_OP_BF16X3 2

typedef struct {
    int32_t E;
    int32_t D;
    int32_t P;
    int32_t L;
    int32_t H;
    int32_t N;
    int32_t Hm;
    int32_t W;
    int32_t use_pos;
    int32_t op_dtype;
} cc_mapper_cfg;

#define CC_MAPPER_HEAD_TENSORS 4
#define CC_MAPPER_LAYER_TENSORS 12

int64_t cc_mapper_param_count(const cc_mapper_cfg* cfg);
int cc_mapper_param_offsets(const cc_mapper_cfg* cfg, int64_t* offsets);
int64_t cc_mapper_ws_bytes(const cc_mapper_cfg* cfg, int32_t B, int32_t save);

int cc_mapper_sync_weights(const cc_mapper_cfg* cfg, const float* w32, uint16_t* w16, void* stream);
int cc_mapper_transpose_weights(const cc_mapper_cfg* cfg, uint16_t* w16, void* stream);

int cc_mapper_fwd(const cc_mapper_cfg* cfg, int32_t B, const float* w32, const uint16_t* w16, const float* emb, void* ws,
                  float* out, int32_t save, void* stream);
int cc_mapper_attention_probs(const cc_mapper_cfg* cfg, int32_t B, void* ws, int32_t layer, float* out, void* stream);
int cc_mapper_bwd(const cc_mapper_cfg* cfg, int32_t B, const float* w32, const uint16_t* w16, void* ws, const float* dout,
                  float* g32, void* stream);
int cc_mapper_bwd_range(const cc_mapper_cfg* cfg, int32_t B, const float* w32, const uint16_t* w16, void* ws, const float* dout,
                        float* g32, int32_t l_hi, int32_t l_lo, void* stream);

typedef struct {
    int32_t D;
    int32_t H;
    int32_t NL;
    int32_t V;
    int32_t Vp;
    int32_t NPOS;
    int32_t op_dtype;
} cc_gpt2_cfg;

#define CC_GPT2_HEAD_TENSORS 2
#define CC_GPT2_LAYER_TENSORS 12
#define CC_GPT2_TAIL_TENSORS 2

typedef struct {
    int32_t B;
    int32_t L;
    int32_t T;
    int32_t cap;
    int32_t mode;
    float p_embd, p_attn, p_resid;
    uint64_t drop_seed;
} cc_gpt2_shape;

int64_t cc_gpt2_param_count(const cc_gpt2_cfg* cfg);
int cc_gpt2_param_offsets(const cc_gpt2_cfg* cfg, int64_t* offsets);
int64_t cc_gpt2_ws_bytes(const cc_gpt2_cfg* cfg, const cc_gpt2_shape* shp);

int cc_gpt2_sync_weights(const cc_gpt2_cfg* cfg, const float* w32, uint16_t* w16, void* stream);
int cc_gpt2_transpose_weights(const cc_gpt2_cfg* cfg, uint16_t* w16, void* stream);

int cc_gpt2_embed(const cc_gpt2_cfg* cfg, const cc_gpt2_shape* shp, const float* w32, const float* prefix, const int64_t* tokens,
                  void* ws, void* stream);
int cc_gpt2_embed_from(const cc_gpt2_cfg* cfg, const cc_gpt2_shape* shp, const float* w32, const float* inputs_embeds, void* ws,
                       void* stream);
int cc_gpt2_fwd(const cc_gpt2_cfg* cfg, const cc_gpt2_shape* shp, const float* w32, const uint16_t* w16, void* ws, void* stream);
int cc_gpt2_logits(const cc_gpt2_cfg* cfg, const cc_gpt2_shape* shp, const float* w32, const uint16_t* w16, void* ws, float* logits,
                   int64_t ldl, void* stream);

int cc_gpt2_logits_bwd(const cc_gpt2_cfg* cfg, const cc_gpt2_shape* shp, const float* w32, const uint16_t* w16, void* ws,
                       const float* dlogits, int64_t ldl, float* dx0, float* g32, void* stream);

int cc_lmhead_ce_fwd(const cc_gpt2_cfg* cfg, const cc_gpt2_shape* shp, const float* w32, const uint16_t* w16, void* ws,
                     const int64_t* tokens, float* stats, void* stream);
int cc_lmhead_score(const cc_gpt2_cfg* cfg, const cc_gpt2_shape* shp, const float* w32, const uint16_t* w16, void* ws,
                    const int64_t* tokens, int32_t ignore_zero, float* token_logprob, float* sample_stats, void* stream);
int cc_lmhead_ce_bwd(const cc_gpt2_cfg* cfg, const cc_gpt2_shape* shp, const float* w32, const uint16_t* w16, void* ws,
                     const float* denom, const float* loss_scale, float* g32, void* stream);
int cc_gpt2_bwd(const cc_gpt2_cfg* cfg, const cc_gpt2_shape* shp, const float* w32, const uint16_t* w16, void* ws,
                const int64_t* tokens, float* dprefix, float* g32, void* stream);
int cc_gpt2_bwd_range(const cc_gpt2_cfg* cfg, const cc_gpt2_shape* shp, const float* w32, const uint16_t* w16, void* ws,
                      const int64_t* tokens, float* dprefix, float* g32, int32_t l_hi, int32_t l_lo, void* stream);

int64_t cc_decode_ws_bytes(const cc_gpt2_cfg* cfg, int32_t R, int32_t Tnew);
int cc_decode_fwd(const cc_gpt2_cfg* cfg, int32_t R, int32_t Tnew, int32_t pos0, int32_t ctx_max, const float* w32,
                  const uint16_t* w16, const float* x, uint16_t* kv, const int32_t* row_map, void* ws, float* logits, int64_t ldl,
                  void* stream);
int64_t cc_decode_part_floats(const cc_gpt2_cfg* cfg, int32_t R);
int cc_decode_fwd_p(const cc_gpt2_cfg* cfg, int32_t R, int32_t Tnew, int32_t pos0, int32_t ctx_max, const float* w32,
                    const uint16_t* w16, const float* x, uint16_t* kv, const int32_t* row_map, void* ws, float* logits, int64_t ldl,
                    float* lpart, void* stream);
int cc_decode_fwd_g(const cc_gpt2_cfg* cfg, int32_t R, int32_t Tnew, int32_t pos0, int32_t ctx_max, const float* w32,
                    const uint16_t* w16, const float* x, uint16_t* kv, const int32_t* row_map, int32_t group, void* ws, float* logits,
                    int64_t ldl, float* lpart, void* stream);
int cc_decode_reorder(const cc_gpt2_cfg* cfg, int32_t R_src, int32_t R_dst, int32_t ctx, int32_t ctx_max, const uint16_t* kv_src,
                      uint16_t* kv_dst, const int32_t* src, void* stream);
int cc_beam_step(int32_t S, int32_t beam, int32_t V, const float* logits, int64_t ldl, float temperature, int32_t first,
                 int32_t stop_token, float* scores, float* seq_lengths, uint8_t* has_stopped, int32_t* next_tokens,
                 int32_t* src_rows, void* ws, void* stream);
int cc_beam_step_p(int32_t S, int32_t beam, int32_t V, const float* logits, int64_t ldl, const float* lpart, int32_t npart,
                   float temperature, int32_t first, int32_t stop_token, float* scores, float* seq_lengths, uint8_t* has_stopped,
                   int32_t* next_tokens, int32_t* src_rows, void* ws, void* stream);
int64_t cc_beam_ws_bytes(int32_t S, int32_t beam, int32_t V);
int cc_embed_tokens(const cc_gpt2_cfg* cfg, int32_t R, const float* w32, const int32_t* tokens, float* out, void* stream);
int cc_embed_tokens_bwd(const cc_gpt2_cfg* cfg, int32_t R, const float* dout, const int32_t* tokens, float* dwte, void* stream);
int cc_embed_tokens_bwd_ws(const cc_gpt2_cfg* cfg, int32_t R, const float* dout, const int32_t* tokens, float* dwte, void* ws, void* stream);
int64_t cc_embed_tokens_bwd_ws_bytes(const cc_gpt2_cfg* cfg, int32_t R);
int cc_beam_advance(const cc_gpt2_cfg* cfg, int32_t R, int32_t beam, const float* w32, const int32_t* next_tokens, const int32_t* src_rows,
                    int32_t pos, int32_t ctx_max, const int32_t* row_map_in, int32_t* row_map_out, int32_t step, int32_t tok_ld,
                    const int32_t* tokens_in, int32_t* tokens_out, float* x_out, void* stream);

int cc_adamw_step(float* p32, const float* g32, float* m, float* v, int64_t n, float lr, float beta1, float beta2, float eps,
                  float weight_decay, int32_t step, float grad_scale, const float* loss_scale, const float* found_inf, void* stream);
int cc_adamw_step_cast(int32_t op_dtype, float* p32, const float* g32, float* m, float* v, int64_t n, float lr, float beta1, float beta2,
                       float eps, float weight_decay, int32_t step, float grad_scale, const float* loss_scale, const float* found_inf,
                       uint16_t* w16, void* stream);
int cc_cast_op16(int32_t op_dtype, const float* src, uint16_t* dst, int64_t n, void* stream);
int cc_grad_wire_pack(const float* g32, uint16_t* wire, int64_t n, void* stream);
int cc_grad_wire_unpack(const uint16_t* wire, float* g32, int64_t n, void* stream);
int cc_grad_nonfinite(const float* g32, int64_t n, float* found_inf, void* stream);
int cc_loss_scale_update(float* state, float* found_inf, float growth, float backoff, int32_t interval, void* stream);

int cc_dropout_mask(uint64_t seed, int32_t site, int32_t layer, float p, int64_t n, uint8_t* out, void* stream);

#define CC_COMM_UID_BYTES 128
#define CC_RED_F32 0
#define CC_RED_BF16 1
#define CC_RED_F16 2
int cc_comm_unique_id(uint8_t* uid_host);
int cc_comm_create(void** comm, int32_t nranks, int32_t rank, const uint8_t* uid_host);
int cc_allreduce_bucket(void* comm, void* buf, int64_t count, int32_t dtype, void* stream);
int cc_broadcast_bucket(void* comm, void* buf, int64_t count, int32_t dtype, int32_t root, void* stream);
int cc_reduce_bucket(void* comm, void* buf, int64_t count, int32_t dtype, int32_t root, void* stream);
int cc_comm_count(void* comm, int32_t* nranks);
int cc_comm_destroy(void* comm);

int cc_sample_step(const float* logits, int32_t R, int32_t V, int32_t ld, float temperature, int32_t top_k, float top_p, int32_t mode,
                   const int64_t* history, int32_t hist_len, int32_t hist_ld, float repetition_penalty, const float* u, int32_t* next_token,
                   float* probs_out, void* stream);
int cc_sample_step_lp(const float* logits, int32_t R, int32_t V, int32_t ld, float temperature, int32_t top_k, float top_p, int32_t mode,
                      const int64_t* history, int32_t hist_len, int32_t hist_ld, float repetition_penalty, int32_t stop_token,
                      float length_penalty, const float* u, int32_t* next_token, float* probs_out, void* stream);

int cc_gemm_op16_f32(int32_t op_dtype, int32_t al, int32_t bl, const uint16_t* A, int32_t lda, const uint16_t* B, int32_t ldb, int32_t M, int32_t N,
                     int32_t K, float* C, int32_t ldc, const float* bias, int32_t ksplit, void* stream);
int64_t cc_wgrad_scratch_bytes(void);
int cc_gemm_wgrad(int32_t op_dtype, const uint16_t* X, int32_t ldx, const uint16_t* Y, int32_t ldy, int32_t Mw, int32_t Nw, int32_t K, float* dW, int32_t ldw,
                  float* scratch, void* stream);
int64_t cc_x3_image_bytes(int64_t rows, int64_t depth);
int cc_x3_split_rows(int32_t op_dtype, const float* src, int64_t ld, int32_t rows, int32_t width, int32_t form, uint16_t* dst, void* stream);
int cc_gemm_act(int32_t op_dtype, int32_t al, int32_t bl, const void* A, int32_t a_img, int32_t lda, const uint16_t* B, int32_t ldb, int32_t M, int32_t N,
                int32_t K, void* C, int32_t c_img, int32_t ldc, const float* bias, int32_t act, void* pre, void* x3, int64_t x3_bytes, void* stream);
int cc_gemm_resid(int32_t op_dtype, int32_t al, int32_t bl, const void* A, int32_t a_img, int32_t lda, const uint16_t* B, int32_t ldb, int32_t M, int32_t N,
                  int32_t K, float* out, const float* res, int32_t ld, const float* bias, float p, uint64_t seed, int32_t site, int32_t layer,
                  void* x3, int64_t x3_bytes, void* stream);
int cc_gemm_dact(int32_t op_dtype, int32_t al, int32_t bl, const void* A, int32_t a_img, int32_t lda, const uint16_t* B, int32_t ldb, int32_t M, int32_t N,
                 int32_t K, void* C, int32_t c_img, int32_t ldc, const void* aux, int32_t act, void* x3, int64_t x3_bytes, void* stream);
int cc_gemm_f32(int32_t op_dtype, int32_t al, int32_t bl, const void* A, int32_t a_img, int32_t lda, const uint16_t* B, int32_t ldb, int32_t M, int32_t N,
                int32_t K, float* C, int32_t ldc, const float* bias, int32_t mode, float alpha, int32_t ksplit, void* x3, int64_t x3_bytes,
                void* stream);
int cc_gemm_wgrad_split(int32_t op_dtype, const void* X, int32_t x_img, int32_t ldx, const float* Y, int32_t ldy, int32_t Mw, int32_t Nw, int32_t K,
                     float* dW, int32_t ldw, float* scratch, void* x3, int64_t x3_bytes, void* stream);
int cc_gemm_tile_mode(int32_t mode);
int cc_gemm_skinny_mode(int32_t mode);
int cc_decode_mode(int32_t mode);
int cc_layernorm_fwd(int32_t op_dtype, const float* x, const float* gamma, const float* beta, uint16_t* y, float* mean, float* rstd, int32_t rows,
                     int32_t D, void* stream);
int cc_attention_fwd(int32_t op_dtype, const uint16_t* qkv, int32_t B, int32_t S, int32_t H, int32_t hd, int32_t causal, uint16_t* out, float* lse,
                     void* stream);
int cc_attention_bwd(int32_t op_dtype, const uint16_t* qkv, const uint16_t* dout, const uint16_t* o, const float* lse, float* delta_ws, int32_t B, int32_t S,
                     int32_t H, int32_t hd, int32_t causal, uint16_t* dqkv, void* stream);
int64_t cc_red_scratch_floats(void);
int cc_layernorm_bwd(int32_t op_dtype, const uint16_t* dy, const float* x, int32_t ldx, const int32_t* row_map, const float* mean,
                     const float* rstd, const float* gamma, const float* dres, float* dx32, uint16_t* dx16, float* dgamma, float* dbeta,
                     float* dcol, int32_t rows, int32_t D, float* red_ws, void* stream);
int cc_colsum_bf16(int32_t op_dtype, const uint16_t* X, int32_t ld, int32_t M, int32_t N, float* out, float* red_ws, void* stream);
int cc_colsum_multi(int32_t op_dtype, const uint16_t* const* X_host, float* const* out_host, int32_t n, int32_t ld, int32_t M, int32_t N,
                    float* red_ws, void* stream);
int cc_batch_sum(const float* src, int64_t src_stride, float* dst, int32_t len, int32_t B, float* red_ws, void* stream);

#define CC_SITE_LMHEAD_FWD 1
#define CC_SITE_LMHEAD_DGRAD 2
#define CC_SITE_GPT2_FC_FWD 3
#define CC_SITE_GPT2_PROJ2_FWD 4
#define CC_SITE_GPT2_FC_DGRAD 5
#define CC_SITE_MAPPER_FC1_FWD 6
#define CC_SITE_MAPPER_QKV_FWD 7
#define CC_SITE_MAPPER_WGRAD_FC2 8
#define CC_SITE_ALL_GEMMS 100
int cc_prof_start(int32_t site, int32_t max_samples);
int cc_prof_stop(float* ms_host, double* flops_host, int32_t* n_host);

#ifdef __cplusplus
}
#endif
#endif
```

Measured before the change: 22120 samples/s.

## Overlap weight-gradient GEMMs on a low-priority side stream during backward

Adds a per-device low-priority side stream with an event ring, and moves the mapper and GPT-2 weight-gradient GEMMs, along with the LM-head wte wgrad, onto it so they run concurrently with the data-gradient chain on the main stream. The GPT-2 path stores per-layer gradient buffers in dead forward activations (x1/u/qkv of the layer above) so the main stream can proceed without overwriting inputs the side stream still reads. The batched wgrad tail-split planning is extended to span the whole deferred batch, and the colsum split is sized for the total count. This adds event-sync overhead and a risk of subtle races on buffer reuse, and it may not help if the data-gradient kernels already fill the GPU.

Measured after the change: 21640 samples/s. -2.2%, worse.

```diff
diff --git a/clipcap_amd/_lib.py b/clipcap_amd/_lib.py
--- a/clipcap_amd/_lib.py
+++ b/clipcap_amd/_lib.py
@@ -111,6 +111,7 @@
     "cc_gemm_wgrad_split": (_I, [_I, _P, _I, _I, _P, _I, _I, _I, _I, _P, _I, _P, _P, _L, _P]),
     "cc_gemm_tile_mode": (_I, [_I]),
     "cc_gemm_skinny_mode": (_I, [_I]),
+    "cc_wgrad_overlap_mode": (_I, [_I]),
     "cc_decode_mode": (_I, [_I]),
     "cc_gemm_op16_f32": (_I, [_I, _I, _I, _P, _I, _P, _I, _I, _I, _I, _P, _I, _P, _I, _P]),
     "cc_layernorm_fwd": (_I, [_I, _P, _P, _P, _P, _P, _P, _I, _I, _P]),
diff --git a/clipcap_amd/csrc/api.hip b/clipcap_amd/csrc/api.hip
--- a/clipcap_amd/csrc/api.hip
+++ b/clipcap_amd/csrc/api.hip
@@ -57,6 +57,43 @@
 inline size_t x3_img(size_t rows, size_t depth) { return ((rows * 3 * depth * sizeof(op16_t)) + 255) & ~size_t(255); }
 template <class WS>
 inline Call call_of(hipStream_t st, const WS& w) { return Call{st, w.red, w.x3, w.x3_bytes}; }
+
+struct Fork {
+    cc_shared::SideStream* s = nullptr;
+    hipStream_t main = nullptr;
+    bool open = false;
+    bool on() const { return s != nullptr; }
+    hipStream_t side() const { return s->st; }
+    int begin(hipStream_t st) {
+        main = st;
+        s = cc_shared::side_stream();
+        if (!s) return CC_ERR_STATE;
+        open = true;
+        return side_after_main();
+    }
+    int side_after_main() {
+        hipEvent_t e = s->event();
+        return (hipEventRecord(e, main) == hipSuccess && hipStreamWaitEvent(s->st, e, 0) == hipSuccess) ? CC_OK : CC_ERR_LAUNCH;
+    }
+    int mark(hipEvent_t* e) {
+        *e = s->event();
+        return hipEventRecord(*e, s->st) == hipSuccess ? CC_OK : CC_ERR_LAUNCH;
+    }
+    int main_after(hipEvent_t e) { return hipStreamWaitEvent(main, e, 0) == hipSuccess ? CC_OK : CC_ERR_LAUNCH; }
+    int join() {
+        if (!open) return CC_OK;
+        open = false;
+        hipEvent_t e;
+        const int rc = mark(&e);
+        return rc != CC_OK ? rc : main_after(e);
+    }
+    ~Fork() { (void)join(); }
+};
+constexpr bool kOverlapMapper = true, kOverlapGpt2 = true;
+inline bool wgrad_overlap(bool call_default) {
+    if (kX3) return false;
+    return cc_shared::g_wgrad_overlap < 0 ? call_default : cc_shared::g_wgrad_overlap != 0;
+}
 
 struct MapperOff {
     int64_t lin_w, lin_b, prefix, pos;
@@ -110,6 +147,7 @@
     bool own_grads;
     float* wg_scratch;
     float* red;
+    float* red_side;
     float* adelta;
     uint16_t* gimg;
     char* x3;
@@ -169,9 +207,10 @@
         w.red = cv.take<float>(RED_SCRATCH_FLOATS);
         w.adelta = cv.take<float>((size_t)B * c->H * S);
         w.gimg = kX3 ? reinterpret_cast<uint16_t*>(cv.take<char>(x3_img(M, std::max<size_t>(3 * (size_t)D, c->Hm)))) : nullptr;
+        w.red_side = kX3 ? nullptr : cv.take<float>(RED_SCRATCH_FLOATS);
     } else {
         w.dx32 = nullptr; w.dx16 = w.dx16b = w.dh16 = w.dxn16 = w.datt16 = w.dqkv16 = w.dlin16 = nullptr; w.wg_scratch = nullptr; w.adelta = nullptr;
-        w.red = nullptr;
+        w.red = w.red_side = nullptr;
         w.gimg = nullptr;
         for (int l = 0; l < c->N; l++) w.gdx[l] = w.gdxb[l] = w.gdh[l] = w.gdqkv[l] = nullptr;
         w.own_grads = false;
@@ -518,6 +557,20 @@
     const bool defer_all = kDeferAll && defer_all_on && w.own_grads && 4 * (l_hi - l_lo) <= 32 && M <= defer_rows;
     if (defer_all) { wb.direct = true; wb.cap = 4 * (l_hi - l_lo); }
     ColsumBatch cs;
+    Fork fork;
+    bool overlap = false;
+    Call cxs = cx;
+    if (defer_all && l_hi > l_lo && wgrad_overlap(kOverlapMapper)) {
+        const int t[4] = {wgrad_direct_tiles(w.gdx[0], D, w.h[0], Hm, D, Hm, M, w.wg_scratch), wgrad_direct_tiles(w.gdh[0], Hm, w.xn2[0], D, Hm, D, M, w.wg_scratch),
+                          wgrad_direct_tiles(w.gdxb[0], D, w.att[0], D, D, D, M, w.wg_scratch), wgrad_direct_tiles(w.gdqkv[0], 3 * D, w.xn1[0], D, 3 * D, D, M, w.wg_scratch)};
+        overlap = t[0] > 0 && t[1] > 0 && t[2] > 0 && t[3] > 0;
+        if (overlap) {
+            CC_TRY(fork.begin(st));
+            cxs.st = fork.side();
+            cxs.red = w.red_side;
+            wb.part_total = (t[0] + t[1] + t[2] + t[3]) * (l_hi - l_lo);
+        }
+    }
 #if CC_OP == 2
     static const bool share = []() { const char* e = cc_lab_env("CC_X3_SHARE"); return !e || atoi(e) != 0; }();
     int g2rc = CC_OK;
@@ -539,12 +592,12 @@
         act_t* dx16_below = l > 0 ? w.gdx[l - 1] : w.datt16;
         const ActIn gx = G2(dx16, D);
         CC_TRY(g2rc);
-        CC_TIMED(CC_SITE_MAPPER_WGRAD_FC2, st, gemm_wgrad(gx, D, w.h[l], Hm, D, Hm, M, g32 + y.w2, Hm, w.wg_scratch, cx, &wb));
+        if (!overlap) CC_TIMED(CC_SITE_MAPPER_WGRAD_FC2, st, gemm_wgrad(gx, D, w.h[l], Hm, D, Hm, M, g32 + y.w2, Hm, w.wg_scratch, cx, &wb));
         if (l == c->N - 1) CC_TRY(colsum_bf16(dx16, D, M, D, g32 + y.b2, cx));
         CC_TRY(gemm_dact(0, 0, gx, D, W16(w16t, y.w2), D, M, Hm, D, dh16, Hm, w.h[l], 1, cx));
         const ActIn gh = G2(dh16, Hm);
         CC_TRY(g2rc);
-        CC_TRY(gemm_wgrad(gh, Hm, w.xn2[l], D, Hm, D, M, g32 + y.w1, D, w.wg_scratch, cx, &wb));
+        if (!overlap) CC_TRY(gemm_wgrad(gh, Hm, w.xn2[l], D, Hm, D, M, g32 + y.w1, D, w.wg_scratch, cx, &wb));
         if (defer_all) cs.add(dh16, g32 + y.b1);
         else CC_TRY(colsum_bf16(dh16, Hm, M, Hm, g32 + y.b1, cx));
         CC_TRY(gemm_bf16out(0, 0, gh, Hm, W16(w16t, y.w1), Hm, M, D, Hm, w.dxn16, D, nullptr, 0, nullptr, cx));
@@ -552,23 +605,34 @@
                       g32 + y.n2b, M, D, cx, g32 + y.bp));
         const ActIn gb = G2(dx16b, D);
         CC_TRY(g2rc);
-        CC_TRY(gemm_wgrad(gb, D, w.att[l], D, D, D, M, g32 + y.wp, D, w.wg_scratch, cx, &wb));
+        if (!overlap) CC_TRY(gemm_wgrad(gb, D, w.att[l], D, D, D, M, g32 + y.wp, D, w.wg_scratch, cx, &wb));
         CC_TRY(gemm_bf16out(0, 0, gb, D, W16(w16t, y.wp), D, M, D, D, w.datt16, D, nullptr, 0, nullptr, cx));
         CC_TRY(attn_bwd(w.qkv[l], w.datt16, w.att[l], w.lse[l], w.adelta, B, S, H, hd, false, dqkv16, st));
         const ActIn gq = G2(dqkv16, 3 * D);
         CC_TRY(g2rc);
-        CC_TRY(gemm_wgrad(gq, 3 * D, w.xn1[l], D, 3 * D, D, M, g32 + y.wq, D, w.wg_scratch, cx, &wb));
+        if (!overlap) CC_TRY(gemm_wgrad(gq, 3 * D, w.xn1[l], D, 3 * D, D, M, g32 + y.wq, D, w.wg_scratch, cx, &wb));
         CC_TRY(gemm_bf16out(0, 0, gq, 3 * D, W16(w16t, y.wq), 3 * D, M, D, 3 * D, w.dxn16, D, nullptr, 0, nullptr, cx));
+        if (overlap) {
+            CC_TRY(fork.side_after_main());
+            CC_TIMED(CC_SITE_MAPPER_WGRAD_FC2, cxs.st, gemm_wgrad(gx, D, w.h[l], Hm, D, Hm, M, g32 + y.w2, Hm, w.wg_scratch, cxs, &wb));
+            CC_TRY(gemm_wgrad(gh, Hm, w.xn2[l], D, Hm, D, M, g32 + y.w1, D, w.wg_scratch, cxs, &wb));
+            CC_TRY(gemm_wgrad(gb, D, w.att[l], D, D, D, M, g32 + y.wp, D, w.wg_scratch, cxs, &wb));
+            CC_TRY(gemm_wgrad(gq, 3 * D, w.xn1[l], D, 3 * D, D, M, g32 + y.wq, D, w.wg_scratch, cxs, &wb));
+            CC_TRY(wgrad_flush(wb, cxs.st));
+            CC_TRY(colsum_bf16_multi(cs, Hm, M, Hm, cxs, l_hi - l_lo));
+            cs.n = 0;
+        }
         if (!defer_all) CC_TRY(wgrad_flush(wb, st));
         CC_TRY(ln_bwd(w.dxn16, w.x[l], D, nullptr, w.mean1[l], w.rstd1[l], w32 + y.n1w, w.dx32, w.dx32, dx16_below, g32 + y.n1w,
                       g32 + y.n1b, M, D, cx, l > 0 ? g32 + o.layer[l - 1].b2 : nullptr));
     }
     CC_TRY(wgrad_flush(wb, st));
     CC_TRY(colsum_bf16_multi(cs, Hm, M, Hm, cx));
-    if (l_lo > 0) return CC_OK;
+    if (l_lo > 0) return fork.join();
     CC_TRY(batch_sum(w.dx32 + (size_t)PP * D, (size_t)S * D, g32 + o.prefix, c->L * D, B, cx));
     if (o.pos >= 0) CC_TRY(batch_sum(w.dx32, (size_t)S * D, g32 + o.pos, PP * D, B, cx));
     CC_TRY(slice_f32_to_bf16(w.dx32, (size_t)S * D, w.dlin16, (size_t)PP * D, PP * D, B, st));
+    CC_TRY(fork.join());
     CC_TRY(gemm_wgrad(w.dlin16, PD, w.emb16, c->E, PD, c->E, B * c->W, g32 + o.lin_w, c->E, w.wg_scratch, cx));
     CC_TRY(colsum_bf16(w.dlin16, PD, B * c->W, PD, g32 + o.lin_b, cx));
     return CC_OK;
@@ -828,16 +892,23 @@
         const int rc2 = gemm_bf16out(0, 0, dlog, c->Vp, W16(w16, o.total + o.wte), c->Vp, Mc, D, c->Vp, w.dhf16, D, nullptr, 0, nullptr, cx);
         return (rc2 != CC_OK || !ef) ? rc2 : lm_dgrad_fix(w.dhf16, w.lmfac, w.target, fix.wte, D, Mc, st);
     };
+    Fork fork;
+    Call cxs = cx;
+    if (full && wgrad_overlap(kOverlapGpt2)) {
+        CC_TRY(fork.begin(st));
+        cxs.st = fork.side();
+        cxs.red = nullptr;
+    }
     CC_TIMED(CC_SITE_LMHEAD_DGRAD, st, lm_dgrad());
     if (full) {
         if (ef) {
-            CC_TRY(lm_scale_rows(w.hf16, w.lmfac, w.hfs16, D, Mc, st));
-            CC_TRY(gemm_wgrad(lg, c->Vp, w.hfs16, D, c->Vp, D, Mc, g32 + o.wte, D, w.wg_scratch, cx));
+            CC_TRY(lm_scale_rows(w.hf16, w.lmfac, w.hfs16, D, Mc, cxs.st));
+            CC_TRY(gemm_wgrad(lg, c->Vp, w.hfs16, D, c->Vp, D, Mc, g32 + o.wte, D, w.wg_scratch, cxs));
             ScatterSrc oh;
             oh.ids32 = w.target; oh.act = w.hf16; oh.fac = w.lmfac;
-            CC_TRY(scatter_rows(oh, Mc, D, c->Vp, g32 + o.wte, w.scat, st));
+            CC_TRY(scatter_rows(oh, Mc, D, c->Vp, g32 + o.wte, w.scat, cxs.st));
         } else {
-            CC_TRY(gemm_wgrad(lg, c->Vp, w.hf16, D, c->Vp, D, Mc, g32 + o.wte, D, w.wg_scratch, cx));
+            CC_TRY(gemm_wgrad(lg, c->Vp, w.hf16, D, c->Vp, D, Mc, g32 + o.wte, D, w.wg_scratch, cxs));
         }
     }
     if (hipMemsetAsync(w.dx32, 0, (size_t)M * D * sizeof(float), st) != hipSuccess) return CC_ERR_LAUNCH;
@@ -845,7 +916,7 @@
     if (hipMemsetAsync(w.dx16.p, 0, dx16_bytes, st) != hipSuccess) return CC_ERR_LAUNCH;
     CC_TRY(ln_bwd(w.dhf16, w.x[c->NL], D, w.row_map, w.meanf, w.rstdf, w32 + o.lnf_w, nullptr, w.dx32, w.dx16, full ? g32 + o.lnf_w : nullptr,
                   full ? g32 + o.lnf_b : nullptr, Mc, D, cx));
-    return CC_OK;
+    return fork.join();
 }
 
 int CC_API(cc_gpt2_logits_bwd)(const cc_gpt2_cfg* c, const cc_gpt2_shape* s, const float* w32, const uint16_t* w16, void* ws, const float* dlogits,
@@ -894,42 +965,71 @@
     wb.defer = full;
     WgradBatch* wbp = full ? &wb : nullptr;
     if (full && (w.dx16.img || w.dx16b.img || w.du16.img || w.dqkv16.img)) return CC_ERR_STATE;
+    Fork fork;
+    Call cxs = cx;
+    const bool overlap = full && l_hi > l_lo && wgrad_overlap(kOverlapGpt2);
+    if (overlap) {
+        CC_TRY(fork.begin(st));
+        cxs.st = fork.side();
+        cxs.red = nullptr;
+    }
+    const auto grad_set = [&](int l, Act& dx16, Act& dx16b, Act& du16, Act& dqkv16) {
+        if (!overlap || l >= c->NL - 1) { dx16 = w.dx16; dx16b = w.dx16b; du16 = w.du16; dqkv16 = w.dqkv16; return; }
+        act_t* half = reinterpret_cast<act_t*>(w.x1[l + 1]);
+        dx16 = Act(half); dx16b = Act(half + (size_t)M * D); du16 = Act(w.u[l + 1]); dqkv16 = Act(w.qkv[l + 1]);
+    };
     for (int l = l_hi - 1; l >= l_lo; l--) {
         const auto& y = o.layer[l];
         const bool top = l == c->NL - 1;
-        if (top) CC_TRY(dropout_bf16(w.dx16.p, (size_t)M * D, make_drop(s->p_resid, s->drop_seed, DROP_RESID_MLP, l), st));
+        Act dx16, dx16b, du16, dqkv16, dx16_below, unused[3];
+        grad_set(l, dx16, dx16b, du16, dqkv16);
+        grad_set(l - 1, dx16_below, unused[0], unused[1], unused[2]);
+        const auto wg_p2 = [&](Call& c2) { return gemm_wgrad(w.hact[l], D4, dx16.p, D, D4, D, M, g32 + y.p2w, D, w.wg_scratch, c2, wbp); };
+        const auto wg_fc = [&](Call& c2) { return gemm_wgrad(w.xn2[l], D, du16.p, D4, D, D4, M, g32 + y.fw, D4, w.wg_scratch, c2, wbp); };
+        const auto wg_proj = [&](Call& c2) { return gemm_wgrad(w.att[l], D, dx16b.p, D, D, D, M, g32 + y.pw, D, w.wg_scratch, c2, wbp); };
+        const auto wg_attn = [&](Call& c2) { return gemm_wgrad(w.xn1[l], D, dqkv16.p, D3, D, D3, M, g32 + y.aw, D3, w.wg_scratch, c2, wbp); };
+        if (top) CC_TRY(dropout_bf16(dx16.p, (size_t)M * D, make_drop(s->p_resid, s->drop_seed, DROP_RESID_MLP, l), st));
         if (full) {
-            CC_TRY(gemm_wgrad(w.hact[l], D4, w.dx16.p, D, D4, D, M, g32 + y.p2w, D, w.wg_scratch, cx, wbp));
-            if (top) CC_TRY(colsum_bf16(w.dx16.p, D, M, D, g32 + y.p2b, cx));
+            if (!overlap) CC_TRY(wg_p2(cx));
+            if (top) CC_TRY(colsum_bf16(dx16.p, D, M, D, g32 + y.p2b, cx));
         }
         {
             static const int tile_dact = env_tile("CC_TILE_DACT");
             TileScope ts(tile_dact);
-            CC_TRY(gemm_dact(0, 0, w.dx16, D, W16(w16, y.p2w), D, M, D4, D, w.du16, D4, w.u[l], gelu_grad_fwd() ? 3 : 2, cx));
+            CC_TRY(gemm_dact(0, 0, dx16, D, W16(w16, y.p2w), D, M, D4, D, du16, D4, w.u[l], gelu_grad_fwd() ? 3 : 2, cx));
         }
         if (full) {
-            CC_TRY(gemm_wgrad(w.xn2[l], D, w.du16.p, D4, D, D4, M, g32 + y.fw, D4, w.wg_scratch, cx, wbp));
-            CC_TRY(colsum_bf16(w.du16.p, D4, M, D4, g32 + y.fb, cx));
-        }
-        CC_TIMED(CC_SITE_GPT2_FC_DGRAD, st, gemm_bf16out(0, 0, w.du16, D4, W16(w16, y.fw), D4, M, D, D4, w.dxn16, D, nullptr, 0, nullptr, cx));
-        CC_TRY(ln_bwd(w.dxn16, w.x1[l], D, nullptr, w.mean2[l], w.rstd2[l], w32 + y.l2w, w.dx32, w.dx32, w.dx16b, full ? g32 + y.l2w : nullptr,
+            if (!overlap) CC_TRY(wg_fc(cx));
+            CC_TRY(colsum_bf16(du16.p, D4, M, D4, g32 + y.fb, cx));
+        }
+        CC_TIMED(CC_SITE_GPT2_FC_DGRAD, st, gemm_bf16out(0, 0, du16, D4, W16(w16, y.fw), D4, M, D, D4, w.dxn16, D, nullptr, 0, nullptr, cx));
+        CC_TRY(ln_bwd(w.dxn16, w.x1[l], D, nullptr, w.mean2[l], w.rstd2[l], w32 + y.l2w, w.dx32, w.dx32, dx16b, full ? g32 + y.l2w : nullptr,
                       full ? g32 + y.l2b : nullptr, M, D, cx, full ? g32 + y.pb : nullptr,
                       make_drop(s->p_resid, s->drop_seed, DROP_RESID_ATTN, l)));
-        if (full) CC_TRY(gemm_wgrad(w.att[l], D, w.dx16b.p, D, D, D, M, g32 + y.pw, D, w.wg_scratch, cx, wbp));
-        CC_TRY(gemm_bf16out(0, 0, w.dx16b, D, W16(w16, y.pw), D, M, D, D, w.datt16, D, nullptr, 0, nullptr, cx));
-        CC_TRY(attn_bwd(w.qkv[l], w.datt16, w.att[l].p, w.lse[l], w.adelta, s->B, s->T, H, hd, true, w.dqkv16, st,
+        if (full && !overlap) CC_TRY(wg_proj(cx));
+        CC_TRY(gemm_bf16out(0, 0, dx16b, D, W16(w16, y.pw), D, M, D, D, w.datt16, D, nullptr, 0, nullptr, cx));
+        CC_TRY(attn_bwd(w.qkv[l], w.datt16, w.att[l].p, w.lse[l], w.adelta, s->B, s->T, H, hd, true, dqkv16, st,
                         make_drop(s->p_attn, s->drop_seed, DROP_ATTN, l)));
         if (full) {
-            CC_TRY(gemm_wgrad(w.xn1[l], D, w.dqkv16.p, D3, D, D3, M, g32 + y.aw, D3, w.wg_scratch, cx, wbp));
-            CC_TRY(colsum_bf16(w.dqkv16.p, D3, M, D3, g32 + y.ab, cx));
-        }
-        CC_TRY(gemm_bf16out(0, 0, w.dqkv16, D3, W16(w16, y.aw), D3, M, D, D3, w.dxn16, D, nullptr, 0, nullptr, cx));
-        if (full) CC_TRY(wgrad_flush(wb, st));
-        CC_TRY(ln_bwd(w.dxn16, w.x[l], D, nullptr, w.mean1[l], w.rstd1[l], w32 + y.l1w, w.dx32, w.dx32, w.dx16, full ? g32 + y.l1w : nullptr,
+            if (!overlap) CC_TRY(wg_attn(cx));
+            CC_TRY(colsum_bf16(dqkv16.p, D3, M, D3, g32 + y.ab, cx));
+        }
+        CC_TRY(gemm_bf16out(0, 0, dqkv16, D3, W16(w16, y.aw), D3, M, D, D3, w.dxn16, D, nullptr, 0, nullptr, cx));
+        if (overlap) {
+            CC_TRY(fork.side_after_main());
+            CC_TRY(wg_p2(cxs));
+            CC_TRY(wg_fc(cxs));
+            CC_TRY(wg_proj(cxs));
+            CC_TRY(wg_attn(cxs));
+            CC_TRY(wgrad_flush(wb, cxs.st));
+        } else if (full) {
+            CC_TRY(wgrad_flush(wb, st));
+        }
+        CC_TRY(ln_bwd(w.dxn16, w.x[l], D, nullptr, w.mean1[l], w.rstd1[l], w32 + y.l1w, w.dx32, w.dx32, dx16_below, full ? g32 + y.l1w : nullptr,
                       full ? g32 + y.l1b : nullptr, M, D, cx, (full && l > 0) ? g32 + o.layer[l - 1].p2b : nullptr,
                       l > 0 ? make_drop(s->p_resid, s->drop_seed, DROP_RESID_MLP, l - 1) : Drop()));
     }
-    if (l_lo > 0) return CC_OK;
+    if (l_lo > 0) return fork.join();
     CC_TRY(dropout_f32(w.dx32, (size_t)M * D, make_drop(s->p_embd, s->drop_seed, DROP_EMBD, 0), st));
     if (s->L > 0) CC_TRY(copy_rows(w.dx32, (size_t)s->T * D, dprefix, (size_t)s->L * D, s->L * D, s->B, st));
     if (full) {
@@ -942,7 +1042,7 @@
         }
         CC_TRY(batch_sum(w.dx32, (size_t)s->T * D, g32 + o.wpe, s->T * D, s->B, cx));
     }
-    return CC_OK;
+    return fork.join();
 }
 
 int CC_API(cc_adamw_step)(float* p32, const float* g32, float* m, float* v, int64_t n, float lr, float beta1, float beta2, float eps,
diff --git a/clipcap_amd/csrc/gemm_api.h b/clipcap_amd/csrc/gemm_api.h
--- a/clipcap_amd/csrc/gemm_api.h
+++ b/clipcap_amd/csrc/gemm_api.h
@@ -52,9 +52,11 @@
     int nd = 0;
     int cap = 4;
     bool direct = false;
+    int part_total = 0, part_first = 0;
     float* scratch = nullptr;
 };
 int wgrad_flush(WgradBatch& b, hipStream_t st);
+int wgrad_direct_tiles(const void* X, int ldx, const void* Y, int ldy, int Mw, int Nw, int K, const float* scratch);
 int gemm_wgrad(ActIn X, int ldx, const act_t* Y, int ldy, int Mw, int Nw, int K, float* dW, int ldw, float* scratch,
                Call& cx, WgradBatch* batch = nullptr);
 struct SkinnyFuse {
diff --git a/clipcap_amd/csrc/gemm_inst_f32.hip b/clipcap_amd/csrc/gemm_inst_f32.hip
--- a/clipcap_amd/csrc/gemm_inst_f32.hip
+++ b/clipcap_amd/csrc/gemm_inst_f32.hip
@@ -74,13 +74,16 @@
         grp.mode = 1;
         if (t256) {
             static const bool tail_on = []() { const char* e = cc_lab_env("CC_WGRAD_TAIL"); return !e || atoi(e) != 0; }();
-            const int full = (first / 256) * 256, rem = first - full;
+            const int total = b.part_total > 0 ? b.part_total : first, base = b.part_total > 0 ? b.part_first : 0;
+            const int full = (total / 256) * 256, rem = total - full;
             int sp = rem > 0 ? 256 / rem : 1;
             sp = std::min(sp, std::min(8, std::max(1, (K / H_BK) / 16)));
             if (tail_on && full > 0 && sp >= 2 && b.scratch && b.n == 0 && (size_t)rem * sp * H_BM * H_BN * sizeof(float) <= WGRAD_SCRATCH_BYTES) {
-                grp.whole = full; grp.split = sp; grp.tail = b.scratch;
+                const int whole = std::min(std::max(full - base, 0), first);
+                if (whole < first) { grp.whole = whole; grp.split = sp; grp.tail = b.scratch; }
             }
         }
+        b.part_first += first;
         b.nd = 0;
         return t256 ? launch_gemm_tt256_group(grp, st) : launch_gemm_tt128_group(grp, st);
     }
@@ -132,6 +135,16 @@
     for (int i = b.nd; i <= TT_GROUP_MAX; i++) grp.first[i] = first;
     b.nd = 0;
     return best_tile == 256 ? launch_gemm_tt256_group(grp, st) : launch_gemm_tt128_group(grp, st);
+}
+
+int wgrad_direct_tiles(const void* X, int ldx, const void* Y, int ldy, int Mw, int Nw, int K, const float* scratch) {
+    const size_t slab = (size_t)Mw * Nw;
+    const bool tt_ok = (Mw & 7) == 0 && (Nw & 7) == 0 && (ldx & 7) == 0 && (ldy & 7) == 0 && ((uintptr_t)X & 15) == 0 && ((uintptr_t)Y & 15) == 0;
+    if (kX3 || g_gemm_tile_mode == 0 || !tt_ok || !scratch || (K % G_BK) || K < 1024 || (slab & 3) ||
+        (((slab * sizeof(float)) + 255) & ~size_t(255)) > WGRAD_SCRATCH_BYTES)
+        return 0;
+    const int tile = (K % H_BK) == 0 ? 256 : 128;
+    return ((Mw + tile - 1) / tile) * ((Nw + tile - 1) / tile);
 }
 
 int wgrad_flush(WgradBatch& b, hipStream_t st) {
diff --git a/clipcap_amd/csrc/kernels.h b/clipcap_amd/csrc/kernels.h
--- a/clipcap_amd/csrc/kernels.h
+++ b/clipcap_amd/csrc/kernels.h
@@ -33,7 +33,7 @@
            float* dcol = nullptr, Drop dmask = Drop());
 int colsum_bf16(const act_t* X, int ld, int M, int N, float* out, Call& cx);
 struct ColsumBatch { const act_t* X[32]; float* out[32]; int n = 0; void add(const act_t* x, float* o) { X[n] = x; out[n] = o; n++; } };
-int colsum_bf16_multi(const ColsumBatch& b, int ld, int M, int N, Call& cx);
+int colsum_bf16_multi(const ColsumBatch& b, int ld, int M, int N, Call& cx, int plan_n = 0);
 
 int attn_probs(const act_t* qkv, int B, int S, int H, int hd, float* out, hipStream_t st);
 int attn_fwd(const act_t* qkv, int B, int S, int H, int hd, bool causal, Act out, float* lse, hipStream_t st, Drop drop = Drop());
diff --git a/clipcap_amd/csrc/kernels.hip b/clipcap_amd/csrc/kernels.hip
--- a/clipcap_amd/csrc/kernels.hip
+++ b/clipcap_amd/csrc/kernels.hip
@@ -597,12 +597,12 @@
         }
     }
 }
-int colsum_bf16_multi(const ColsumBatch& b, int ld, int M, int N, Call& cx) {
+int colsum_bf16_multi(const ColsumBatch& b, int ld, int M, int N, Call& cx, int plan_n) {
     const hipStream_t st = cx.st;
-    if ((N & 7) || (ld & 7) || b.n < 0 || b.n > 32) return CC_ERR_SHAPE;
+    if ((N & 7) || (ld & 7) || b.n < 0 || b.n > 32 || plan_n > 32 || (plan_n > 0 && plan_n < b.n)) return CC_ERR_SHAPE;
     if (M <= 0 || N <= 0 || b.n == 0) return CC_OK;
     const int cb = (N + 63) / 64;
-    int slices = std::max(1, std::min((M + 255) / 256, std::max(1, 1024 / (cb * b.n))));
+    int slices = std::max(1, std::min((M + 255) / 256, std::max(1, 1024 / (cb * (plan_n > 0 ? plan_n : b.n)))));
     const int rps = ((M + slices - 1) / slices + 31) / 32 * 32;
     slices = (M + rps - 1) / rps;
     float* part = slices > 1 ? red_scratch(cx, (size_t)b.n * slices * N) : nullptr;
diff --git a/clipcap_amd/csrc/shared.cpp b/clipcap_amd/csrc/shared.cpp
--- a/clipcap_amd/csrc/shared.cpp
+++ b/clipcap_amd/csrc/shared.cpp
@@ -8,6 +8,7 @@
 #include <algorithm>
 #include <cstdlib>
 #include <cstring>
+#include <mutex>
 
 namespace cc_shared {
 int g_gemm_tile_mode = []() { const char* e = cc_lab_env("CC_GEMM_S256"); return e ? atoi(e) : -1; }();
@@ -21,6 +22,33 @@
 }();
 Prof g_prof;
 int g_decode_last_path = 0;
+int g_wgrad_overlap = -1;
+
+SideStream* side_stream() {
+    constexpr int kMaxDev = 64;
+    static std::mutex mu;
+    static SideStream* tab[kMaxDev] = {};
+    int dev = 0;
+    if (hipGetDevice(&dev) != hipSuccess || dev < 0 || dev >= kMaxDev) return nullptr;
+    std::lock_guard<std::mutex> lock(mu);
+    if (tab[dev]) return tab[dev];
+    int least = 0, greatest = 0;
+    if (hipDeviceGetStreamPriorityRange(&least, &greatest) != hipSuccess) return nullptr;
+    SideStream* s = new SideStream;
+    bool ok = hipStreamCreateWithPriority(&s->st, hipStreamNonBlocking, least) == hipSuccess;
+    int made = 0;
+    while (ok && made < 16) {
+        ok = hipEventCreateWithFlags(&s->ev[made], hipEventDisableTiming) == hipSuccess;
+        if (ok) made++;
+    }
+    if (!ok) {
+        for (int i = 0; i < made; i++) (void)hipEventDestroy(s->ev[i]);
+        if (s->st) (void)hipStreamDestroy(s->st);
+        delete s;
+        return nullptr;
+    }
+    return tab[dev] = s;
+}
 }
 
 using namespace cc_shared;
@@ -32,6 +60,12 @@
 int cc_gemm_tile_mode(int32_t mode) {
     const int old = g_gemm_tile_mode;
     g_gemm_tile_mode = mode;
+    return old;
+}
+
+int cc_wgrad_overlap_mode(int32_t mode) {
+    const int old = g_wgrad_overlap;
+    g_wgrad_overlap = mode < 0 ? -1 : (mode ? 1 : 0);
     return old;
 }
 
diff --git a/clipcap_amd/csrc/shared.h b/clipcap_amd/csrc/shared.h
--- a/clipcap_amd/csrc/shared.h
+++ b/clipcap_amd/csrc/shared.h
@@ -11,6 +11,15 @@
 extern int g_gemm_small_x2;
 extern int g_decode_mode;
 extern int g_decode_last_path;
+extern int g_wgrad_overlap;
+
+struct SideStream {
+    hipStream_t st = nullptr;
+    hipEvent_t ev[16] = {};
+    unsigned next = 0;
+    hipEvent_t event() { return ev[next++ & 15]; }
+};
+SideStream* side_stream();
 
 struct Prof {
     int site = 0, cap = 0, n = 0;
diff --git a/include/clipcap_hip.h b/include/clipcap_hip.h
--- a/include/clipcap_hip.h
+++ b/include/clipcap_hip.h
@@ -185,6 +185,7 @@
                      float* dW, int32_t ldw, float* scratch, void* x3, int64_t x3_bytes, void* stream);
 int cc_gemm_tile_mode(int32_t mode);
 int cc_gemm_skinny_mode(int32_t mode);
+int cc_wgrad_overlap_mode(int32_t mode);
 int cc_decode_mode(int32_t mode);
 int cc_layernorm_fwd(int32_t op_dtype, const float* x, const float* gamma, const float* beta, uint16_t* y, float* mean, float* rstd, int32_t rows,
                      int32_t D, void* stream);
```
